# pettni/smooth_feedback

Measured on AMD Instinct MI355X. Metric: QP solves/sec, higher is better.
Workload: dtype f64

## Files before the change

### smooth_feedback_amd/csrc/capi_sparse.hip

```cpp
#include <hip/hip_runtime.h>

#include <algorithm>
#include <chrono>
#include <cstdio>
#include <map>
#include <mutex>
#include <string>
#include <vector>

#include "../../include/sfb.h"
#include "capi_common.h"
#include "qp_sparse_kernel.h"
#include "sparse_plan.h"

struct sfb_sparse_qp_plan {
  sfb::SparsePlanHost host;
  bool pruned = false;
  sfb::SparsePlanHost full;
  std::vector<int32_t> Aorig, Amasked;
  std::mutex mu;
  struct DevCopy {
    int32_t *blob = nullptr, *blob_full = nullptr;
    sfb::SparsePlanDev dev{}, dev_full{};
  };
  std::map<int, DevCopy> per_device;
  struct HostDev {
    std::mutex mu;
    std::pair<char *, size_t> ws{nullptr, 0};
    int64_t batch = -1;
    uint64_t origin = 0;
    hipStream_t stream = nullptr;
    hipEvent_t uploaded = nullptr;
  };
  std::map<int, HostDev> host_dev;
};

namespace sfb {
const SparsePlanHost &plan_host(const sfb_sparse_qp_plan *plan) { return plan->host; }
const SparsePlanHost &plan_io(const sfb_sparse_qp_plan *plan) { return plan->pruned ? plan->full : plan->host; }
}

namespace {

thread_local uint64_t tl_multi_origin = 0;

sfb_status upload_plan(const sfb::SparsePlanHost &h, const std::vector<int32_t> *Aorig, const std::vector<int32_t> *Amasked,
                       int nnzA_io, int32_t **blob_out, sfb::SparsePlanDev &d)
{
  static const std::vector<int32_t> none;
  const std::vector<int32_t> *arrs[] = {&h.Pp, &h.Pi, &h.Pcol, &h.Ap, &h.Aj, &h.Arow, &h.Acp, &h.Aci, &h.Acpos,
                                        &h.Prp, &h.Prj, &h.Prpos, &h.Sp, &h.Sj, &h.Spos, &h.perm, &h.pinv,
                                        &h.Kp, &h.Ki, &h.Kdesc, &h.Lp, &h.Li, &h.Rp, &h.Rk, &h.Rpos, &h.Rlen,
                                        &h.fmap, &h.fidx, &h.bmap, &h.bidx, &h.Kmap, &h.rptr, &h.rtgt, &h.rab, &h.snptr, &h.snR, &h.poff, &h.pmap, &h.fmask, &h.bmask,
                                        &h.f2s, &h.seg, &h.pmapL, &h.rsplit, &h.KmapL, &h.KdescT, &h.KmapT, &h.ztop, &h.ustream, &h.utype, &h.uomap,
                                        Aorig ? Aorig : &none, Amasked ? Amasked : &none};
  constexpr int NA = sizeof(arrs) / sizeof(arrs[0]);
  size_t off[NA + 1];
  off[0] = 0;
  for (int a = 0; a < NA; ++a) off[a + 1] = off[a] + ((arrs[a]->size() + 3) / 4) * 4 + 4;
  const size_t self_words = (sizeof(sfb::SparsePlanDev) + 15) / 16 * 4;
  std::vector<int32_t> blob(off[NA] + self_words, 0);
  for (int a = 0; a < NA; ++a) std::copy(arrs[a]->begin(), arrs[a]->end(), blob.begin() + off[a]);
  int32_t *dblob = nullptr;
  hipError_t e = hipMalloc(reinterpret_cast<void **>(&dblob), blob.size() * sizeof(int32_t));
  if (e != hipSuccess) return sfb::hip_fail(e, "hipMalloc(plan)");
  e = hipMemcpy(dblob, blob.data(), blob.size() * sizeof(int32_t), hipMemcpyHostToDevice);
  if (e != hipSuccess) {
    (void)hipFree(dblob);
    return sfb::hip_fail(e, "hipMemcpy(plan)");
  }
  d.n = h.n; d.m = h.m; d.k = h.k; d.nnzP = h.nnzP; d.nnzA = h.nnzA; d.nnzK = h.nnzK; d.nnzL = h.nnzL;
  const int32_t **ptrs[] = {&d.Pp, &d.Pi, &d.Pcol, &d.Ap, &d.Aj, &d.Arow, &d.Acp, &d.Aci, &d.Acpos,
                            &d.Prp, &d.Prj, &d.Prpos, &d.Sp, &d.Sj, &d.Spos, &d.perm, &d.pinv,
                            &d.Kp, &d.Ki, &d.Kdesc, &d.Lp, &d.Li, &d.Rp, &d.Rk, &d.Rpos, &d.Rlen,
                            &d.fmap, &d.fidx, &d.bmap, &d.bidx, &d.Kmap, &d.rptr, &d.rtgt, &d.rab, &d.snptr, &d.snR, &d.poff, &d.pmap, &d.fmask, &d.bmask,
                            &d.f2s, &d.seg, &d.pmapL, &d.rsplit, &d.KmapL, &d.KdescT, &d.KmapT, &d.ztop, &d.ustream, &d.utype, &d.uomap,
                            &d.Aorig, &d.Amasked};
  d.funits = h.funits; d.bunits = h.bunits; d.ffull0 = h.ffull0; d.ffull1 = h.ffull1; d.bfull0 = h.bfull0; d.bfull1 = h.bfull1; d.idx_scale = h.idx_scale; d.rsteps = h.rsteps; d.maxcol = h.maxcol; d.nsn = h.nsn; d.lds_doubles = h.lds_doubles; d.nseg = h.nseg; d.nnzKT = h.nnzKT; d.nztop = h.nztop; d.units = h.units; d.nunits = h.nunits;
  for (int a = 0; a < NA; ++a) *ptrs[a] = dblob + off[a];
  d.nnzA_io = nnzA_io;
  d.nmasked = Amasked ? (int)Amasked->size() - 512 : 0;
  if (!Aorig) d.Aorig = d.Amasked = nullptr;
  if ((e = sfb::sparse_device_words(&d.dev_active, &d.dev_busy)) != hipSuccess) {
    (void)hipFree(dblob);
    return sfb::hip_fail(e, "launch bookkeeping of the device");
  }
  d.self = reinterpret_cast<const sfb::SparsePlanDev *>(dblob + off[NA]);
  e      = hipMemcpy(dblob + off[NA], &d, sizeof(d), hipMemcpyHostToDevice);
  if (e != hipSuccess) {
    (void)hipFree(dblob);
    return sfb::hip_fail(e, "hipMemcpy(plan struct)");
  }
  *blob_out = dblob;
  return SFB_OK;
}

sfb_status plan_on_device(sfb_sparse_qp_plan *plan, const sfb_sparse_qp_plan::DevCopy **out)
{
  int devid = 0;
  hipError_t e = hipGetDevice(&devid);
  if (e != hipSuccess) return sfb::hip_fail(e, "hipGetDevice");
  std::lock_guard<std::mutex> lk(plan->mu);
  auto it = plan->per_device.find(devid);
  if (it != plan->per_device.end()) {
    *out = &it->second;
    return SFB_OK;
  }
  sfb_sparse_qp_plan::DevCopy dc;
  sfb_status st;
  if (plan->pruned) {
    st = upload_plan(plan->host, &plan->Aorig, &plan->Amasked, plan->full.nnzA, &dc.blob, dc.dev);
    if (st != SFB_OK) return st;
    st = upload_plan(plan->full, nullptr, nullptr, plan->full.nnzA, &dc.blob_full, dc.dev_full);
    if (st != SFB_OK) {
      (void)hipFree(dc.blob);
      return st;
    }
  } else {
    st = upload_plan(plan->host, nullptr, nullptr, plan->host.nnzA, &dc.blob, dc.dev);
    if (st != SFB_OK) return st;
  }
  auto ins = plan->per_device.emplace(devid, dc);
  *out     = &ins.first->second;
  return SFB_OK;
}

struct WsLayout {
  size_t item_bytes, main_bytes, pool_off, aux_off, total;
};
WsLayout ws_layout(const sfb_sparse_qp_plan *plan, int64_t batch)
{
  const sfb::SparsePlanHost &h = plan->host;
  WsLayout L{};
  L.item_bytes = sfb::qp_sparse_ws_doubles(h.n, h.m, h.nnzL, h.funits, h.bunits, plan->pruned ? h.nnzA : 0) * sizeof(double);
  L.main_bytes = (size_t)batch * L.item_bytes;
  L.pool_off   = L.main_bytes;
  size_t pool  = 0;
  if (plan->pruned) {
    const sfb::SparsePlanHost &f = plan->full;
    pool = (size_t)std::min<int64_t>(batch, sfb::qp_sparse_fallback_slots()) *
           sfb::qp_sparse_ws_doubles(f.n, f.m, f.nnzL, f.funits, f.bunits, 0) * sizeof(double);
  }
  L.aux_off = L.pool_off + pool;
  L.total   = L.aux_off + (sfb::qp_sparse_aux_bytes(batch) + 15) / 16 * 16;
  return L;
}

sfb_status check_sparse_args(const sfb_sparse_qp_plan *plan, const sfb_qp_params *prm, int64_t batch, const void *Px,
                             const void *q, const void *Ax, const void *l, const void *u, const void *wx,
                             const void *wy, const void *x, const void *y, const void *code)
{
  if (!plan) return sfb::fail(SFB_ERR_INVALID_ARG, "plan is NULL");
  if (!prm) return sfb::fail(SFB_ERR_INVALID_ARG, "prm is NULL");
  if (batch < 0) return sfb::fail(SFB_ERR_INVALID_ARG, "batch < 0");
  if (batch > 0 && (!q || !l || !u || !x || !y || !code || (plan->host.nnzP > 0 && !Px) || (sfb::plan_io(plan).nnzA > 0 && !Ax)))
    return sfb::fail(SFB_ERR_INVALID_ARG, "NULL problem / solution pointer");
  if ((wx == nullptr) != (wy == nullptr))
    return sfb::fail(SFB_ERR_INVALID_ARG, "warm_x and warm_y must both be given or both be NULL");
  if (prm->max_iter > 0xFFFFFFFFll) return sfb::fail(SFB_ERR_INVALID_ARG, "max_iter exceeds uint32");
  if (batch > 0x7FFFFFFFll) return sfb::fail(SFB_ERR_UNSUPPORTED, "batch exceeds 2^31-1 per call");
  if ((size_t)std::max(plan->host.lds_doubles, plan->pruned ? plan->full.lds_doubles : 0) * sizeof(double) > 150 * 1024)
    return sfb::fail(SFB_ERR_UNSUPPORTED, "n+m too large for the LDS-resident work vector (max 19200)");
  return SFB_OK;
}

}

extern "C" {

sfb_status sfb_sparse_qp_plan_create(int n, int m, const int32_t *P_colptr, const int32_t *P_rowind,
                                     const int32_t *A_rowptr, const int32_t *A_colind, int ordering,
                                     const int32_t *user_perm, sfb_sparse_qp_plan **plan)
{
  return sfb_sparse_qp_plan_create_staged(n, m, P_colptr, P_rowind, A_rowptr, A_colind, ordering, user_perm, nullptr,
                                          plan);
}

sfb_status sfb_sparse_qp_plan_create_staged(int n, int m, const int32_t *P_colptr, const int32_t *P_rowind,
                                            const int32_t *A_rowptr, const int32_t *A_colind, int ordering,
                                            const int32_t *user_perm, const int32_t *stage,
                                            sfb_sparse_qp_plan **plan)
{
  return sfb_sparse_qp_plan_create_pruned(n, m, P_colptr, P_rowind, A_rowptr, A_colind, ordering, user_perm, stage, nullptr,
                                          plan);
}

sfb_status sfb_sparse_qp_plan_create_pruned(int n, int m, const int32_t *P_colptr, const int32_t *P_rowind,
                                            const int32_t *A_rowptr, const int32_t *A_colind, int ordering,
                                            const int32_t *user_perm, const int32_t *stage, const uint8_t *A_keep,
                                            sfb_sparse_qp_plan **plan)
{
  if (!plan) return sfb::fail(SFB_ERR_INVALID_ARG, "plan out-pointer is NULL");
  *plan = nullptr;
  auto *p = new (std::nothrow) sfb_sparse_qp_plan();
  if (!p) return sfb::fail(SFB_ERR_INVALID_ARG, "out of memory");
  const char *msg = "";
  bool any_masked = false;
  if (A_keep && n >= 1 && m >= 1 && A_rowptr && A_rowptr[0] == 0 && A_rowptr[m] >= 0) {
    bool monotone = true;
    for (int r = 0; r < m && monotone; ++r) monotone = A_rowptr[r + 1] >= A_rowptr[r] && A_rowptr[r + 1] <= A_rowptr[m];
    for (int e = 0; monotone && e < A_rowptr[m] && !any_masked; ++e) any_masked = A_keep[e] == 0;
  }
  if (!any_masked) {
    if (!sfb::build_sparse_plan(n, m, P_colptr, P_rowind, A_rowptr, A_colind, ordering, user_perm, stage, p->host, &msg)) {
      delete p;
      return sfb::fail(SFB_ERR_INVALID_ARG, msg);
    }
    *plan = p;
    return SFB_OK;
  }
  const int nnzA = A_rowptr[m];
  if (nnzA > 0 && !A_colind) {
    delete p;
    return sfb::fail(SFB_ERR_INVALID_ARG, "A_colind is NULL");
  }
  std::vector<int32_t> Ap(m + 1, 0), Aj;
  Aj.reserve(nnzA);
  for (int r = 0; r < m; ++r) {
    if (A_rowptr[r + 1] < A_rowptr[r] || A_rowptr[r + 1] > nnzA) {
      delete p;
      return sfb::fail(SFB_ERR_INVALID_ARG, "A row pointers not monotone");
    }
    for (int e = A_rowptr[r]; e < A_rowptr[r + 1]; ++e)
      if (A_colind[e] < 0 || A_colind[e] >= n) {
        delete p;
        return sfb::fail(SFB_ERR_INVALID_ARG, "A column index out of range");
      } else if (A_keep[e]) {
        Aj.push_back(A_colind[e]);
        p->Aorig.push_back(e);
      } else {
        p->Amasked.push_back(e);
      }
// ... 343 lines not shown
```

### smooth_feedback_amd/csrc/knobs.cpp

```cpp
#include "knobs.h"

#include <atomic>
#include <cstdio>
#include <cstring>
#include <deque>
#include <map>
#include <mutex>
#include <string>

namespace sfb {

namespace {
const char *const kKnobs[] = {"SFB_SP_GRID",  "SFB_SP_SLICE",  "SFB_SP_PAUSE",      "SFB_SP_PREDICT",   "SFB_SP_LAT",
                              "SFB_SP_FORCE_LAT", "SFB_SP_LAT_WAVES", "SFB_SP_POLISHERS", "SFB_SP_LAT_HELP", "SFB_SP_PHASED", "SFB_SP_LEAN_WAVES", "SFB_MID_GRID", "SFB_MID_SLICE",
                              "SFB_QP4_MAX_WAVES", "SFB_QP_DENSE_BIG", "SFB_EKF_PERSISTENT", "SFB_PLAN_UNITS", "SFB_PLAN_DEBUG", "SFB_MPC_TIMING"};
std::mutex g_mu;
std::atomic<int> g_set{0};
std::map<std::string, const char *> &table()
{
  static std::map<std::string, const char *> t;
  return t;
}
const char *intern(const char *value)
{
  static std::deque<std::string> pool;
  for (const auto &v : pool)
    if (v == value) return v.c_str();
  pool.emplace_back(value);
  return pool.back().c_str();
}
}

const char *knob(const char *name)
{
  if (g_set.load(std::memory_order_acquire) == 0) return nullptr;
  std::lock_guard<std::mutex> lk(g_mu);
  const auto &t = table();
  const auto it = t.find(name);
  return it == t.end() ? nullptr : it->second;
}

int knob_set(const char *name, const char *value)
{
  if (name == nullptr) return 1;
  bool known = false;
  for (const char *k : kKnobs) known = known || std::strcmp(k, name) == 0;
  if (!known) return 1;
  std::lock_guard<std::mutex> lk(g_mu);
  if (value == nullptr) {
    table().erase(name);
    g_set.store((int)table().size(), std::memory_order_release);
  } else {
    table()[name] = intern(value);
    g_set.store((int)table().size(), std::memory_order_release);
    std::fprintf(stderr, "[sfb] debug knob %s=%s set through sfb_debug_set (tests and measurements only; results do not depend on it)\n",
                 name, value);
  }
  return 0;
}

}
```

### smooth_feedback_amd/csrc/qp_sparse.hip

```cpp
#include <hip/hip_runtime.h>

#include <cstdlib>
#include <map>
#include <mutex>

#include <algorithm>
#include <type_traits>
#include <utility>
#include <cfloat>
#include <cmath>

#include "knobs.h"
#include "../../include/sfb.h"
#include "qp_sparse_kernel.h"
#include "wave_util.h"

#ifndef SFB_SWEEP_ASM
#define SFB_SWEEP_ASM 1
#endif
#ifndef SFB_SWEEP_DEPTH
#define SFB_SWEEP_DEPTH 8
#endif

namespace sfb {

namespace {

__device__ __forceinline__ int uni(const int v) { return __builtin_amdgcn_readfirstlane(v); }

struct Ws {
  double *Lx, *LxF, *LxB, *D, *Dinv, *tv;
  double *sx, *qc, *xs, *xus, *dxus;
  double *sy, *rho, *rinv, *lo, *hi, *ys, *zs, *yus, *zus, *dyus, *act;
  double *hdr;
  double *Axc;
};
constexpr int kHdrStamp = 6, kHdrC = 7, kHdrSigma = 8, kHdrScaling = 9;
constexpr int kHdrCode = 10, kHdrComplete = 11;
[[maybe_unused]] constexpr int kHdrTl2 = 12;
enum { PH_SETUP = 1, PH_ADMM = 2, PH_FINISH = 3 };
constexpr int phases_pack(int ph0, int ph1, unsigned pause_at = 0, int dq_mode = 0)
{
  return ph0 | (ph1 << 4) | (int)((pause_at & 0xFFFFFu) << 8) | (dq_mode << 28);
}
constexpr int PH_EVERYTHING = phases_pack(PH_SETUP, PH_FINISH);
constexpr unsigned long long kFactorStamp = 0x5FB0FAC7A11CE5EDull;

__device__ __forceinline__ Ws carve_ws(double *base, int n, int m, int nnzL, int funits, int bunits)
{
  const int k = n + m;
  Ws w;
  double *p = base;
  w.Lx = p; p += nnzL;
  w.D = p; p += k;
  p += 2;
  w.LxF = p; p += (size_t)(funits + kSweepPadDev) * 128;
  w.LxB = p; p += (size_t)(bunits + kSweepPadDev) * 128;
  w.Dinv = p; p += k;   w.tv = p; p += k;
  w.sx = p; p += n;     w.qc = p; p += n;     w.xs = p; p += n;   w.xus = p; p += n;  w.dxus = p; p += n;
  p += n;
  w.sy = p; p += m;     w.rho = p; p += m;    w.rinv = p; p += m; w.lo = p; p += m;   w.hi = p; p += m;
  w.ys = p; p += m;     w.zs = p; p += m;     w.yus = p; p += m;  w.zus = p; p += m;  w.dyus = p; p += m;
  w.act = p; p += m;
  w.hdr = p; p += 16;
  w.Axc = p;
  return w;
}
__device__ __forceinline__ Ws polish_ws(const Ws &w, double *base, const size_t off, int n, int m, int nnzL, int funits, int bunits)
{
  const int k = n + m;
  Ws v = w;
  double *p = base + off;
  v.Lx = p; p += nnzL;
  v.D = p; p += k;
  p += 2;
  v.LxF = p; p += (size_t)(funits + kSweepPadDev) * 128;
  v.LxB = p; p += (size_t)(bunits + kSweepPadDev) * 128;
  v.Dinv = p;
  return v;
}

struct Item {
  const double *Px, *q, *Ax, *l, *u;
};

typedef int vint4k __attribute__((ext_vector_type(4)));
template<int U>
__device__ __forceinline__ void kkt_fill(const int32_t *__restrict__ desc4, const int32_t *__restrict__ map, const int p_begin,
                                         const int p_end, const Item &it, const Ws &w, double *ACC, const int mode,
                                         const double c, const double sigma, const double delta, const int lane)
{
  const vint4k *desc = reinterpret_cast<const vint4k *>(desc4);
  vint4k dn[U];
  int mn[U];
  auto fetch = [&](const int p0) {
#pragma unroll
    for (int u = 0; u < U; ++u) {
      const bool on = p0 + u * kWave < p_end;
      dn[u] = desc[on ? p0 + u * kWave : p_begin];
      mn[u] = map[on ? p0 + u * kWave : p_begin];
    }
  };
  if (p_begin + lane < p_end) fetch(p_begin + lane);
  for (int p0 = p_begin + lane; p0 < p_end; p0 += kWave * U) {
    vint4k d[U];
    int mp[U];
#pragma unroll
    for (int u = 0; u < U; ++u) {
      d[u]  = dn[u];
      mp[u] = mn[u];
    }
    double s1[U], s2[U], val[U], ac[U];
#pragma unroll
    for (int u = 0; u < U; ++u) {
      const bool on  = p0 + u * kWave < p_end;
      const int kind = on ? d[u].x : K_SIGMA, idx = d[u].y, r = d[u].z, cc = d[u].w;
      d[u].x         = kind;
      const bool isP = kind == K_P, isA = kind == K_A;
      s1[u]  = (isP || isA) ? (isP ? w.sx : w.sy)[r] : 0.0;
      s2[u]  = (isP || isA) ? w.sx[cc] : 0.0;
      val[u] = isP ? it.Px[idx] : (isA ? it.Ax[idx] : (kind == K_RHO ? w.rho[idx] : 0.0));
      ac[u]  = (isA && mode != 0) ? w.act[r] : 1.0;
    }
    if (p0 + kWave * U < p_end) fetch(p0 + kWave * U);
#pragma unroll
    for (int u = 0; u < U; ++u) {
      const int kind = d[u].x, r = d[u].z, cc = d[u].w;
      double v;
      if (kind == K_P) {
        if (mode == 0) v = c * s1[u] * s2[u] * val[u];
        else v = c * s2[u] * s1[u] * val[u];
        if (r == cc) v += (mode == 0) ? sigma : delta;
      } else if (kind == K_A) {
        v = s1[u] * s2[u] * val[u];
        if (ac[u] == 0.0) v = 0.0;
      } else if (kind == K_SIGMA) {
        v = (mode == 0) ? sigma : 0.0 + delta;
      } else {
        v = (mode == 0) ? (-1.0 / val[u]) : 0.0 - delta;
      }
      if (p0 + u * kWave < p_end) ACC[mp[u]] = v;
    }
  }
}

template<int DEPTH, bool PIPE>
__device__ __forceinline__ void trailing_block(const double *pan, const double *mul, const int R, const int wd,
                                               const int (&tp)[DEPTH], const unsigned (&ab)[DEPTH], double (&v)[DEPTH],
                                               double *ACC)
{
  int ra[DEPTH], rb[DEPTH];
#pragma unroll
  for (int dd = 0; dd < DEPTH; ++dd) {
    ra[dd] = wd + (int)(ab[dd] & 0xFFFFu);
    rb[dd] = wd + (int)(ab[dd] >> 16);
  }
  if constexpr (PIPE) {
    double a[DEPTH], b[DEPTH];
#pragma unroll
    for (int dd = 0; dd < DEPTH; ++dd) {
      a[dd] = pan[ra[dd]];
      b[dd] = mul[rb[dd]];
    }
    for (int jj = 0; jj < wd; ++jj) {
      const int jn = (jj + 1 < wd) ? jj + 1 : jj;
      double an[DEPTH], bn[DEPTH];
#pragma unroll
      for (int dd = 0; dd < DEPTH; ++dd) {
        an[dd] = pan[jn * R + ra[dd]];
        bn[dd] = mul[jn * R + rb[dd]];
      }
#pragma unroll
      for (int dd = 0; dd < DEPTH; ++dd) v[dd] = fma(-a[dd], b[dd], v[dd]);
#pragma unroll
      for (int dd = 0; dd < DEPTH; ++dd) {
        a[dd] = an[dd];
        b[dd] = bn[dd];
      }
    }
  } else {
    for (int jj = 0; jj < wd; ++jj) {
      double a[DEPTH], b[DEPTH];
#pragma unroll
      for (int dd = 0; dd < DEPTH; ++dd) {
        a[dd] = pan[jj * R + ra[dd]];
        b[dd] = mul[jj * R + rb[dd]];
      }
#pragma unroll
      for (int dd = 0; dd < DEPTH; ++dd) v[dd] = fma(-a[dd], b[dd], v[dd]);
    }
  }
#pragma unroll
  for (int dd = 0; dd < DEPTH; ++dd) ACC[tp[dd]] = v[dd];
}

constexpr int kPanelCols = 16;

template<int W>
__device__ __forceinline__ bool panel_eliminate_w(double (&reg)[kPanelCols], const int wd, const int R, double *pan,
                                                  double *mul, const int lane)
{
#pragma unroll
  for (int jj = 0; jj < W; ++jj) {
    if (jj < wd) {
      const double d = lane_bcast(reg[jj], jj);
      if (d == 0.0) return false;
      const double v  = reg[jj] / d;
      const double mv = v * d;
      if (lane > jj) reg[jj] = v;
      if (lane < R) {
        pan[jj * R + lane] = reg[jj];
        mul[jj * R + lane] = mv;
      }
#pragma unroll
      for (int rb = jj + 1; rb < W; ++rb) reg[rb] = fma(-v, lane_bcast(mv, rb), reg[rb]);
    }
  }
  return true;
}
__device__ __forceinline__ bool panel_eliminate(double (&reg)[kPanelCols], const int wd, const int R, double *pan, double *mul,
                                                const int lane)
{
  return panel_eliminate_w<kPanelCols>(reg, wd, R, pan, mul, lane);
}

#ifndef SFB_COPY_DEPTH
#define SFB_COPY_DEPTH 16
#endif
#ifndef SFB_COPY_UB
#define SFB_COPY_UB 8
#endif
template<int DEPTH>
__device__ __forceinline__ void ldl_sweep_copies(const SparsePlanDev &pl, const Ws &w, const int lane)
{
  const int k = uni(pl.k), nnzL = uni(pl.nnzL);
  const double *ACC = w.Lx;
  auto gather_copy = [&](const int32_t *__restrict__ map, double *__restrict__ dst, const int total) {
    int srcn[DEPTH];
#pragma unroll
    for (int dd = 0; dd < DEPTH; ++dd) srcn[dd] = map[lane + dd * kWave];
    for (int q0 = lane; q0 < total; q0 += kWave * DEPTH) {
      int src[DEPTH];
      double v[DEPTH];
#pragma unroll
      for (int dd = 0; dd < DEPTH; ++dd) src[dd] = srcn[dd];
#pragma unroll
      for (int dd = 0; dd < DEPTH; ++dd) v[dd] = ACC[src[dd] >= 0 ? src[dd] : nnzL + k + 1];
      if (q0 + kWave * DEPTH < total) {
#pragma unroll
        for (int dd = 0; dd < DEPTH; ++dd) srcn[dd] = map[q0 + kWave * DEPTH + dd * kWave];
      }
#pragma unroll
      for (int dd = 0; dd < DEPTH; ++dd) __builtin_nontemporal_store(v[dd], &dst[q0 + dd * kWave]);
    }
  };
  static_assert(kSweepPadDev * 2 >= DEPTH, "copy loop assumes whole blocks");
  wave_sync();
  gather_copy(pl.fmap, w.LxF, (uni(pl.funits) + kSweepPadDev) * 2 * kWave);
  gather_copy(pl.bmap, w.LxB, (uni(pl.bunits) + kSweepPadDev) * 2 * kWave);
  wave_sync();
}

typedef int vint4u __attribute__((ext_vector_type(4)));
template<int DEPTH>
__device__ inline int ldl_numeric_units(const SparsePlanDev &pl, const Item &it, const Ws &w, double *t, const int mode,
                                        const double c, const double sigma, const double delta, const int lane,
                                        unsigned long long *fill_ticks = nullptr)
{
  unsigned long long fclk = fill_ticks ? wall_clock64() : 0ull;
  auto fill_lap = [&](const bool is_fill) {
    if (fill_ticks) {
      const unsigned long long now = wall_clock64();
      if (is_fill) *fill_ticks += now - fclk;
      fclk = now;
    }
  };
  const int nnzL = uni(pl.nnzL);
#ifdef SFB_PROF_LDL
  unsigned long long pt[6] = {0, 0, 0, 0, 0, 0}, pc = __builtin_amdgcn_s_memtime();
#define SFB_ULAP(i) { const unsigned long long now_ = __builtin_amdgcn_s_memtime(); pt[i] += now_ - pc; pc = now_; }
#else
#define SFB_ULAP(i)
#endif
  double *ACC = w.Lx;
  for (int z = 0, nz = uni(pl.nztop); z < nz; ++z) {
    const int z0 = uni(pl.ztop[2 * z]), zn = uni(pl.ztop[2 * z + 1]);
    for (int p = lane; p < zn; p += kWave) ACC[z0 + p] = 0.0;
  }
  wave_sync();
  kkt_fill<4>(pl.KdescT, pl.KmapT, 0, uni(pl.nnzKT), it, w, ACC, mode, c, sigma, delta, lane);
  wave_sync();
  SFB_ULAP(0)
  fill_lap(true);
  const vint4u *__restrict__ stream = reinterpret_cast<const vint4u *>(pl.ustream);
  auto at = [&](const unsigned off) -> double & { return *reinterpret_cast<double *>(reinterpret_cast<char *>(t) + off); };
  bool zero_pivot = false;
  constexpr int UB = SFB_COPY_UB;
  for (int sg = 0, nseg = uni(pl.nseg); sg < nseg; ++sg) {
    const int32_t *sgp = pl.seg + 12 * sg;
    const int u0 = uni(sgp[0]), u1 = uni(sgp[1]), c0 = uni(sgp[2]), c1 = uni(sgp[3]), closed = uni(sgp[4]), nLs = uni(sgp[5]);
    const int accN = uni(sgp[6]), kp0 = uni(sgp[7]), kp1 = uni(sgp[8]), gL = uni(sgp[9]), nout = uni(sgp[10]);
    const int32_t *__restrict__ omap = pl.uomap + uni(sgp[11]);
    const int sink = accN + nout;
    if (closed) {
      for (int e = lane; e < accN; e += kWave) t[e] = 0.0;
      wave_lds_fence();
      kkt_fill<4>(pl.Kdesc, pl.KmapL, kp0, kp1, it, w, t, mode, c, sigma, delta, lane);
    } else {
      for (int e0 = lane; e0 < accN; e0 += kWave * UB) {
        double v[UB];
#pragma unroll
        for (int e = 0; e < UB; ++e) {
          const int x = e0 + e * kWave;
          v[e] = (x < accN) ? ACC[x < nLs ? gL + x : nnzL + c0 + (x - nLs)] : 0.0;
        }
#pragma unroll
        for (int e = 0; e < UB; ++e)
          if (e0 + e * kWave < accN) t[e0 + e * kWave] = v[e];
      }
    }
    for (int e0 = lane; e0 < nout; e0 += kWave * UB) {
      int src[UB];
      double v[UB];
#pragma unroll
      for (int e = 0; e < UB; ++e) src[e] = omap[e0 + e * kWave];
#pragma unroll
      for (int e = 0; e < UB; ++e) v[e] = ACC[src[e]];
#pragma unroll
      for (int e = 0; e < UB; ++e)
        if (e0 + e * kWave < nout) t[accN + e0 + e * kWave] = v[e];
    }
    if (lane < 3) t[sink + lane] = (lane == 2) ? 1.0 : 0.0;
    wave_lds_fence();
    SFB_ULAP(1)
    fill_lap(true);
    {
      typedef const __attribute__((address_space(1))) vint4u *gstream_t;
      gstream_t sp = (gstream_t)(stream + (size_t)u0 * kWave + lane);
      auto fetch = [&](vint4u (&q)[DEPTH]) {
#pragma unroll
        for (int d = 0; d < DEPTH; ++d) q[d] = sp[d * kWave];
        sp += DEPTH * kWave;
      };
      auto run = [&](const vint4u (&q)[DEPTH], const int ub) {
#pragma unroll
        for (int d = 0; d < DEPTH; ++d) {
          const unsigned x0 = (unsigned)q[d].x, y0 = (unsigned)q[d].y, x1 = (unsigned)q[d].z, y1 = (unsigned)q[d].w;
          const bool dm = __builtin_amdgcn_readfirstlane((int)y0) == -1;
          if (ub + d < u1) {
            if (dm) {
              const double T0 = at(x0 & 0xFFFFu), D0 = at(x0 >> 16), T1 = at(x1 & 0xFFFFu), D1 = at(x1 >> 16);
              at(x0 & 0xFFFFu) = T0 / D0;
              at(x1 & 0xFFFFu) = T1 / D1;
            } else {
              const double T0 = at(x0 & 0xFFFFu), A0 = at(x0 >> 16), B0 = at(y0 & 0xFFFFu), D0 = at(y0 >> 16);
              const double T1 = at(x1 & 0xFFFFu), A1 = at(x1 >> 16), B1 = at(y1 & 0xFFFFu), D1 = at(y1 >> 16);
              at(x0 & 0xFFFFu) = fma(-A0, B0 * D0, T0);
              at(x1 & 0xFFFFu) = fma(-A1, B1 * D1, T1);
            }
          }
        }
      };
      vint4u qa[DEPTH], qb[DEPTH];
      fetch(qa);
      for (int u = u0; u < u1; u += 2 * DEPTH) {
        fetch(qb);
        run(qa, u);
        fetch(qa);
        if (u + DEPTH < u1) run(qb, u + DEPTH);
      }
    }
    wave_lds_fence();
    SFB_ULAP(2)
    for (int e = lane; e < nLs; e += kWave) ACC[gL + e] = t[e];
    for (int j = c0 + lane; j < c1; j += kWave) {
      const double d = t[nLs + (j - c0)];
      zero_pivot = zero_pivot || d == 0.0;
      ACC[nnzL + j]      = d;
      w.Dinv[pl.f2s[j]] = 1.0 / d;
    }
    for (int e0 = lane; e0 < nout; e0 += kWave * UB) {
      int dst[UB];
#pragma unroll
      for (int e = 0; e < UB; ++e) dst[e] = omap[e0 + e * kWave];
#pragma unroll
      for (int e = 0; e < UB; ++e)
        if (e0 + e * kWave < nout) ACC[dst[e]] = t[accN + e0 + e * kWave];
    }
    wave_sync();
    SFB_ULAP(3)
    fill_lap(false);
  }
  if (wave_ballot(zero_pivot)) return 0;
  ldl_sweep_copies<SFB_COPY_DEPTH>(pl, w, lane);
  SFB_ULAP(4)
#ifdef SFB_PROF_LDL
  if (lane == 0 && (blockIdx.x == 0 || blockIdx.x == gridDim.x - 1))
    printf("[ldl units block %u mode %d] zero+open fill %llu  segments: working set in %llu  units %llu  out %llu | copies %llu  (cycles of s_memtime)\n",
           blockIdx.x, mode, pt[0], pt[1], pt[2], pt[3], pt[4]);
#endif
  return 1;
}

template<int DEPTH>
__device__ inline int ldl_numeric_dev(const SparsePlanDev &pl, const Item &it, const Ws &w, double *t, const int mode,
                                      const double c, const double sigma, const double delta, const int lane,
                                      unsigned long long *fill_ticks = nullptr)
{
  if (uni(pl.units)) return ldl_numeric_units<DEPTH>(pl, it, w, t, mode, c, sigma, delta, lane, fill_ticks);
  unsigned long long fclk = fill_ticks ? wall_clock64() : 0ull;
  auto fill_lap = [&](const bool is_fill) {
    if (fill_ticks) {
      const unsigned long long now = wall_clock64();
      if (is_fill) *fill_ticks += now - fclk;
      fclk = now;
    }
  };
  const int k = uni(pl.k), nnzL = uni(pl.nnzL);
#ifdef SFB_PROF_LDL
  unsigned long long pt[14] = {0, 0, 0, 0, 0, 0, 0, 0, 0, 0, 0, 0, 0, 0}, pc = __builtin_amdgcn_s_memtime();
#define SFB_LAP(i) { const unsigned long long now_ = __builtin_amdgcn_s_memtime(); pt[i] += now_ - pc; pc = now_; }
#else
#define SFB_LAP(i)
#endif
  double *ACC   = w.Lx;
  const int pad = nnzL + k;
  for (int z = 0, nz = uni(pl.nztop); z < nz; ++z) {
    const int z0 = uni(pl.ztop[2 * z]), zn = uni(pl.ztop[2 * z + 1]);
    for (int p = lane; p < zn; p += kWave) ACC[z0 + p] = 0.0;
  }
  wave_sync();
  kkt_fill<4>(pl.KdescT, pl.KmapT, 0, uni(pl.nnzKT), it, w, ACC, mode, c, sigma, delta, lane);
  wave_sync();
  SFB_LAP(0)
  fill_lap(true);
  for (int sg = 0, nseg = uni(pl.nseg); sg < nseg; ++sg) {
    const int32_t *sgp = pl.seg + 12 * sg;
    const int sn0 = uni(sgp[0]), sn1 = uni(sgp[1]), on_chip = uni(sgp[4]);
    fill_lap(false);
    if (on_chip) {
      const int accN = uni(sgp[6]), kp0 = uni(sgp[7]), kp1 = uni(sgp[8]), nLs = uni(sgp[5]);
      const int gL = uni(sgp[9]), gD = nnzL + uni(sgp[2]) - nLs;
      const int zero = accN + 1;
      double *scr    = t + ((accN + 2 + 1) & ~1);
      for (int e = lane; e < accN + 2; e += kWave) t[e] = 0.0;
      wave_lds_fence();
      kkt_fill<4>(pl.Kdesc, pl.KmapL, kp0, kp1, it, w, t, mode, c, sigma, delta, lane);
      wave_lds_fence();
      SFB_LAP(1)
      fill_lap(true);
      constexpr int DL = 4;
      int j0 = uni(pl.snptr[sn0]), wd = uni(pl.snptr[sn0 + 1]) - j0, R = uni(pl.snR[sn0]);
      int srcL[kPanelCols];
      {
        const int32_t *pmL = pl.pmapL + uni(pl.poff[sn0]);
#pragma unroll
        for (int jj = 0; jj < kPanelCols; ++jj) srcL[jj] = (jj < wd && lane < R) ? pmL[jj * R + lane] : zero;
      }
      for (int sn = sn0; sn < sn1; ++sn) {
        const int s0 = uni(pl.rptr[sn]), sp = uni(pl.rsplit[sn]), s1 = uni(pl.rptr[sn + 1]);
        double *pan = scr, *mul = scr + wd * R;
        int tpx[DL];
        unsigned abx[DL];
        double accx[DL];
#pragma unroll
        for (int dd = 0; dd < DL; ++dd) {
          tpx[dd] = pl.rtgt[(sp + dd) * kWave + lane];
          abx[dd] = (unsigned)pl.rab[(sp + dd) * kWave + lane];
          if (sp + dd >= s1) {
            tpx[dd] = pad;
            abx[dd] = 0u;
          }
        }
#pragma unroll
        for (int dd = 0; dd < DL; ++dd) accx[dd] = ACC[tpx[dd]];
        double reg[kPanelCols];
#pragma unroll
        for (int jj = 0; jj < kPanelCols; ++jj) reg[jj] = t[srcL[jj]];
        const int snn = (sn + 1 < sn1) ? sn + 1 : sn;
        const int j0n = uni(pl.snptr[snn]), wdn = uni(pl.snptr[snn + 1]) - j0n, Rn = uni(pl.snR[snn]);
        int srcN[kPanelCols];
        {
          const int32_t *pmN = pl.pmapL + uni(pl.poff[snn]);
#pragma unroll
          for (int jj = 0; jj < kPanelCols; ++jj) srcN[jj] = (jj < wdn && lane < Rn) ? pmN[jj * Rn + lane] : zero;
        }
        SFB_LAP(8)
        if (!panel_eliminate(reg, wd, R, pan, mul, lane)) return 0;
        SFB_LAP(9)
#pragma unroll
        for (int jj = 0; jj < kPanelCols; ++jj) {
          if (srcL[jj] < accN) ACC[srcL[jj] + (srcL[jj] < nLs ? gL : gD)] = reg[jj];
          if (jj < wd && lane == jj) t[srcL[jj]] = reg[jj];
        }
        wave_lds_fence();
        SFB_LAP(10)
        for (int s = s0; s < sp; s += DL) {
          int tp[DL];
          unsigned ab[DL];
          double acc[DL];
#pragma unroll
          for (int dd = 0; dd < DL; ++dd) {
            tp[dd] = pl.rtgt[(s + dd) * kWave + lane];
            ab[dd] = (unsigned)pl.rab[(s + dd) * kWave + lane];
            if (s + dd >= sp) {
              tp[dd] = accN;
              ab[dd] = 0u;
            }
          }
#pragma unroll
          for (int dd = 0; dd < DL; ++dd) acc[dd] = t[tp[dd]];
          trailing_block<DL, true>(pan, mul, R, wd, tp, ab, acc, t);
        }
        SFB_LAP(11)
        trailing_block<DL, true>(pan, mul, R, wd, tpx, abx, accx, ACC);
        for (int s = sp + DL; s < s1; s += DL) {
          int tp[DL];
          unsigned ab[DL];
          double acc[DL];
#pragma unroll
          for (int dd = 0; dd < DL; ++dd) {
            tp[dd] = pl.rtgt[(s + dd) * kWave + lane];
            ab[dd] = (unsigned)pl.rab[(s + dd) * kWave + lane];
            if (s + dd >= s1) {
              tp[dd] = pad;
              ab[dd] = 0u;
            }
          }
#pragma unroll
          for (int dd = 0; dd < DL; ++dd) acc[dd] = ACC[tp[dd]];
          trailing_block<DL, true>(pan, mul, R, wd, tp, ab, acc, ACC);
        }
        wave_lds_fence();
        SFB_LAP(12)
        j0 = j0n; wd = wdn; R = Rn;
#pragma unroll
        for (int jj = 0; jj < kPanelCols; ++jj) srcL[jj] = srcN[jj];
      }
      {
        const int c0 = uni(sgp[2]), c1 = uni(sgp[3]);
        for (int j = c0 + lane; j < c1; j += kWave) w.Dinv[pl.f2s[j]] = 1.0 / t[nLs + (j - c0)];
      }
      SFB_LAP(2)
      wave_sync();
      continue;
    }
    for (int sn = sn0; sn < sn1; ++sn) {
    const int j0 = uni(pl.snptr[sn]), wd = uni(pl.snptr[sn + 1]) - j0;
    const int R  = uni(pl.snR[sn]);
    double *pan  = t;
    double *mul  = t + wd * R;
    const int s0 = uni(pl.rsplit[sn]), s1 = uni(pl.rptr[sn + 1]);
    int tp0[DEPTH];
    unsigned ab0[DEPTH];
    double acc0[DEPTH];
#pragma unroll
    for (int dd = 0; dd < DEPTH; ++dd) {
      tp0[dd] = pl.rtgt[(s0 + dd) * kWave + lane];
      ab0[dd] = (unsigned)pl.rab[(s0 + dd) * kWave + lane];
      if (s0 + dd >= s1) {
        tp0[dd] = pad;
        ab0[dd] = 0u;
// ... 242 lines not shown
                     "ds_read_b64 %[a1], %[np1]\n\t"
                     "ds_read_b64 %[b1], %[nt1]\n\t"
                     "global_load_dwordx2 %[ixo], %[ip], off offset:%[io]"
                     : [a0] "+v"(a0), [b0] "+v"(b0), [a1] "+v"(a1), [b1] "+v"(b1), [np0] "=&v"(np0), [nt0] "=&v"(nt0), [np1] "=&v"(np1),
                       [nt1] "=&v"(nt1), [ixo] "=v"(ix[D])
                     : [vx] "v"(vx), [vy] "v"(vy), [ct0] "v"(ct0), [ct1] "v"(ct1), [tb] "v"(tb), [ixx] "v"(ix[N].x), [ixy] "v"(ix[N].y),
                       [ip] "v"(ip[D / 8]), [io] "n"((D % 8) * kWave * 8), [w] "n"(W));
      }
      ct0 = nt0;
      ct1 = nt1;
      (void)np0; (void)np1;
    };
    auto unit = [&]<int D>(std::integral_constant<int, D> dd) {
      unit_g(dd, std::integral_constant<int, 12>{}, std::integral_constant<int, 0>{}, lx[D].x, lx[D].y);
    };
    int u_first = 0;
    if constexpr (RES > 0) {
      auto for_prefix = [&]<int... U>(std::integer_sequence<int, U...>, auto &&fn) { (fn(std::integral_constant<int, U>{}), ...); };
      for_prefix(std::make_integer_sequence<int, RES + DEPTH>{}, [&]<int U>(std::integral_constant<int, U>) {
        constexpr int D = U % DEPTH;
        constexpr auto loads = [](int v) { return v < RES ? 1 : 2; };
        constexpr int W = loads(U + 2) + loads(U + 3) + loads(U + 4) + loads(U + 5) + loads(U + 6) + loads(U + 7);
        constexpr int TK = (U + DEPTH < RES) ? 1 : 0;
        double vx, vy;
        if constexpr (U < RES) {
          int l0, h0, l1, h1;
          asm volatile("v_accvgpr_read_b32 %0, a[%4]\n\tv_accvgpr_read_b32 %1, a[%5]\n\tv_accvgpr_read_b32 %2, a[%6]\n\tv_accvgpr_read_b32 %3, a[%7]"
                       : "=v"(l0), "=v"(h0), "=v"(l1), "=v"(h1)
                       : "n"(kAgprFree + 4 * U), "n"(kAgprFree + 4 * U + 1), "n"(kAgprFree + 4 * U + 2), "n"(kAgprFree + 4 * U + 3));
          vx = __hiloint2double(h0, l0);
          vy = __hiloint2double(h1, l1);
        } else {
          vx = lx[D].x;
          vy = lx[D].y;
        }
        unit_g(std::integral_constant<int, D>{}, std::integral_constant<int, W>{}, std::integral_constant<int, TK>{}, vx, vy);
        if constexpr (D == DEPTH - 1) {
          advance(DEPTH);
          mt += DEPTH;
        }
      });
      static_assert((RES + DEPTH) % DEPTH == 0, "whole blocks");
      u_first = RES + DEPTH;
    }
    for (int u0 = u_first; u0 + (NEXT ? DEPTH : 0) < units; u0 += DEPTH) {
      for_units(std::make_integer_sequence<int, DEPTH>{}, unit);
      advance(DEPTH);
      mt += DEPTH;
    }
    if constexpr (NEXT) {
#pragma unroll
      for (int e = 0; e < NVP; ++e) vp[e] = reinterpret_cast<const vdouble2 *>(vals_next) + lane + e * 4 * kWave;
#pragma unroll
      for (int e = 0; e < NIP; ++e) ip[e] = reinterpret_cast<const vint2 *>(idx_next) + lane + e * 8 * kWave;
      {
        const unsigned long long a = reinterpret_cast<unsigned long long>(mask_next);
        const unsigned lo = (unsigned)__builtin_amdgcn_readfirstlane((int)(unsigned)a);
        const unsigned hi = (unsigned)__builtin_amdgcn_readfirstlane((int)(unsigned)(a >> 32));
        mt = reinterpret_cast<const int32_t *>(((unsigned long long)hi << 32) | lo);
      }
      for_units(std::make_integer_sequence<int, DEPTH>{}, unit);
    }
    asm volatile("s_waitcnt lgkmcnt(0)" : "+v"(a0), "+v"(b0), "+v"(a1), "+v"(b1) : : "memory");
    if constexpr (NEXT) {
      wave_lds_fence();
    } else {
#pragma unroll
      for (int d = 0; d < DEPTH; ++d) stream_wait<0>(lx[d], ix[d]);
      wave_sync();
    }
    return;
#undef SFB_SDWA_HI
#undef SFB_SDWA_LO
  }
  stream_wait<2 * (DEPTH - 1)>(lx[0], ix[0]);
  Addr cur = extract(ix[0]);
  auto block = [&]<int MODE>(std::integral_constant<int, MODE> msk, const int u0) {
    constexpr bool MASKED = MODE == 2;
    sint8 mk;
    if constexpr (MASKED) mask_fetch(mk, mask32, __builtin_amdgcn_readfirstlane((u0 + DEPTH) * 4));
    for_units(std::make_integer_sequence<int, DEPTH>{}, [&]<int D>(std::integral_constant<int, D> dd) {
      constexpr int N = (D + 1) % DEPTH;
      const double a0 = at(cur.p0), b0 = at(cur.t0), a1 = at(cur.p1), b1 = at(cur.t1);
      stream_wait<2 * (DEPTH - 2)>(lx[N], ix[N]);
      const Addr nxt = extract(ix[N]);
      at(cur.t0) = fma(-lx[D].x, a0, b0);
      at(cur.t1) = fma(-lx[D].y, a1, b1);
      if constexpr (D == 0 && MASKED) mask_wait(mk);
      issue(dd, msk, mk);
      cur = nxt;
    });
    advance(DEPTH);
  };
  const int r0 = max(0, min(units, full0 - DEPTH)), r1 = max(r0, min(units, full1 - DEPTH));
  int u0 = 0;
  if constexpr (LEAN) {
    for (; u0 < r0; u0 += DEPTH) block(std::integral_constant<int, 2>{}, u0);
    for (; u0 < r1; u0 += DEPTH) block(std::integral_constant<int, 1>{}, u0);
    for (; u0 < units; u0 += DEPTH) block(std::integral_constant<int, 2>{}, u0);
  } else {
    for (; u0 + (NEXT ? DEPTH : 0) < units; u0 += DEPTH) {
      block(std::integral_constant<int, 0>{}, u0);
    }
    if constexpr (NEXT) {
#pragma unroll
      for (int e = 0; e < NVP; ++e) vp[e] = reinterpret_cast<const vdouble2 *>(vals_next) + lane + e * 4 * kWave;
#pragma unroll
      for (int e = 0; e < NIP; ++e) ip[e] = reinterpret_cast<const vint2 *>(idx_next) + lane + e * 8 * kWave;
      block(std::integral_constant<int, 0>{}, u0);
    }
  }
  if constexpr (NEXT) {
    wave_lds_fence();
  } else {
#pragma unroll
    for (int d = 0; d < DEPTH; ++d) stream_wait<0>(lx[d], ix[d]);
    wave_sync();
  }
}

template<int SD>
__device__ inline void ldl_solve_dev(const SparsePlanDev &pl, const Ws &w, double *t, const int lane, const bool lean,
                                     const double *dinv_lds = nullptr)
{
  const double *const Dinv = dinv_lds ? dinv_lds : w.Dinv;
  const int k = uni(pl.k);
  const bool bo = uni(pl.idx_scale) == 8;
  auto sweep = [&](const int32_t *idx, const int units, const double *vals, const int32_t *mask, const int f0, const int f1) {
    if (lean) {
      vdouble2 lx[SFB_SWEEP_DEPTH];
      vint2 ix[SFB_SWEEP_DEPTH];
      if (bo) sweep_dev<SFB_SWEEP_DEPTH, true, true>(idx, units, vals, t, lane, mask, f0, f1, lx, ix);
      else sweep_dev<SFB_SWEEP_DEPTH, false, true>(idx, units, vals, t, lane, mask, f0, f1, lx, ix);
    } else {
      vdouble2 lx[SD];
      vint2 ix[SD];
      if (bo) sweep_dev<SD, true, false>(idx, units, vals, t, lane, mask, f0, f1, lx, ix);
      else sweep_dev<SD, false, false>(idx, units, vals, t, lane, mask, f0, f1, lx, ix);
    }
  };
  sweep(pl.fidx, uni(pl.funits), w.LxF, pl.fmask, uni(pl.ffull0), uni(pl.ffull1));
  for (int j0 = lane; j0 < k; j0 += kWave * 8) {
    double dv[8];
#pragma unroll
    for (int e = 0; e < 8; ++e) dv[e] = (j0 + e * kWave < k) ? Dinv[j0 + e * kWave] : 0.0;
#pragma unroll
    for (int e = 0; e < 8; ++e)
      if (j0 + e * kWave < k) t[j0 + e * kWave] = dv[e] * t[j0 + e * kWave];
  }
  wave_sync();
  sweep(pl.bidx, uni(pl.bunits), w.LxB, pl.bmask, uni(pl.bfull0), uni(pl.bfull1));
}

constexpr int kLatRegRows = 12;
__host__ __device__ constexpr size_t lat_lds_doubles(const int n, const int m)
{
  return (size_t)(((n + m + 2) + 1) & ~1) + n + 2 * (size_t)m + (n + m) + 8 + (2 * kLatRegRows * 64) / 4 + (kLatRegRows * 64) / 8 + 4;
}
constexpr int kLatResident = (256 - kAgprFree) / 4;
__device__ __forceinline__ bool lat_resident_ok(const SparsePlanDev &pl) { return uni(pl.funits) >= kLatResident + 16; }
__device__ __forceinline__ void lat_resident_load(const double *LxF, const int lane)
{
  asm volatile("" ::: "a255");
  const vdouble2 *p = reinterpret_cast<const vdouble2 *>(LxF) + lane;
  auto for_units = [&]<int... U>(std::integer_sequence<int, U...>, auto &&fn) { (fn(std::integral_constant<int, U>{}), ...); };
  for_units(std::make_integer_sequence<int, kLatResident / 4>{}, [&]<int G>(std::integral_constant<int, G>) {
    const vdouble2 *pg = p + G * 4 * kWave;
    asm volatile("global_load_dwordx4 a[%1:%2], %0, off\n\t"
                 "global_load_dwordx4 a[%3:%4], %0, off offset:1024\n\t"
                 "global_load_dwordx4 a[%5:%6], %0, off offset:2048\n\t"
                 "global_load_dwordx4 a[%7:%8], %0, off offset:3072"
                 :
                 : "v"(pg), "n"(kAgprFree + 16 * G), "n"(kAgprFree + 16 * G + 3), "n"(kAgprFree + 16 * G + 4), "n"(kAgprFree + 16 * G + 7),
                   "n"(kAgprFree + 16 * G + 8), "n"(kAgprFree + 16 * G + 11), "n"(kAgprFree + 16 * G + 12), "n"(kAgprFree + 16 * G + 15)
                 : "memory");
  });
  asm volatile("s_waitcnt vmcnt(0)" ::: "memory");
}
__device__ __forceinline__ void ldl_solve_lat(const SparsePlanDev &pl, const Ws &w, double *t, const int lane, const double *Dinv,
                                              vdouble2 (&lx)[8], vint2 (&ix)[8], const bool pre, const bool next, const bool resident = false)
{
  const int k = uni(pl.k);
  if (resident) sweep_dev<8, true, false, false, true, kLatResident>(pl.fidx, uni(pl.funits), w.LxF, t, lane, pl.fmask, 0, 0, lx, ix, pl.bidx, w.LxB, pl.bmask);
  else if (pre) sweep_dev<8, true, false, true, true>(pl.fidx, uni(pl.funits), w.LxF, t, lane, pl.fmask, 0, 0, lx, ix, pl.bidx, w.LxB, pl.bmask);
  else sweep_dev<8, true, false, false, true>(pl.fidx, uni(pl.funits), w.LxF, t, lane, pl.fmask, 0, 0, lx, ix, pl.bidx, w.LxB, pl.bmask);
  for (int j0 = lane; j0 < k; j0 += kWave * 8) {
    double dv[8];
#pragma unroll
    for (int e = 0; e < 8; ++e) dv[e] = (j0 + e * kWave < k) ? Dinv[j0 + e * kWave] : 0.0;
#pragma unroll
    for (int e = 0; e < 8; ++e)
      if (j0 + e * kWave < k) t[j0 + e * kWave] = dv[e] * t[j0 + e * kWave];
  }
  wave_lds_fence();
  if (next) sweep_dev<8, true, false, true, true>(pl.bidx, uni(pl.bunits), w.LxB, t, lane, pl.bmask, 0, 0, lx, ix, pl.fidx, w.LxF, pl.fmask);
  else sweep_dev<8, true, false, true, false>(pl.bidx, uni(pl.bunits), w.LxB, t, lane, pl.bmask, 0, 0, lx, ix);
}

template<int UB>
__device__ __forceinline__ double lane_max_abs_b(const double *v, const int len, const int lane)
{
  double r = 0.0;
  for (int e0 = lane; e0 < len; e0 += kWave * UB) {
    double x[UB];
#pragma unroll
    for (int e = 0; e < UB; ++e) x[e] = (e0 + e * kWave < len) ? v[e0 + e * kWave] : 0.0;
#pragma unroll
    for (int e = 0; e < UB; ++e) r = fmax(r, fabs(x[e]));
  }
  return wave_max(r);
}
__device__ __forceinline__ double lane_max_abs(const double *v, int len, int lane)
{
  double r = 0.0;
  for (int e = lane; e < len; e += kWave) r = fmax(r, fabs(v[e]));
  return wave_max(r);
}

constexpr int kRowChunk = 8;
template<class PosF, class IdxF>
__device__ __forceinline__ double sp_row_dot(const int p0, const int p1, const double *vals, PosF pos, IdxF idx,
                                             const double *v)
{
  double s = 0.0;
  for (int q = p0; q < p1; q += kRowChunk) {
    int ps[kRowChunk], ix[kRowChunk];
    double a[kRowChunk], x[kRowChunk];
#pragma unroll
    for (int e = 0; e < kRowChunk; ++e) {
      const bool on = q + e < p1;
      ps[e] = on ? pos(q + e) : 0;
      ix[e] = on ? idx(q + e) : 0;
    }
#pragma unroll
    for (int e = 0; e < kRowChunk; ++e) {
      a[e] = vals[ps[e]];
      x[e] = v[ix[e]];
    }
#pragma unroll
    for (int e = 0; e < kRowChunk; ++e)
      if (q + e < p1) s = fma(a[e], x[e], s);
  }
  return s;
}
template<int RB, int CE, class PtrF, class PosF, class IdxF>
__device__ __forceinline__ void sp_rows_dot(double (&s)[RB], const int i0, const int nrows, PtrF ptr, const double *vals, PosF pos,
                                            IdxF idx, const double *v)
{
  int p[RB], pe[RB];
#pragma unroll
  for (int r = 0; r < RB; ++r) {
    const int i = i0 + r * kWave;
    const bool on = i < nrows;
    p[r]  = on ? ptr(i) : 0;
    pe[r] = on ? ptr(i + 1) : 0;
    s[r]  = 0.0;
  }
  for (;;) {
    bool more = false;
#pragma unroll
    for (int r = 0; r < RB; ++r) more = more || p[r] < pe[r];
    if (!more) break;
    int ps[RB][CE], ix[RB][CE];
    double a[RB][CE], x[RB][CE];
#pragma unroll
    for (int r = 0; r < RB; ++r)
#pragma unroll
      for (int e = 0; e < CE; ++e) {
        const bool on = p[r] + e < pe[r];
        ps[r][e] = on ? pos(p[r] + e) : 0;
        ix[r][e] = on ? idx(p[r] + e) : 0;
      }
#pragma unroll
    for (int r = 0; r < RB; ++r)
#pragma unroll
      for (int e = 0; e < CE; ++e) {
        a[r][e] = vals[ps[r][e]];
        x[r][e] = v[ix[r][e]];
      }
#pragma unroll
    for (int r = 0; r < RB; ++r) {
#pragma unroll
      for (int e = 0; e < CE; ++e)
        if (p[r] + e < pe[r]) s[r] = fma(a[r][e], x[r][e], s[r]);
      p[r] += CE;
    }
  }
}
template<int RB, int CE>
__device__ __forceinline__ void sp_rows_A(double (&s)[RB], const SparsePlanDev &pl, const Item &it, int i0, const double *v)
{
  sp_rows_dot<RB, CE>(s, i0, uni(pl.m), [&](int i) { return pl.Ap[i]; }, it.Ax, [](int p) { return p; },
                      [&](int p) { return pl.Aj[p]; }, v);
}
template<int RB, int CE>
__device__ __forceinline__ void sp_rows_P(double (&s)[RB], const SparsePlanDev &pl, const Item &it, int i0, const double *v)
{
  sp_rows_dot<RB, CE>(s, i0, uni(pl.n), [&](int i) { return pl.Prp[i]; }, it.Px, [&](int p) { return pl.Prpos[p]; },
                      [&](int p) { return pl.Prj[p]; }, v);
}
template<int RB, int CE>
__device__ __forceinline__ void sp_rows_At(double (&s)[RB], const SparsePlanDev &pl, const Item &it, int j0, const double *v)
{
  sp_rows_dot<RB, CE>(s, j0, uni(pl.n), [&](int j) { return pl.Acp[j]; }, it.Ax, [&](int p) { return pl.Acpos[p]; },
                      [&](int p) { return pl.Aci[p]; }, v);
}
__device__ __forceinline__ double sp_row_A(const SparsePlanDev &pl, const Item &it, int i, const double *v)
{
  return sp_row_dot(pl.Ap[i], pl.Ap[i + 1], it.Ax, [](int p) { return p; }, [&](int p) { return pl.Aj[p]; }, v);
}
__device__ __forceinline__ double sp_row_At(const SparsePlanDev &pl, const Item &it, int j, const double *v)
// ... 145 lines not shown
        for (int rr = 0; rr < RBX; ++rr) an = fmax(an, fabs(Atdy[rr]));
      }
      const double Aty_norm = wave_max(an);
      wave_sync();
      const double mxv      = (side == 1 || !(Aty_norm < acc)) ? Aty_norm : acc;
      if (mxv < thr) return SFB_QP_PRIMAL_INFEASIBLE;
    }
  }
  {
    double dmx = 0.0;
    constexpr int UBV = RBX > 4 ? 6 : 1;
    for (int e0 = lane; e0 < n; e0 += kWave * UBV) {
      double v[UBV];
#pragma unroll
      for (int e = 0; e < UBV; ++e) v[e] = (e0 + e * kWave < n) ? w.dxus[e0 + e * kWave] : 0.0;
#pragma unroll
      for (int e = 0; e < UBV; ++e)
        if (e0 + e * kWave < n) {
          t[e0 + e * kWave] = v[e];
          dmx               = fmax(dmx, fabs(v[e]));
        }
    }
    const double dx_norm = wave_max(dmx);
    const double thr     = kp.eps_dinf * dx_norm;
    wave_sync();
    double pn            = 0.0;
    for (int j0 = lane; j0 < n; j0 += kWave * 8) {
      double Pdx[8];
      sp_rows_P<8, 1>(Pdx, pl, it, j0, t);
#pragma unroll
      for (int rr = 0; rr < 8; ++rr) pn = fmax(pn, fabs(Pdx[rr]));
    }
    const double Pdx_n = wave_max(pn);
    if (!(Pdx_n <= thr)) return -1;
    wave_sync();
    double qdx = 0.0;
    for (int c0 = 0; c0 < n; c0 += chunk) {
      const int c1 = min(n, c0 + chunk);
      for (int j = c0 + lane; j < c1; j += kWave) {
        t[2 * (j - c0)]     = it.q[j];
        t[2 * (j - c0) + 1] = w.dxus[j];
      }
      wave_sync();
      {
        const int cnt = c1 - c0;
        int e = 0;
        for (; e + 8 <= cnt; e += 8) {
          vdouble2 v[8];
#pragma unroll
          for (int qq = 0; qq < 8; ++qq) v[qq] = *reinterpret_cast<const vdouble2 *>(t + 2 * (e + qq));
#pragma unroll
          for (int qq = 0; qq < 8; ++qq) qdx = fma(v[qq].x, v[qq].y, qdx);
        }
        for (; e < cnt; ++e) qdx = fma(t[2 * e], t[2 * e + 1], qdx);
      }
      wave_sync();
    }
    if (!(qdx <= thr)) return -1;
    bool rowok = true;
    for (int i = lane; i < m; i += kWave) {
      const double Adx = sp_row_A(pl, it, i, w.dxus), ui = it.u[i], li = it.l[i];
      if (ui == inf) rowok = rowok && (Adx >= -thr);
      else if (li == -inf) rowok = rowok && (Adx <= thr);
      else rowok = rowok && (fabs(Adx) < thr);
    }
    if (!wave_ballot(!rowok)) return SFB_QP_DUAL_INFEASIBLE;
  }
  return -1;
}

__device__ __noinline__ void sp_trace_row(const SparsePlanDev &pl, const Item &it, const Ws &w, double *t, const int lane,
                                          const uint32_t iter, const unsigned long long t0_ticks, double *row)
{
  const int n = uni(pl.n), m = uni(pl.m);
  const int chunk = (uni(pl.k) + 1) / 2;
  double pri = 0.0, dua = 0.0, o = 0.0;
  for (int i = lane; i < m; i += kWave) pri = fmax(pri, fabs(sp_row_A(pl, it, i, w.xus) - w.zus[i]));
  for (int c0 = 0; c0 < n; c0 += chunk) {
    const int c1 = min(n, c0 + chunk);
    for (int j = c0 + lane; j < c1; j += kWave) {
      const double Px = sp_row_P(pl, it, j, w.xus), qj = it.q[j];
      dua = fmax(dua, fabs(Px + qj + sp_row_At(pl, it, j, w.yus)));
      t[2 * (j - c0)]     = 0.5 * Px + qj;
      t[2 * (j - c0) + 1] = w.xus[j];
    }
    wave_sync();
    for (int e = 0; e < c1 - c0; ++e) o += t[2 * e] * t[2 * e + 1];
    wave_sync();
  }
  pri = wave_max(pri);
  dua = wave_max(dua);
  if (lane == 0) {
    row[0] = (double)iter;
    row[1] = o;
    row[2] = pri;
    row[3] = dua;
    row[4] = (double)(wall_clock64() - t0_ticks) * 0.01;
  }
}

template<int RB, int CE, class PtrF, class IdxF, class LoadF, class FmaF>
__device__ __forceinline__ void sp_rows_chain(double (&acc)[RB], const int i0, const int nrows, PtrF ptr, IdxF idx, LoadF load, FmaF fm)
{
  using IdxT = decltype(idx(0));
  using ValT = decltype(load(idx(0)));
  int p[RB], pe[RB];
#pragma unroll
  for (int r = 0; r < RB; ++r) {
    const int i = i0 + r * kWave;
    p[r] = pe[r] = 0;
    if (i < nrows) {
      const auto pp = ptr(i);
      p[r]  = pp.a;
      pe[r] = pp.b;
    }
  }
  IdxT ix[RB][CE];
  auto fetch = [&] {
#pragma unroll
    for (int r = 0; r < RB; ++r)
#pragma unroll
      for (int e = 0; e < CE; ++e) ix[r][e] = idx((p[r] + e < pe[r]) ? p[r] + e : 0);
  };
  fetch();
  for (;;) {
    bool more = false;
#pragma unroll
    for (int r = 0; r < RB; ++r) more = more || p[r] < pe[r];
    if (!more) break;
    ValT v[RB][CE];
    IdxT ic[RB][CE];
    bool on[RB][CE];
#pragma unroll
    for (int r = 0; r < RB; ++r)
#pragma unroll
      for (int e = 0; e < CE; ++e) {
        ic[r][e] = ix[r][e];
        v[r][e]  = load(ic[r][e]);
        on[r][e] = p[r] + e < pe[r];
      }
#pragma unroll
    for (int r = 0; r < RB; ++r) p[r] += CE;
    fetch();
#pragma unroll
    for (int r = 0; r < RB; ++r)
#pragma unroll
      for (int e = 0; e < CE; ++e)
        if (on[r][e]) acc[r] = fm(r, ic[r][e], v[r][e], acc[r]);
  }
}

template<int SD, bool WIDE = false>
__device__ inline void sp_polish(const SparsePlanDev &pl, const Item &it, const Ws &w, const Ws &wf, const DenseKernelParams &kp,
                                 double *t, const double c, const int lane, const bool lean)
{
  const int n = uni(pl.n), m = uni(pl.m), k = uni(pl.k);
  const double inf = INFINITY, eps = DBL_EPSILON;
  for (int i = lane; i < m; i += kWave) {
    const double yi = w.ys[i];
    double a        = 0.0;
    if (yi < -100 * eps && it.l[i] != -inf) a = 1.0;
    if (yi > 100 * eps && it.u[i] != inf) a = 2.0;
    w.act[i] = a;
  }
  for (int e = lane; e < k; e += kWave) w.tv[e] = 0.0;
  wave_sync();
  if (!ldl_numeric_dev<8>(pl, it, wf, t, 1, c, kp.sigma, kp.delta, lane)) return;
  for (uint32_t iter = 0; iter != kp.polish_iter; ++iter) {
#ifndef SFB_POLISH_RB
#define SFB_POLISH_RB 2
#define SFB_POLISH_CE 2
#endif
#ifndef SFB_POLISH_WIDE_RB
#define SFB_POLISH_WIDE_RB 2
#define SFB_POLISH_WIDE_CE 4
#endif
    constexpr int RB = WIDE ? SFB_POLISH_WIDE_RB : SFB_POLISH_RB, CE = WIDE ? SFB_POLISH_WIDE_CE : SFB_POLISH_CE;
    struct Ix { int a, b; };
    struct V3 { double a, b, c; };
    struct V4 { double a, b, c, d; };
    const bool zero_tv = iter == 0;
    for (int i0 = lane; i0 < n; i0 += kWave * RB) {
      double acc[RB], sxi[RB], qi[RB];
      int pv[RB];
#pragma unroll
      for (int r = 0; r < RB; ++r) {
        const int i = i0 + r * kWave;
        const bool on = i < n;
        acc[r] = 0.0;
        sxi[r] = on ? w.sx[i] : 0.0;
        qi[r]  = on ? it.q[i] : 0.0;
        pv[r]  = on ? pl.pinv[i] : k;
      }
      sp_rows_chain<RB, CE>(acc, i0, n, [&](int i) { return zero_tv ? Ix{0, 0} : Ix{pl.Sp[i], pl.Sp[i + 1]}; },
                            [&](int q) { return Ix{pl.Spos[q], pl.Sj[q]}; },
                            [&](const Ix &x) { return V3{it.Px[x.a], w.sx[x.b], w.tv[x.b]}; },
                            [&](int r, const Ix &x, const V3 &v, double a) {
                              const int i = i0 + r * kWave;
                              const double s_ec = (x.b > i) ? v.b : sxi[r], s_er = (x.b > i) ? sxi[r] : v.b;
                              return fma(c * s_ec * s_er * v.a, v.c, a);
                            });
      sp_rows_chain<RB, CE>(acc, i0, n, [&](int i) { return zero_tv ? Ix{0, 0} : Ix{pl.Acp[i], pl.Acp[i + 1]}; },
                            [&](int q) { return Ix{pl.Acpos[q], pl.Aci[q]}; },
                            [&](const Ix &x) { return V4{w.act[x.b], w.sy[x.b], it.Ax[x.a], w.tv[n + x.b]}; },
                            [&](int r, const Ix &, const V4 &v, double a) { return (v.a != 0.0) ? fma(v.b * sxi[r] * v.c, v.d, a) : a; });
#pragma unroll
      for (int r = 0; r < RB; ++r) {
        const double h = -c * (sxi[r] * qi[r]);
        if (i0 + r * kWave < n) t[pv[r]] = h - acc[r];
      }
    }
    for (int r0 = lane; r0 < m; r0 += kWave * RB) {
      double acc[RB], a_[RB], syr[RB], lb[RB], ub[RB];
      int pv[RB];
#pragma unroll
      for (int r = 0; r < RB; ++r) {
        const int rr = r0 + r * kWave;
        const bool on = rr < m;
        acc[r] = 0.0;
        a_[r]  = on ? w.act[rr] : 0.0;
        syr[r] = on ? w.sy[rr] : 0.0;
        lb[r]  = on ? it.l[rr] : 0.0;
        ub[r]  = on ? it.u[rr] : 0.0;
        pv[r]  = on ? pl.pinv[n + rr] : k;
      }
      sp_rows_chain<RB, CE>(acc, r0, m,
                            [&](int rr) { return (!zero_tv && w.act[rr] != 0.0) ? Ix{pl.Ap[rr], pl.Ap[rr + 1]} : Ix{0, 0}; },
                            [&](int q) { return Ix{q, pl.Aj[q]}; },
                            [&](const Ix &x) { return V3{it.Ax[x.a], w.sx[x.b], w.tv[x.b]}; },
                            [&](int r, const Ix &, const V3 &v, double a) { return fma(syr[r] * v.b * v.a, v.c, a); });
#pragma unroll
      for (int r = 0; r < RB; ++r) {
        double h = 0.0;
        if (a_[r] != 0.0) h = (a_[r] == 1.0) ? syr[r] * lb[r] : syr[r] * ub[r];
        if (r0 + r * kWave < m) t[pv[r]] = h - acc[r];
      }
    }
    wave_sync();
    ldl_solve_dev<SD>(pl, wf, t, lane, lean);
    for (int e = lane; e < k; e += kWave) w.tv[e] += t[pl.pinv[e]];
    wave_sync();
  }
  for (int j = lane; j < n; j += kWave) w.xs[j] = w.tv[j];
  for (int i = lane; i < m; i += kWave)
    if (w.act[i] != 0.0) w.ys[i] = w.tv[n + i];
  wave_sync();
}

constexpr int kQFresh = 0, kQHead = 16, kQTail = 32, kQRing = 48;

enum { SP_DONE = 0, SP_SUSPENDED = 2, SP_PAUSED = 3 };

__device__ __forceinline__ bool sp_guard_ok(const SparsePlanDev &pl, const double *__restrict__ Ax, const int lane)
{
  constexpr int UB = 8;
  const int nmasked = uni(pl.nmasked);
  bool bad = false;
  int srcn[UB];
#pragma unroll
  for (int e = 0; e < UB; ++e) srcn[e] = pl.Amasked[lane + e * kWave];
  for (int p0 = lane; p0 < nmasked; p0 += kWave * UB) {
    int src[UB];
    double v[UB];
#pragma unroll
    for (int e = 0; e < UB; ++e) src[e] = srcn[e];
#pragma unroll
    for (int e = 0; e < UB; ++e) v[e] = Ax[src[e]];
    if (p0 + kWave * UB < nmasked) {
#pragma unroll
      for (int e = 0; e < UB; ++e) srcn[e] = pl.Amasked[p0 + kWave * UB + e * kWave];
    }
#pragma unroll
    for (int e = 0; e < UB; ++e) bad = bad || !(v[e] == 0.0);
  }
  return wave_ballot(bad) == 0ull;
}

template<bool LAT, bool TRACE = false, bool WIDE = false>
__device__ __forceinline__ int sp_solve_item(const SparsePlanDev &pl, const DenseKernelParams &kp, const double *__restrict__ gPx,
                                             const double *__restrict__ gq, const double *__restrict__ gAx,
                                             const double *__restrict__ gl, const double *__restrict__ gu,
                                             const double *__restrict__ gwx, const double *__restrict__ gwy,
                                             double *__restrict__ gx, double *__restrict__ gy, double *__restrict__ gobj,
                                             uint32_t *__restrict__ giter, int32_t *__restrict__ gcode,
                                             double *__restrict__ gws, const size_t ws_doubles, const int lean_waves,
                                             bool lean, const size_t b, const size_t slot, double *t, const int lane,
                                             bool resume, const int32_t *queue, const int batch,
                                             const uint32_t slice, const bool allow_reuse, const int phases, float *score,
                                             double *trace = nullptr, const int trace_cap = 0, double *phase_us = nullptr)
{
  [[maybe_unused]] unsigned long long ph_clk = 0, ph_fill = 0;
  [[maybe_unused]] unsigned long long ph_t[6] = {0, 0, 0, 0, 0, 0};
  [[maybe_unused]] auto phase_lap = [&](const int i) {
    if constexpr (TRACE) {
      const unsigned long long now = wall_clock64();
      ph_t[i] += now - ph_clk;
      ph_clk = now;
    }
  };
  if constexpr (TRACE) ph_clk = wall_clock64();
  const int ph0 = phases & 15, ph1 = (phases >> 4) & 15;
  const uint32_t pause_at = ((uint32_t)phases >> 8) & 0xFFFFFu;
  const int n = uni(pl.n), m = uni(pl.m), k = uni(pl.k);
  const int nnzP = uni(pl.nnzP), nnzA = uni(pl.nnzA);
  Item it{gPx + b * (size_t)nnzP, gq + b * (size_t)n, gAx + b * (size_t)uni(pl.nnzA_io), gl + b * (size_t)m,
          gu + b * (size_t)m};
  const Ws w = carve_ws(gws + slot * ws_doubles, n, m, uni(pl.nnzL), uni(pl.funits), uni(pl.bunits));
#ifdef SFB_SP_TIMELINE
  unsigned long long tl0 = wall_clock64(), tl1 = 0, tl2 = 0;
#endif
  double c = 1.0;
  int ret_code = -1;
  uint32_t iter = 0;
  const uint32_t sci   = kp.stop_check_iter;
  const uint32_t maxit = kp.max_iter;
  uint32_t next_chk    = (sci >= 2) ? 1u : 0xFFFFFFFFu;
  [[maybe_unused]] int trace_rows = 0;
  if (lane == 0) t[k] = 0.0;
  const double inf = INFINITY;
  unsigned long long t0_ticks = wall_clock64();
  if (ph0 >= PH_ADMM) {
    if (w.hdr[kHdrComplete] == 1.0) return SP_DONE;
#ifdef SFB_SP_TIMELINE
    const bool tl_continued = !resume;
#endif
    if (!resume) ret_code = (int)w.hdr[kHdrCode];
    resume = true;
#ifdef SFB_SP_TIMELINE
    if (tl_continued && lane == 0) w.hdr[5] = (double)wall_clock64();
    wave_sync();
#endif
  }
  if (resume) {
    c        = w.hdr[0];
    iter     = (uint32_t)w.hdr[1];
    next_chk = (uint32_t)w.hdr[2];
    t0_ticks = (unsigned long long)w.hdr[3];
#ifdef SFB_SP_TIMELINE
    tl0 = (unsigned long long)w.hdr[4];
    tl1 = (unsigned long long)w.hdr[5];
#endif
    if (pl.Aorig != nullptr) it.Ax = w.Axc;
  } else {
  const bool keep = allow_reuse && kp.reuse != 0 && (unsigned long long)__double_as_longlong(w.hdr[kHdrStamp]) == kFactorStamp &&
                    w.hdr[kHdrSigma] == kp.sigma && w.hdr[kHdrScaling] == (double)kp.scaling;
  if (pl.Aorig != nullptr && keep) it.Ax = w.Axc;
  else if (pl.Aorig != nullptr) {
    constexpr int UB = 8;
    int srcn[UB];
#pragma unroll
    for (int e = 0; e < UB; ++e) srcn[e] = pl.Aorig[lane + e * kWave];
    for (int p0 = lane; p0 < nnzA; p0 += kWave * UB) {
      int src[UB];
      double v[UB];
#pragma unroll
      for (int e = 0; e < UB; ++e) src[e] = srcn[e];
#pragma unroll
      for (int e = 0; e < UB; ++e) v[e] = it.Ax[src[e]];
      if (p0 + kWave * UB < nnzA) {
#pragma unroll
        for (int e = 0; e < UB; ++e) srcn[e] = pl.Aorig[p0 + kWave * UB + e * kWave];
      }
#pragma unroll
      for (int e = 0; e < UB; ++e)
        if (p0 + e * kWave < nnzA) w.Axc[p0 + e * kWave] = v[e];
    }
    it.Ax = w.Axc;
    wave_sync();
  }

  bool keep_scaling = keep && !kp.scaling;
  if (kp.scaling) {
    for (int j = lane; j < n; j += kWave) {
      double v = 0.0;
      for (int p = pl.Pp[j]; p < pl.Pp[j + 1]; ++p) v = fmax(v, fabs(it.Px[p]));
      if (v == 0.0) v = 1.0;
      t[j] = v;
    }
    wave_sync();
    double sum = t[0];
    {
      int j = 1;
      for (; j + 16 <= n; j += 16) {
        double v[16];
#pragma unroll
        for (int qq = 0; qq < 16; ++qq) v[qq] = t[j + qq];
#pragma unroll
        for (int qq = 0; qq < 16; ++qq) sum += v[qq];
      }
      for (; j < n; ++j) sum += t[j];
    }
    const double qn = lane_max_abs(it.q, n, lane);
    c               = 1.0 / fmax(fmax(1e-6, sum / (double)n), qn);
    wave_sync();
    keep_scaling = keep && c == w.hdr[kHdrC];
  }
  if (!keep_scaling) {
    for (int j = lane; j < n; j += kWave) w.sx[j] = 1.0;
    for (int i = lane; i < m; i += kWave) w.sy[i] = 1.0;
    wave_sync();
  }
  if (kp.scaling && !keep_scaling) {
    int pass = 0;
    double crit;
    do {
      for (int e = lane; e < k; e += kWave) t[e] = 0.0;
      wave_sync();
      constexpr int UB = 8;
      {
        int rr[UB], cc[UB];
        double pv[UB];
        auto fetchP = [&](const int p0) {
#pragma unroll
          for (int e = 0; e < UB; ++e) {
            const int p = p0 + e * kWave;
            const bool on = p < nnzP;
            rr[e] = on ? pl.Pi[p] : 0;
            cc[e] = on ? pl.Pcol[p] : 0;
            pv[e] = on ? it.Px[p] : 0.0;
          }
        };
        fetchP(lane);
        for (int p0 = lane; p0 < nnzP; p0 += kWave * UB) {
          int c0[UB];
          double v0[UB], sr[UB], sc[UB];
#pragma unroll
          for (int e = 0; e < UB; ++e) {
            sr[e] = w.sx[rr[e]];
            sc[e] = w.sx[cc[e]];
            c0[e] = cc[e];
            v0[e] = pv[e];
          }
          fetchP(p0 + kWave * UB);
#pragma unroll
          for (int e = 0; e < UB; ++e)
            if (p0 + e * kWave < nnzP)
              __hip_atomic_fetch_max(&t[c0[e]], fabs(c * sr[e] * sc[e] * v0[e]), __ATOMIC_RELAXED, __HIP_MEMORY_SCOPE_WORKGROUP);
        }
      }
      {
        int rr[UB], cc[UB];
        double av[UB];
        auto fetchA = [&](const int p0) {
#pragma unroll
          for (int e = 0; e < UB; ++e) {
            const int p = p0 + e * kWave;
            const bool on = p < nnzA;
            rr[e] = on ? pl.Arow[p] : 0;
            cc[e] = on ? pl.Aj[p] : 0;
            av[e] = on ? it.Ax[p] : 0.0;
          }
        };
        fetchA(lane);
        for (int p0 = lane; p0 < nnzA; p0 += kWave * UB) {
          int r0[UB], c0[UB];
          double v0[UB], sr[UB], sc[UB];
#pragma unroll
          for (int e = 0; e < UB; ++e) {
            sr[e] = w.sy[rr[e]];
            sc[e] = w.sx[cc[e]];
            r0[e] = rr[e];
            c0[e] = cc[e];
            v0[e] = av[e];
          }
          fetchA(p0 + kWave * UB);
#pragma unroll
          for (int e = 0; e < UB; ++e) {
            if (p0 + e * kWave < nnzA) {
              const double v = fabs(sr[e] * sc[e] * v0[e]);
              __hip_atomic_fetch_max(&t[c0[e]], v, __ATOMIC_RELAXED, __HIP_MEMORY_SCOPE_WORKGROUP);
              __hip_atomic_fetch_max(&t[n + r0[e]], v, __ATOMIC_RELAXED, __HIP_MEMORY_SCOPE_WORKGROUP);
            }
          }
        }
      }
      wave_sync();
      double cm = 0.0;
      for (int e = lane; e < k; e += kWave) {
        double inc = t[e];
        if (inc == 0.0) inc = 1.0;
        t[e] = inc;
        cm   = fmax(cm, fabs(inc - 1.0));
      }
      wave_sync();
      for (int j = lane; j < n; j += kWave) w.sx[j] = sqrt(1.0 / fmax(t[j], 1e-8)) * w.sx[j];
      for (int i = lane; i < m; i += kWave) w.sy[i] = sqrt(1.0 / fmax(t[n + i], 1e-8)) * w.sy[i];
      crit = wave_max(cm);
      wave_sync();
    } while (pass++ < 10 && crit > 0.1);
  }

  bool keep_factor = keep_scaling;
  {
    bool bad = false, rho_changed = false;
    for (int i = lane; i < m; i += kWave) {
      const double li = it.l[i], ui = it.u[i], syi = w.sy[i];
      bad = bad || (li == inf) || (ui == -inf) || (ui - li < 0.0);
      double rho;
      if (li == -inf && ui == inf) rho = 1e-6;
      else if (syi * fabs(li - ui) < 1e-5) rho = 1e3 * kp.rho_bar;
      else rho = kp.rho_bar;
      if (keep_scaling) rho_changed = rho_changed || !(w.rho[i] == rho);
      w.rho[i]  = rho;
      w.rinv[i] = 1.0 / rho;
      w.lo[i]   = syi * li;
      w.hi[i]   = syi * ui;
    }
    for (int j = lane; j < n; j += kWave) w.qc[j] = c * w.sx[j] * it.q[j];
    if (wave_ballot(bad)) ret_code = SFB_QP_PRIMAL_INFEASIBLE;
    if (keep_scaling && wave_ballot(rho_changed)) keep_factor = false;
  }
  wave_sync();

  phase_lap(0);
  if (!keep_factor) {
    if (lane == 0) w.hdr[kHdrStamp] = 0.0;
    if (!ldl_numeric_dev<8>(pl, it, w, t, 0, c, kp.sigma, kp.delta, lane, TRACE ? &ph_fill : nullptr)) {
      ret_code = SFB_QP_UNKNOWN;
    } else if (lane == 0 && allow_reuse) {
      w.hdr[kHdrStamp]   = __longlong_as_double((long long)kFactorStamp);
      w.hdr[kHdrC]       = c;
      w.hdr[kHdrSigma]   = kp.sigma;
      w.hdr[kHdrScaling] = (double)kp.scaling;
    }
  }

  if constexpr (TRACE) {
    phase_lap(2);
    ph_t[1] = ph_fill;
    ph_t[2] -= ph_fill;
  }
#ifdef SFB_SP_TIMELINE
  tl1 = wall_clock64();
#endif
  if (gwx != nullptr) {
    const double *wx = gwx + b * (size_t)n, *wy = gwy + b * (size_t)m;
    for (int j = lane; j < n; j += kWave) w.xs[j] = (1.0 / w.sx[j]) * wx[j];
    for (int i = lane; i < m; i += kWave) {
      const double syi = w.sy[i];
      w.ys[i]          = c * ((1.0 / syi) * wy[i]);
      double acc       = 0.0;
      for (int q = pl.Ap[i], q1 = pl.Ap[i + 1]; q < q1; q += kRowChunk) {
        int j[kRowChunk];
        double av[kRowChunk], xv[kRowChunk];
#pragma unroll
        for (int a = 0; a < kRowChunk; ++a) {
          j[a]  = (q + a < q1) ? pl.Aj[q + a] : 0;
          av[a] = (q + a < q1) ? it.Ax[q + a] : 0.0;
        }
#pragma unroll
        for (int a = 0; a < kRowChunk; ++a) xv[a] = wx[j[a]];
#pragma unroll
        for (int a = 0; a < kRowChunk; ++a)
          if (q + a < q1) acc = fma(syi * av[a], xv[a], acc);
      }
      w.zs[i] = acc;
    }
  } else {
    for (int j = lane; j < n; j += kWave) w.xs[j] = 0.0;
    for (int i = lane; i < m; i += kWave) {
      w.ys[i] = 0.0;
      w.zs[i] = 0.0;
    }
  }
  wave_sync();
  }

  if (ph1 == PH_SETUP) {
    if (lane == 0) {
      w.hdr[0] = c;
      w.hdr[1] = 0.0;
      w.hdr[2] = (double)next_chk;
      w.hdr[3] = (double)t0_ticks;
#ifdef SFB_SP_TIMELINE
      w.hdr[4] = (double)tl0;
      w.hdr[5] = (double)tl1;
#endif
      w.hdr[kHdrCode]     = (double)ret_code;
      w.hdr[kHdrComplete] = 0.0;
    }
    return SP_DONE;
  }

  const uint32_t iter0 = iter;
  bool need_rhs        = true;
  double *vxs = w.xs, *vqc = w.qc, *vys = w.ys, *vzs = w.zs, *vrinv = w.rinv, *vrho = w.rho, *vlo = w.lo, *vhi = w.hi;
  const int32_t *vpinv = pl.pinv;
  [[maybe_unused]] double *vdinv = nullptr;
  [[maybe_unused]] const uint16_t *vp16 = nullptr;
  [[maybe_unused]] const uint8_t *vcls  = nullptr;
  const double rho_c0 = 1e-6, rho_c1 = 1e3 * kp.rho_bar, rho_c2 = kp.rho_bar;
  const double rinv_c0 = 1.0 / rho_c0, rinv_c1 = 1.0 / rho_c1, rinv_c2 = 1.0 / rho_c2;
  auto pinv_at = [&](const int e) -> int {
    if constexpr (LAT) return (int)vp16[e];
    else return vpinv[e];
  };
  auto rho_at = [&](const int i) -> double {
    if constexpr (LAT) { const int cl = vcls[i]; return cl == 0 ? rho_c0 : (cl == 1 ? rho_c1 : rho_c2); }
    else return vrho[i];
  };
  auto rinv_at = [&](const int i) -> double {
    if constexpr (LAT) { const int cl = vcls[i]; return cl == 0 ? rinv_c0 : (cl == 1 ? rinv_c1 : rinv_c2); }
    else return vrinv[i];
  };
  const bool iterates  = ph0 <= PH_ADMM && iter != maxit && ret_code < 0;
  constexpr int kLatRows = kLatRegRows;
  if constexpr (LAT) {
    if (n > kLatRows * kWave || m > kLatRows * kWave) __builtin_trap();
  }
  [[maybe_unused]] double xr[kLatRows], yr[kLatRows], zr[kLatRows];
  [[maybe_unused]] double *lqc = nullptr, *llo = nullptr, *lhi = nullptr;
  [[maybe_unused]] const double *lrtab = nullptr;
  auto regs_to_lds = [&](const double (&v)[kLatRows], double *dst, const int len) {
    double *const dl = dst + lane;
#pragma unroll
    for (int r = 0; r < kLatRows; ++r)
      if (lane < len - r * kWave) dl[r * kWave] = v[r];
  };
  auto lds_to_regs = [&](double (&v)[kLatRows], const double *src, const int len) {
    const double *const sl = src + lane;
#pragma unroll
    for (int r = 0; r < kLatRows; ++r) v[r] = (lane < len - r * kWave) ? sl[r * kWave] : 0.0;
  };
  [[maybe_unused]] auto copy_in = [&](double *dst, const double *src, const int len) {
    constexpr int UB = 6;
    for (int e0 = lane; e0 < len; e0 += kWave * UB) {
      double v[UB];
#pragma unroll
      for (int e = 0; e < UB; ++e) v[e] = (e0 + e * kWave < len) ? src[e0 + e * kWave] : 0.0;
#pragma unroll
      for (int e = 0; e < UB; ++e)
        if (e0 + e * kWave < len) dst[e0 + e * kWave] = v[e];
    }
  };
  auto iterate_in = [&] {
    if constexpr (LAT) {
      copy_in(t, w.xs, n);
      copy_in(t + n, w.ys, m);
      copy_in(lhi, w.zs, m);
      wave_sync();
      lds_to_regs(xr, t, n);
      lds_to_regs(yr, t + n, m);
      lds_to_regs(zr, lhi, m);
      wave_sync();
      copy_in(lhi, w.hi, m);
      wave_sync();
    }
  };
  if constexpr (LAT) {
    double *cq = t + ((k + 2) & ~1), *clo = cq + n, *chi = clo + m;
    lqc = cq; llo = clo; lhi = chi;
    vdinv = chi + m;
    constexpr int kPad = kLatRows * kWave;
    double *ltab = vdinv + k;
    lrtab = ltab;
    uint16_t *lp = reinterpret_cast<uint16_t *>(ltab + 8);
    uint8_t *lc  = reinterpret_cast<uint8_t *>(lp + 2 * kPad);
    vp16 = lp;
    vcls = lc;
#pragma unroll
    for (int r = 0; r < kLatRows; ++r) xr[r] = yr[r] = zr[r] = 0.0;
    if (iterates) {
      copy_in(cq, w.qc, n);
      copy_in(clo, w.lo, m);
#pragma unroll 1
      for (int e0 = lane; e0 < kPad; e0 += 4 * kWave) {
        int px[4], py[4];
        double rho[4];
#pragma unroll
        for (int q = 0; q < 4; ++q) {
// ... 244 lines not shown
          const double nu = tv[e], yo = yr[R0 + e], zo = zr[R0 + e];
          double zn = v_alpha * (ri * nu) + v_alphac * (ri * yo) + zo;
          zn = (zn < lo[e]) ? lo[e] : zn;
          zn = (hi[e] < zn) ? hi[e] : zn;
          const double yn = v_alphac * yo + v_alpha * nu + rh * zo - rh * zn;
          yr[R0 + e]  = yn;
          zr[R0 + e]  = zn;
          t_at(pv[e]) = zn - ri * yn;
        }
      };
      static_assert(kLatRows == 12, "batches of the register form");
      xbatch(std::integral_constant<int, 0>{}, std::integral_constant<int, 6>{});
      xbatch(std::integral_constant<int, 6>{}, std::integral_constant<int, 6>{});
      ybatch(std::integral_constant<int, 0>{}, std::integral_constant<int, 4>{});
      ybatch(std::integral_constant<int, 4>{}, std::integral_constant<int, 4>{});
      ybatch(std::integral_constant<int, 8>{}, std::integral_constant<int, 4>{});
    } else
    {
    all_rows(std::integral_constant<int, UNR_A>{}, n, xrows);
    all_rows(std::integral_constant<int, UNR_B>{}, m, yrows);
    }
    if constexpr (LAT) {
      if (chk) {
        vectors_home();
        vxs = t; vys = t + n; vzs = lhi;
      }
    }
    if (chk) {
      constexpr int UBU = LAT ? 6 : 1;
      for (int j0 = lane; j0 < n; j0 += kWave * UBU) {
        double sxv[UBU], xov[UBU];
#pragma unroll
        for (int e = 0; e < UBU; ++e) {
          const bool on = j0 + e * kWave < n;
          sxv[e] = on ? w.sx[j0 + e * kWave] : 0.0;
          xov[e] = on ? w.dxus[j0 + e * kWave] : 0.0;
        }
#pragma unroll
        for (int e = 0; e < UBU; ++e) {
          const int j = j0 + e * kWave;
          if (j < n) {
            const double xn = vxs[j], sxj = sxv[e], xo = xov[e];
            w.xus[j]  = sxj * xn;
            t[j]      = sxj * xn;
            w.dxus[j] = sxj * (xn - xo);
          }
        }
      }
      for (int i0 = lane; i0 < m; i0 += kWave * UBU) {
        double syv[UBU], yov[UBU];
#pragma unroll
        for (int e = 0; e < UBU; ++e) {
          const bool on = i0 + e * kWave < m;
          syv[e] = on ? w.sy[i0 + e * kWave] : 1.0;
          yov[e] = on ? w.dyus[i0 + e * kWave] : 0.0;
        }
#pragma unroll
        for (int e = 0; e < UBU; ++e) {
          const int i = i0 + e * kWave;
          if (i < m) {
            const double yn = vys[i], zn = vzs[i], syi = syv[e], yo = yov[e];
            w.yus[i]  = syi * yn / c;
            t[n + i]  = syi * yn / c;
            w.zus[i]  = (1.0 / syi) * zn;
            w.dyus[i] = syi * (yn - yo) / c;
          }
        }
      }
    }
    wave_sync();
    if (chk) {
      ret_code = sp_check_stopping<LAT ? 6 : 4>(pl, it, w, kp, t, lane, pause_at != 0 ? score : nullptr);
      if constexpr (TRACE) {
        if (trace != nullptr && trace_rows < trace_cap) sp_trace_row(pl, it, w, t, lane, iter, t0_ticks, trace + ((size_t)b * (size_t)trace_cap + (size_t)trace_rows) * 5);
        ++trace_rows;
      }
      if (ret_code < 0 && max_time_exceeded(kp.max_time_ns, t0_ticks)) ret_code = SFB_QP_MAX_TIME;
      wave_sync();
      if constexpr (LAT) iterate_in();
      lean = __builtin_amdgcn_readfirstlane(__hip_atomic_load(pl.dev_active, __ATOMIC_RELAXED, __HIP_MEMORY_SCOPE_AGENT)) >
             lean_waves;
      if (iter > 600) __builtin_amdgcn_s_setprio(3);
      else if (iter > 300) __builtin_amdgcn_s_setprio(2);
      else if (iter > 100) __builtin_amdgcn_s_setprio(1);
      if (pause_at != 0 && ret_code < 0 && iter + 1 >= pause_at && iter + 1 != maxit) {
        if (lane == 0) {
          w.hdr[0] = c;
          w.hdr[1] = (double)(iter + 1);
          w.hdr[2] = (double)next_chk;
          w.hdr[3] = (double)t0_ticks;
#ifdef SFB_SP_TIMELINE
          w.hdr[4] = (double)tl0;
          w.hdr[5] = (double)tl1;
#endif
          w.hdr[kHdrCode]     = -1.0;
          w.hdr[kHdrComplete] = 0.0;
        }
        __builtin_amdgcn_s_setprio(0);
        vectors_home();
        return SP_PAUSED;
      }
      if (queue != nullptr && ret_code < 0 && iter + 1 != maxit && iter + 1 - iter0 >= slice) {
        int wait = 0;
        if (lane == 0) {
          const int fresh = __hip_atomic_load(&queue[kQFresh], __ATOMIC_RELAXED, __HIP_MEMORY_SCOPE_AGENT);
          const int head  = __hip_atomic_load(&queue[kQHead], __ATOMIC_RELAXED, __HIP_MEMORY_SCOPE_AGENT);
          const int tail  = __hip_atomic_load(&queue[kQTail], __ATOMIC_RELAXED, __HIP_MEMORY_SCOPE_AGENT);
          wait            = (fresh < batch) || (tail - head > 0);
        }
        if (__builtin_amdgcn_readfirstlane(wait)) {
          if (lane == 0) {
            w.hdr[0] = c;
            w.hdr[1] = (double)(iter + 1);
            w.hdr[2] = (double)next_chk;
            w.hdr[3] = (double)t0_ticks;
#ifdef SFB_SP_TIMELINE
            w.hdr[4] = (double)tl0;
            w.hdr[5] = (double)tl1;
#endif
          }
          __builtin_amdgcn_s_setprio(0);
          vectors_home();
          return SP_SUSPENDED;
        }
      }
    }
  }
  __builtin_amdgcn_s_setprio(0);
  vectors_home();

#ifdef SFB_SP_TIMELINE
  tl2 = wall_clock64();
#endif
  if (ph1 == PH_ADMM) {
    if (lane == 0) {
      w.hdr[0] = c;
      w.hdr[1] = (double)iter;
      w.hdr[kHdrCode] = (double)ret_code;
#ifdef SFB_SP_TIMELINE
      w.hdr[kHdrTl2] = (double)tl2;
#endif
    }
    return SP_DONE;
  }
#ifdef SFB_SP_TIMELINE
  if (ph0 == PH_FINISH) tl2 = (unsigned long long)w.hdr[kHdrTl2];
#endif
  phase_lap(3);
  if (ret_code == SFB_QP_OPTIMAL && kp.polish) {
    if (kp.reuse != 0 && allow_reuse) {
      const Ws wp = polish_ws(w, gws + slot * ws_doubles,
                              qp_sparse_polish_offset(n, m, uni(pl.nnzL), uni(pl.funits), uni(pl.bunits), pl.Aorig ? nnzA : 0), n, m,
                              uni(pl.nnzL), uni(pl.funits), uni(pl.bunits));
      sp_polish<SFB_SWEEP_DEPTH, WIDE>(pl, it, w, wp, kp, t, c, lane, lean);
    } else {
      if (lane == 0) w.hdr[kHdrStamp] = 0.0;
      sp_polish<SFB_SWEEP_DEPTH, WIDE>(pl, it, w, w, kp, t, c, lane, lean);
    }
  }

  phase_lap(4);
  double *ox = gx + b * (size_t)n, *oy = gy + b * (size_t)m;
  for (int j = lane; j < n; j += kWave) {
    const double v = w.sx[j] * w.xs[j];
    ox[j]    = v;
    w.xus[j] = v;
  }
  for (int i = lane; i < m; i += kWave) oy[i] = w.sy[i] * w.ys[i] / c;
  wave_sync();
  if (gobj != nullptr) {
    const int chunk = (k + 1) / 2;
    double o        = 0.0;
    for (int c0 = 0; c0 < n; c0 += chunk) {
      const int c1 = min(n, c0 + chunk);
      struct Ix { int a, b; };
      struct V2 { double a, b; };
      constexpr int RB = 4, CE = 2;
      for (int i0 = c0 + lane; i0 < c1; i0 += kWave * RB) {
        double acc[RB], xi[RB], qi[RB];
#pragma unroll
        for (int r = 0; r < RB; ++r) {
          const int i = i0 + r * kWave;
          acc[r] = 0.0;
          xi[r]  = (i < c1) ? w.xus[i] : 0.0;
          qi[r]  = (i < c1) ? it.q[i] : 0.0;
        }
        sp_rows_chain<RB, CE>(acc, i0, c1, [&](int i) { return Ix{pl.Prp[i], pl.Prp[i + 1]}; },
                              [&](int q) { return Ix{pl.Prpos[q], pl.Prj[q]}; },
                              [&](const Ix &x) { return V2{it.Px[x.a], w.xus[x.b]}; },
                              [&](int, const Ix &, const V2 &v, double a) { return fma(0.5 * v.a, v.b, a); });
#pragma unroll
        for (int r = 0; r < RB; ++r) {
          const int i = i0 + r * kWave;
          if (i < c1) {
            t[2 * (i - c0)]     = xi[r];
            t[2 * (i - c0) + 1] = acc[r] + qi[r];
          }
        }
      }
      wave_sync();
      const int cnt = c1 - c0;
      int e = 0;
      for (; e + 8 <= cnt; e += 8) {
        vdouble2 v[8];
#pragma unroll
        for (int qq = 0; qq < 8; ++qq) v[qq] = *reinterpret_cast<const vdouble2 *>(t + 2 * (e + qq));
#pragma unroll
        for (int qq = 0; qq < 8; ++qq) o = fma(v[qq].x, v[qq].y, o);
      }
      for (; e < cnt; ++e) o = fma(t[2 * e], t[2 * e + 1], o);
      wave_sync();
    }
    if (lane == 0) gobj[b] = o;
  }
  if (lane == 0) {
    gcode[b] = (ret_code >= 0) ? ret_code : SFB_QP_MAX_ITERATIONS;
    if (giter != nullptr) giter[b] = iter;
#ifdef SFB_SP_TIMELINE
    oy[0] = (double)tl0; oy[1] = (double)tl1; oy[2] = (double)tl2; oy[3] = (double)wall_clock64();
#endif
  }
  if constexpr (TRACE) {
    wave_sync();
    phase_lap(5);
    if (phase_us != nullptr && lane == 0)
      for (int i = 0; i < 6; ++i) phase_us[b * 6 + i] = (double)ph_t[i] * 0.01;
  }
  return SP_DONE;
}

}

constexpr int kFbSlots = 64;
constexpr int kDqTail = 0, kDqHead = 32, kDqOver = 64, kDqOwn = 80, kDqRing = 96;
constexpr int kDqStarted = 88;

template<bool LAT, bool TRACE = false, bool POLISHER = false>
__global__ void __launch_bounds__(64, LAT ? 1 : ((TRACE || POLISHER) ? 2 : 3)) qp_sparse_kernel(const SparsePlanDev *__restrict__ plp, const DenseKernelParams kp,
                                                       const double *__restrict__ gPx, const double *__restrict__ gq,
                                                       const double *__restrict__ gAx, const double *__restrict__ gl,
                                                       const double *__restrict__ gu, const double *__restrict__ gwx,
                                                       const double *__restrict__ gwy, double *__restrict__ gx,
                                                       double *__restrict__ gy, double *__restrict__ gobj,
                                                       uint32_t *__restrict__ giter, int32_t *__restrict__ gcode,
                                                       double *__restrict__ gws, const size_t ws_doubles,
                                                       const int lean_waves, const int32_t *__restrict__ order,
                                                       int32_t *__restrict__ queue, const int batch, const uint32_t slice,
                                                       const SparsePlanDev *__restrict__ plf, double *__restrict__ gwsf,
                                                       const size_t wsf_doubles, int32_t *__restrict__ fbflags, const int phases, const int nfb,
                                                       float *__restrict__ keys, const int32_t *__restrict__ nfresh_dev,
                                                       const int mode_sel, double *__restrict__ trace, const int trace_cap,
                                                       double *__restrict__ phase_us)
{
  constexpr int dq_mode = POLISHER ? 2 : 0;
  const int ph0    = phases & 15;
  if constexpr (LAT) {
    if (blockIdx.x == 0 && threadIdx.x == 0 && ((phases >> 28) & 1) == 1)
      __hip_atomic_store(&(fbflags + kFbSlots + 2 * batch + 16)[kDqStarted], 1, __ATOMIC_RELAXED, __HIP_MEMORY_SCOPE_AGENT);
  }
  const int nfresh = nfresh_dev ? __builtin_amdgcn_readfirstlane(nfresh_dev[0]) : batch;
  const int nwaves = nfresh_dev ? __builtin_amdgcn_readfirstlane(nfresh_dev[1]) : (queue == nullptr ? (int)gridDim.x : batch);
  if (nfresh_dev != nullptr && (int)blockIdx.x >= nwaves) return;
  if (nfresh_dev != nullptr && mode_sel >= 0 && __builtin_amdgcn_readfirstlane(nfresh_dev[2]) != mode_sel) return;
  extern __shared__ __attribute__((aligned(16))) double t[];
  const int lane = threadIdx.x;
  for (bool first = true;; first = false) {
    int item = -1, resume = 0;
    if constexpr (dq_mode == 2) {
      if (first && (int)blockIdx.x >= __builtin_amdgcn_readfirstlane((fbflags + kFbSlots + 2 * batch)[10])) return;
      if (lane == 0) {
        int32_t *const doneq = fbflags + kFbSlots + 2 * batch + 16;
        for (;;) {
          if (__hip_atomic_load(&doneq[kDqOver], __ATOMIC_RELAXED, __HIP_MEMORY_SCOPE_AGENT) != 0) break;
          const int head = __hip_atomic_load(&doneq[kDqHead], __ATOMIC_RELAXED, __HIP_MEMORY_SCOPE_AGENT);
          const int tail = __hip_atomic_load(&doneq[kDqTail], __ATOMIC_RELAXED, __HIP_MEMORY_SCOPE_AGENT);
          if (head < tail) {
            if (atomicCAS(&doneq[kDqHead], head, head + 1) != head) continue;
            int v;
            while ((v = __hip_atomic_load(&doneq[kDqRing + head], __ATOMIC_RELAXED, __HIP_MEMORY_SCOPE_AGENT)) == 0) __builtin_amdgcn_s_sleep(4);
            item = v - 1;
            break;
          }
          __builtin_amdgcn_s_sleep(100);
        }
      }
      resume = 1;
    } else if (queue == nullptr) {
      if (first) item = order ? order[blockIdx.x] : (int)blockIdx.x;
    } else if (lane == 0) {
      if (__hip_atomic_load(&queue[kQFresh], __ATOMIC_RELAXED, __HIP_MEMORY_SCOPE_AGENT) < nfresh) {
        const int tk = atomicAdd(&queue[kQFresh], 1);
        if (tk < nfresh) item = order ? order[tk] : tk;
      }
      while (item < 0) {
        const int head = __hip_atomic_load(&queue[kQHead], __ATOMIC_RELAXED, __HIP_MEMORY_SCOPE_AGENT);
        const int tail = __hip_atomic_load(&queue[kQTail], __ATOMIC_RELAXED, __HIP_MEMORY_SCOPE_AGENT);
        if (tail - head <= 0) break;
        if (atomicCAS(&queue[kQHead], head, head + 1) != head) continue;
        int32_t *e = &queue[kQRing + (unsigned)head % (unsigned)batch];
        int v;
        while ((v = __hip_atomic_load(e, __ATOMIC_RELAXED, __HIP_MEMORY_SCOPE_AGENT)) == 0) __builtin_amdgcn_s_sleep(4);
        __hip_atomic_store(e, 0, __ATOMIC_RELAXED, __HIP_MEMORY_SCOPE_AGENT);
        item   = v - 1;
        resume = 1;
      }
      if constexpr (LAT) {
        if (item < 0 && ((phases >> 28) & 3) == 3) {
          int32_t *const doneq = fbflags + kFbSlots + 2 * batch + 16;
          const unsigned long long own_bit = 1ull << (nfresh_dev[8] & 63);
          for (;;) {
            if ((__hip_atomic_load(plp->dev_busy, __ATOMIC_RELAXED, __HIP_MEMORY_SCOPE_SYSTEM) & ~own_bit) != 0ull) break;
            if (__hip_atomic_load(plp->dev_active, __ATOMIC_RELAXED, __HIP_MEMORY_SCOPE_AGENT) -
                    __hip_atomic_load(&doneq[kDqOwn], __ATOMIC_RELAXED, __HIP_MEMORY_SCOPE_AGENT) > 0)
              break;
            const int head = __hip_atomic_load(&doneq[kDqHead], __ATOMIC_RELAXED, __HIP_MEMORY_SCOPE_AGENT);
            const int tail = __hip_atomic_load(&doneq[kDqTail], __ATOMIC_RELAXED, __HIP_MEMORY_SCOPE_AGENT);
            if (head >= tail) break;
            if (atomicCAS(&doneq[kDqHead], head, head + 1) != head) continue;
            int v;
            while ((v = __hip_atomic_load(&doneq[kDqRing + head], __ATOMIC_RELAXED, __HIP_MEMORY_SCOPE_AGENT)) == 0) __builtin_amdgcn_s_sleep(4);
            item   = v - 1;
            resume = 2;
            break;
          }
        }
      }
    }
    item   = __builtin_amdgcn_readfirstlane(item);
    resume = __builtin_amdgcn_readfirstlane(resume);
    const int lean_waves_item = lean_waves;
    if (item < 0) break;
    if (resume) __builtin_amdgcn_fence(__ATOMIC_ACQUIRE, "agent");
    const bool helper = LAT && resume == 2;
    if (dq_mode == 2 || helper) resume = 0;
    wave_sync();
    const SparsePlanDev *use = plp;
    double *wsb              = gws;
    size_t wsd = ws_doubles, slot = (queue == nullptr) ? (size_t)blockIdx.x : (size_t)item;
    int fbslot = -1;
    if (plf != nullptr && !resume && ph0 <= PH_SETUP && !sp_guard_ok(*plp, gAx + (size_t)item * (size_t)uni(plp->nnzA_io), lane)) {
      if (lane == 0) {
        for (int probe = blockIdx.x % nfb;; probe = (probe + 1) % nfb) {
          if (atomicCAS(&fbflags[probe], 0, 1) == 0) { fbslot = probe; break; }
          __builtin_amdgcn_s_sleep(8);
        }
      }
      fbslot = __builtin_amdgcn_readfirstlane(fbslot);
      use = plf; wsb = gwsf; wsd = wsf_doubles; slot = (size_t)fbslot;
    }
    int seen = 0;
    const bool counts_own = dq_mode == 2 || (LAT && ((phases >> 28) & 1) == 1);
    if (counts_own && lane == 0) atomicAdd(&(fbflags + kFbSlots + 2 * batch + 16)[kDqOwn], 1);
    int32_t *const active = plp->dev_active;
    if (lane == 0) seen = atomicAdd(active, 1);
    const bool lean = (nwaves > lean_waves_item) || __builtin_amdgcn_readfirstlane(seen) >= lean_waves_item;
    const int st = sp_solve_item<LAT, TRACE, LAT || POLISHER>(*use, kp, gPx, gq, gAx, gl, gu, gwx, gwy, gx, gy, gobj, giter, gcode, wsb, wsd, lean_waves_item,
                                 lean, (size_t)item, slot, t, lane, resume != 0, fbslot >= 0 ? nullptr : queue, nfresh, slice,
                                  fbslot < 0 && slot == (size_t)item,
                                 fbslot >= 0 ? PH_EVERYTHING : (helper ? (PH_FINISH | (PH_FINISH << 4)) : phases), keys ? keys + item : nullptr, trace,
                                 trace_cap, phase_us);
    if (keys != nullptr && st != SP_PAUSED && lane == 0) keys[item] = -1.0f;
    if (fbslot >= 0 && phases != PH_EVERYTHING && lane == 0)
      carve_ws(gws + (size_t)item * ws_doubles, uni(plp->n), uni(plp->m), uni(plp->nnzL), uni(plp->funits), uni(plp->bunits)).hdr[kHdrComplete] = 1.0;
    if ((dq_mode == 2 || helper) && lane == 0)
      carve_ws(gws + (size_t)item * ws_doubles, uni(plp->n), uni(plp->m), uni(plp->nnzL), uni(plp->funits), uni(plp->bunits)).hdr[kHdrComplete] = 1.0;
    wave_sync();
    if constexpr (LAT) {
      if (st == SP_DONE && !helper && (phases & 0xFF) == (PH_ADMM | (PH_ADMM << 4)) && ((phases >> 28) & 1) == 1 && lane == 0) {
        int32_t *const doneq = fbflags + kFbSlots + 2 * batch + 16;
        __builtin_amdgcn_fence(__ATOMIC_RELEASE, "agent");
        asm volatile("s_waitcnt vmcnt(0)" ::: "memory");
        const int tl = atomicAdd(&doneq[kDqTail], 1);
        __hip_atomic_store(&doneq[kDqRing + tl], item + 1, __ATOMIC_RELAXED, __HIP_MEMORY_SCOPE_AGENT);
      }
    }
    if (lane == 0) {
      atomicSub(active, 1);
      if (counts_own) atomicSub(&(fbflags + kFbSlots + 2 * batch + 16)[kDqOwn], 1);
      if (fbslot >= 0) __hip_atomic_store(&fbflags[fbslot], 0, __ATOMIC_RELEASE, __HIP_MEMORY_SCOPE_AGENT);
      if (st == SP_SUSPENDED) {
        __builtin_amdgcn_fence(__ATOMIC_RELEASE, "agent");
        asm volatile("s_waitcnt vmcnt(0)" ::: "memory");
        const int tl = atomicAdd(&queue[kQTail], 1);
        int32_t *e   = &queue[kQRing + (unsigned)tl % (unsigned)batch];
        while (__hip_atomic_load(e, __ATOMIC_RELAXED, __HIP_MEMORY_SCOPE_AGENT) != 0) __builtin_amdgcn_s_sleep(4);
        __hip_atomic_store(e, item + 1, __ATOMIC_RELAXED, __HIP_MEMORY_SCOPE_AGENT);
      }
    }
    wave_sync();
    if (queue == nullptr && dq_mode != 2) break;
  }
}

__global__ void sp_gate_kernel(const int32_t *__restrict__ started)
{
  for (int spin = 0; spin < 200000; ++spin) {
    if (__hip_atomic_load(started, __ATOMIC_RELAXED, __HIP_MEMORY_SCOPE_AGENT) != 0) break;
    __builtin_amdgcn_s_sleep(32);
  }
}

constexpr int kRankBins = 4096, kRankThreads = 1024;
__global__ __launch_bounds__(kRankThreads) void sp_rank_kernel(const float *__restrict__ keys, const int batch,
                                                               int32_t *__restrict__ order2, int32_t *__restrict__ count,
                                                               const int g_lo, const int g_hi, const int lat_lo, const int lat_hi,
                                                               const int lat_max, const int stream_bit, const int pol_lo, const int pol_hi)
{
  __shared__ int hist[kRankBins];
  __shared__ int psum[kRankThreads];
  const int tid = threadIdx.x;
  auto bin_of = [](float k) { return (kRankBins - 1) - (int)(__float_as_uint(k) >> 19); };
  for (int b = tid; b < kRankBins; b += kRankThreads) hist[b] = 0;
  __syncthreads();
  for (int i = tid; i < batch; i += kRankThreads) {
    const float k = keys[i];
    if (!(k < 0.0f)) atomicAdd(&hist[bin_of(fabsf(k))], 1);
  }
  __syncthreads();
  constexpr int per = kRankBins / kRankThreads;
  int mine[per], tot = 0;
  for (int e = 0; e < per; ++e) { mine[e] = hist[tid * per + e]; tot += mine[e]; }
  psum[tid] = tot;
  __syncthreads();
  for (int d = 1; d < kRankThreads; d <<= 1) {
    const int v = (tid >= d) ? psum[tid - d] : 0;
    __syncthreads();
    psum[tid] += v;
    __syncthreads();
  }
  int start = psum[tid] - tot;
  for (int e = 0; e < per; ++e) { hist[tid * per + e] = start; start += mine[e]; }
  const int total = psum[kRankThreads - 1];
  __syncthreads();
  {
    auto lg = [](int b) { return exp2f(fminf(40.0f, fmaxf(0.0f, (float)((kRankBins - 1) - b) * (1.0f / 16.0f) - 127.0f))); };
    float part = 0.0f;
    int first  = kRankBins;
    for (int e = 0; e < per; ++e) {
      part += (float)mine[e] * lg(tid * per + e);
      if (mine[e] > 0 && first == kRankBins) first = tid * per + e;
    }
    __shared__ float fsum[kRankThreads];
    fsum[tid] = part;
    psum[tid] = first;
    __syncthreads();
    for (int d = kRankThreads / 2; d > 0; d >>= 1) {
      if (tid < d) {
        fsum[tid] += fsum[tid + d];
        psum[tid] = min(psum[tid], psum[tid + d]);
      }
      __syncthreads();
    }
    if (tid == 0) {
      const float want = (psum[0] < kRankBins) ? fsum[0] / lg(psum[0]) : 0.0f;
      const int w64 = ((int)fminf(want, 1e9f) + 32) / 64 * 64;
      const int lat = lat_hi > 0 && w64 <= lat_max;
      count[0] = total;
      count[1] = lat ? max(lat_lo, min(lat_hi, w64)) : max(g_lo, min(g_hi, w64));
      count[2] = lat;
      count[4] = total;
      count[5] = g_hi;
      count[6] = lat;
      count[8] = stream_bit;
      count[10] = (total >= 8 * max(1, lat_hi) && fsum[0] / (float)total < 100.0f) ? pol_hi : pol_lo;
    }
  }
  __syncthreads();
  for (int i = tid; i < batch; i += kRankThreads) {
    const float k = keys[i];
    if (!(k < 0.0f)) order2[atomicAdd(&hist[bin_of(fabsf(k))], 1)] = i;
  }
}

struct SparseDeviceBook {
  struct Slot {
    int bit = 0;
    hipStream_t polish = nullptr;
    hipEvent_t ev1 = nullptr, ev2 = nullptr, last = nullptr;
    int inflight = 0;
    int enqueueing = 0;
  };
  std::mutex mu;
  int dev = -1, cus = 0;
  int lat_opt_in = -1;
  std::map<size_t, int> per_cu_std, per_cu_lat;
  int32_t *active = nullptr;
  unsigned long long *busy_host = nullptr;
  const unsigned long long *busy_dev = nullptr;
  std::map<hipStream_t, Slot> slots;
  int next_bit = 0;
};

static SparseDeviceBook *sparse_book()
{
  static std::mutex mu;
  static std::map<int, SparseDeviceBook *> books;
  int dev = 0;
  if (hipGetDevice(&dev) != hipSuccess) { (void)hipGetLastError(); return nullptr; }
  std::lock_guard<std::mutex> lk(mu);
  const auto it = books.find(dev);
  if (it != books.end()) return it->second;
  auto *b = new SparseDeviceBook();
  b->dev  = dev;
  int32_t *words = nullptr;
  if (hipDeviceGetAttribute(&b->cus, hipDeviceAttributeMultiprocessorCount, dev) != hipSuccess ||
      hipMalloc(reinterpret_cast<void **>(&words), 64 * sizeof(int32_t)) != hipSuccess ||
      hipMemset(words, 0, 64 * sizeof(int32_t)) != hipSuccess) {
    (void)hipGetLastError();
    if (words) (void)hipFree(words);
    delete b;
    return nullptr;
  }
  b->active   = words;
  b->busy_dev = reinterpret_cast<const unsigned long long *>(words + 32);
  void *hostw = nullptr, *devw = nullptr;
  if (hipHostMalloc(&hostw, 64, hipHostMallocMapped) == hipSuccess && hipHostGetDevicePointer(&devw, hostw, 0) == hipSuccess) {
    b->busy_host  = static_cast<unsigned long long *>(hostw);
    *b->busy_host = 0ull;
    b->busy_dev   = static_cast<const unsigned long long *>(devw);
  } else {
    (void)hipGetLastError();
    if (hostw) (void)hipHostFree(hostw);
  }
  books[dev] = b;
  return b;
}

hipError_t sparse_device_words(int32_t **active, const unsigned long long **busy)
{
  SparseDeviceBook *b = sparse_book();
  if (b == nullptr) return hipErrorOutOfMemory;
  *active = b->active;
  *busy   = b->busy_dev;
  return hipSuccess;
}

static SparseDeviceBook::Slot &sparse_slot(SparseDeviceBook &b, hipStream_t stream)
{
  const auto it = b.slots.find(stream);
  if (it != b.slots.end()) return it->second;
  if (b.slots.size() >= 64) {
    auto sh = b.slots.begin();
    std::advance(sh, (size_t)(reinterpret_cast<uintptr_t>(stream) >> 6) % b.slots.size());
    return sh->second;
  }
  SparseDeviceBook::Slot sl;
  sl.bit = b.next_bit++ & 63;
  int least = 0, greatest = 0;
  if (hipDeviceGetStreamPriorityRange(&least, &greatest) != hipSuccess ||
      hipStreamCreateWithPriority(&sl.polish, hipStreamNonBlocking, least) != hipSuccess) {
    (void)hipGetLastError();
    sl.polish = nullptr;
  }
  if (hipEventCreateWithFlags(&sl.ev1, hipEventDisableTiming) != hipSuccess || hipEventCreateWithFlags(&sl.ev2, hipEventDisableTiming) != hipSuccess ||
      hipEventCreateWithFlags(&sl.last, hipEventDisableTiming) != hipSuccess) {
    (void)hipGetLastError();
    if (sl.polish) (void)hipStreamDestroy(sl.polish);
    sl.polish = nullptr;
    sl.ev1 = sl.ev2 = sl.last = nullptr;
  }
  return b.slots.emplace(stream, sl).first->second;
}

static SparseDeviceBook::Slot sparse_enqueue_begin(SparseDeviceBook &b, hipStream_t stream, bool *others_busy)
{
  std::lock_guard<std::mutex> lk(b.mu);
  SparseDeviceBook::Slot &mine = sparse_slot(b, stream);
  bool others = false;
  for (auto &kv : b.slots) {
    SparseDeviceBook::Slot &sl = kv.second;
    if (&sl == &mine || sl.inflight == 0) continue;
    if (sl.enqueueing > 0) {
      others = true;
      continue;
    }
    const hipError_t q = hipEventQuery(sl.last);
    if (q == hipErrorNotReady) {
      (void)hipGetLastError();
      others = true;
      continue;
    }
    (void)hipGetLastError();
    sl.inflight = 0;
    if (b.busy_host) __atomic_fetch_and(b.busy_host, ~(1ull << sl.bit), __ATOMIC_RELEASE);
  }
  if (mine.last != nullptr) {
    mine.inflight = 1;
    ++mine.enqueueing;
    if (b.busy_host) __atomic_fetch_or(b.busy_host, 1ull << mine.bit, __ATOMIC_RELEASE);
  }
  *others_busy = others;
  return mine;
}
static void sparse_enqueue_end(SparseDeviceBook &b, const SparseDeviceBook::Slot &sl, hipStream_t stream)
{
  if (sl.last == nullptr) return;
  if (hipEventRecord(sl.last, stream) != hipSuccess) (void)hipGetLastError();
  std::lock_guard<std::mutex> lk(b.mu);
  for (auto &kv : b.slots)
    if (kv.second.last == sl.last && kv.second.enqueueing > 0) --kv.second.enqueueing;
}

static bool sparse_lat_opt_in(SparseDeviceBook &b)
{
  std::lock_guard<std::mutex> lk(b.mu);
  if (b.lat_opt_in < 0) {
    b.lat_opt_in = hipFuncSetAttribute(reinterpret_cast<const void *>(qp_sparse_kernel<true>), hipFuncAttributeMaxDynamicSharedMemorySize, 80 * 1024) == hipSuccess;
    if (!b.lat_opt_in) (void)hipGetLastError();
  }
  return b.lat_opt_in == 1;
}

static int sparse_resident_blocks(SparseDeviceBook &b, size_t lds, bool lat = false)
{
  std::lock_guard<std::mutex> lk(b.mu);
  auto &cache = lat ? b.per_cu_lat : b.per_cu_std;
  const auto it = cache.find(lds);
  if (it != cache.end()) return it->second * b.cus;
  int per_cu = 0;
  const hipError_t e = lat ? hipOccupancyMaxActiveBlocksPerMultiprocessor(&per_cu, qp_sparse_kernel<true>, kWave, lds)
                           : hipOccupancyMaxActiveBlocksPerMultiprocessor(&per_cu, qp_sparse_kernel<false>, kWave, lds);
  if (e != hipSuccess) { (void)hipGetLastError(); return 0; }
  cache[lds] = per_cu;
  return per_cu * b.cus;
}

static size_t sparse_aux_queue_ints(int64_t batch) { return (size_t)batch + kQRing + kFbSlots; }
size_t qp_sparse_aux_bytes(int64_t batch) { return (sparse_aux_queue_ints(batch) + 2 * (size_t)batch + 16 + kDqRing + (size_t)batch) * sizeof(int32_t); }
int qp_sparse_fallback_slots() { return kFbSlots; }

hipError_t qp_sparse_launch(const SparsePlanDev &pl, const DenseKernelParams &kp, int64_t batch, const double *Px,
                            const double *q, const double *Ax, const double *l, const double *u, const double *wx,
                            const double *wy, double *x, double *y, double *obj, uint32_t *iter, int32_t *code,
                            double *workspace, hipStream_t stream, const int32_t *order, int32_t *aux,
                            const SparsePlanDev *fallback, double *fallback_ws, double *trace, int trace_cap, double *phase_us)
{
  if (pl.Aorig != nullptr && (fallback == nullptr || fallback_ws == nullptr || aux == nullptr)) return hipErrorInvalidValue;
  SparseDeviceBook *const book = sparse_book();
  if (book == nullptr) return hipErrorInvalidDevice;
  const bool pruned = pl.Aorig != nullptr;
  const size_t lds = (size_t)std::max(pl.lds_doubles, pruned ? fallback->lds_doubles : 0) * sizeof(double);
  const size_t wsd = qp_sparse_ws_doubles(pl);
  const char *lw        = sfb::knob("SFB_SP_LEAN_WAVES");
  const int lean_waves  = lw ? atoi(lw) : 512;
  const char *sl   = sfb::knob("SFB_SP_SLICE");
  const int slice  = sl ? atoi(sl) : 50;
  unsigned grid    = (unsigned)batch;
  int32_t *qarg    = nullptr;
  bool sliced      = false;
  if (aux != nullptr && slice > 0) {
    int resident = sparse_resident_blocks(*book, lds);
    if (const char *g = sfb::knob("SFB_SP_GRID"); g && atoi(g) > 0) resident = std::min(resident, atoi(g));
    const bool lat_ok  = pl.n <= kLatRegRows * kWave && pl.m <= kLatRegRows * kWave && lat_lds_doubles(pl.n, pl.m) * sizeof(double) <= 80 * 1024;
    const int64_t hold = lat_ok ? std::min<int64_t>(resident, 3 * (int64_t)book->cus) : resident;
    if (resident > 0 && batch > hold) {
      grid   = (unsigned)std::min<int64_t>(resident, batch);
      qarg   = aux;
      sliced = true;
    }
  }
  const char *ph    = sfb::knob("SFB_SP_PHASED");
  const bool phased = sliced && ph && atoi(ph) == 1;
  struct DoneQ { int32_t *q = nullptr; int mode = 0; hipStream_t on = nullptr; };
  auto launch = [&](unsigned g, int32_t *qa, int lw, int phases, const int32_t *ord = nullptr, uint32_t slc = 0, float *keys = nullptr,
                    const int32_t *nfresh = nullptr, int mode_sel = -1, bool lat = false, size_t lds_lat = 0, DoneQ dq = DoneQ{}) -> hipError_t {
    if ((qa != nullptr || pruned) && dq.mode != 2) {
      hipError_t e = hipMemsetAsync(aux, 0, sparse_aux_queue_ints(batch) * sizeof(int32_t), stream);
      if (e != hipSuccess) return e;
    }
    auto *kern = (trace || phase_us) ? qp_sparse_kernel<false, true>
                                     : (dq.mode == 2 ? qp_sparse_kernel<false, false, true> : (lat ? qp_sparse_kernel<true> : qp_sparse_kernel<false>));
    hipLaunchKernelGGL(kern, dim3(g), dim3(kWave), lat ? lds_lat : lds, dq.mode == 2 ? dq.on : stream, pl.self, kp, Px, q, Ax, l, u, wx, wy, x, y,
                       obj, iter, code, workspace, wsd, lw, ord, qa, (int)batch, slc ? slc : (uint32_t)std::max(1, slice),
                       pruned ? fallback->self : nullptr, fallback_ws, pruned ? qp_sparse_ws_doubles(*fallback) : 0,
                       aux ? aux + batch + kQRing : nullptr, phases, (int)std::min<int64_t>(batch, kFbSlots), keys, nfresh, mode_sel,
                       trace, trace_cap, phase_us);
    return hipGetLastError();
  };
  if (trace != nullptr || phase_us != nullptr) return launch((unsigned)batch, nullptr, lean_waves, PH_EVERYTHING, order);
  const char *pr       = sfb::knob("SFB_SP_PREDICT");
  const char *pa       = sfb::knob("SFB_SP_PAUSE");
  const unsigned pause = pa ? (unsigned)std::max(0, atoi(pa)) : 2u;
  const bool predicted = sliced && !phased && !(pr && atoi(pr) == 0) && pause > 0 && kp.stop_check_iter >= 2 && kp.max_iter > 2 * pause;
  if (predicted) {
    int32_t *xtra   = aux + sparse_aux_queue_ints(batch);
    float *keys     = reinterpret_cast<float *>(xtra);
    int32_t *order2 = xtra + batch, *count = xtra + 2 * batch;
    bool others_busy = false;
    const SparseDeviceBook::Slot slot = sparse_enqueue_begin(*book, stream, &others_busy);
    struct EnqueueEnd {
      SparseDeviceBook &bk;
      const SparseDeviceBook::Slot &sl;
      hipStream_t st;
      ~EnqueueEnd() { sparse_enqueue_end(bk, sl, st); }
    } enqueue_end{*book, slot, stream};
    hipError_t e = launch(grid, qarg, lean_waves, phases_pack(PH_SETUP, PH_FINISH, pause), order, 0, keys);
    if (e != hipSuccess) return e;
    const double stream_bytes = (double)(pl.funits + pl.bunits) * 128.0 * sizeof(double), mall = 256.0 * 1024.0 * 1024.0;
    unsigned g_lo = std::min(grid, ((unsigned)std::max(256.0, 0.70 * mall / stream_bytes) + 32u) / 64u * 64u), g_hi = grid;
    const size_t lds_lat = std::max(lds, lat_lds_doubles(pl.n, pl.m) * sizeof(double));
    int lat_hi = 0, lat_lo = 0;
    const bool lat_fits = lds_lat <= 80 * 1024 && pl.n <= kLatRegRows * kWave && pl.m <= kLatRegRows * kWave;
    if (const char *lt = sfb::knob("SFB_SP_LAT"); !(lt && atoi(lt) == 0) && lat_fits) {
      if (sparse_lat_opt_in(*book)) lat_hi = std::min<int>(sparse_resident_blocks(*book, lds_lat, true), (int)grid);
      if (const char *lw = sfb::knob("SFB_SP_LAT_WAVES"); lw && atoi(lw) > 0) lat_hi = std::min(lat_hi, atoi(lw));
      lat_lo = std::min(lat_hi, 448);
    }
    const int lat_max = 0x7FFFFFFF;
    int pol_lo = book->cus, pol_hi = 2 * book->cus;
    if (const char *pk = sfb::knob("SFB_SP_POLISHERS"); pk && atoi(pk) > 0) pol_lo = pol_hi = atoi(pk);
    pol_lo = (int)std::min<int64_t>(pol_lo, batch);
    pol_hi = (int)std::min<int64_t>(pol_hi, batch);
    hipLaunchKernelGGL(sp_rank_kernel, dim3(1), dim3(kRankThreads), 0, stream, keys, (int)batch, order2, count, (int)g_lo, (int)g_hi,
                       lat_lo, lat_hi, lat_max, slot.bit, pol_lo, pol_hi);
    if ((e = hipGetLastError()) != hipSuccess) return e;
    const uint32_t slice3 = 0x40000000u;
    if (lat_hi > 0) {
      DoneQ prod{}, cons{};
      const char *po  = sfb::knob("SFB_SP_POLISHERS");
      const int npolish = pol_hi;
      if (hipStream_t hs = (po && atoi(po) == 0) ? nullptr : slot.polish; hs != nullptr) {
        int32_t *dq = count + 16;
        if (hipMemsetAsync(dq, 0, (size_t)(kDqRing + batch) * sizeof(int32_t), stream) == hipSuccess && hipEventRecord(slot.ev1, stream) == hipSuccess) {
          const char *hp = sfb::knob("SFB_SP_LAT_HELP");
          prod = DoneQ{dq, ((hp && atoi(hp) == 0) || others_busy) ? 1 : 3, nullptr};
          cons = DoneQ{dq, 2, hs};
        }
      }
      (void)hipGetLastError();
      e = launch((unsigned)lat_hi, qarg, 0x7FFFFFFF, phases_pack(PH_ADMM, PH_ADMM, 0, prod.mode), order2, slice3, nullptr, count, 1, true, lds_lat, prod);
      if (e == hipSuccess && cons.mode == 2) {
        e = hipMemsetAsync(cons.q + kDqOver, 0xFF, sizeof(int32_t), stream);
        bool polishers_out = false;
        if (e == hipSuccess) e = hipStreamWaitEvent(cons.on, slot.ev1, 0);
        if (e == hipSuccess) {
          hipLaunchKernelGGL(sp_gate_kernel, dim3(1), dim3(1), 0, cons.on, cons.q + kDqStarted);
          e = hipGetLastError();
        }
        if (e == hipSuccess) {
          e = launch((unsigned)npolish, qarg, 0, phases_pack(PH_FINISH, PH_FINISH, 0, 2), nullptr, slice3, nullptr, nullptr, -1, false, 0, cons);
          polishers_out = e == hipSuccess;
        }
        if (e == hipSuccess) e = hipEventRecord(slot.ev2, cons.on);
        if (e == hipSuccess) e = hipStreamWaitEvent(stream, slot.ev2, 0);
        if (e != hipSuccess && polishers_out) {
          (void)hipStreamSynchronize(stream);
          (void)hipStreamSynchronize(cons.on);
        }
      }
      if (e != hipSuccess) return e;
      e = launch(grid, qarg, lean_waves, phases_pack(PH_FINISH, PH_FINISH), order2, slice3, nullptr, count + 4, 1);
      if (e != hipSuccess) return e;
    }
    return launch(g_hi, qarg, (int)std::max(512.0, mall / stream_bytes), phases_pack(PH_ADMM, PH_FINISH), order2, slice3,
                  nullptr, count, lat_hi > 0 ? 0 : -1);
  }
  if (const char *fl = sfb::knob("SFB_SP_FORCE_LAT"); !phased && fl && atoi(fl) == 1 && pl.n <= kLatRegRows * kWave && pl.m <= kLatRegRows * kWave) {
    const size_t lds_lat = std::max(lds, lat_lds_doubles(pl.n, pl.m) * sizeof(double));
    (void)hipFuncSetAttribute(reinterpret_cast<const void *>(qp_sparse_kernel<true>), hipFuncAttributeMaxDynamicSharedMemorySize, 160 * 1024);
    return launch(grid, qarg, lean_waves, PH_EVERYTHING, order, 0, nullptr, nullptr, -1, true, lds_lat);
  }
  if (!phased && !sliced) {
    const char *lt       = sfb::knob("SFB_SP_LAT");
    const size_t lds_lat = std::max(lds, lat_lds_doubles(pl.n, pl.m) * sizeof(double));
    if (!(lt && atoi(lt) == 0) && batch <= 3 * (int64_t)book->cus && lds_lat <= 80 * 1024 && pl.n <= kLatRegRows * kWave &&
        pl.m <= kLatRegRows * kWave && sparse_lat_opt_in(*book))
      return launch(grid, qarg, 0x7FFFFFFF , PH_EVERYTHING, order, 0, nullptr, nullptr, -1, true, lds_lat);
  }
  if (!phased) return launch(grid, qarg, lean_waves, PH_EVERYTHING, order);
  const double stream_bytes = (double)(pl.funits + pl.bunits) * 128.0 * sizeof(double);
  unsigned grid2 = (unsigned)std::max(256.0, 0.70 * 256.0 * 1024.0 * 1024.0 / stream_bytes);
  grid2 = std::min(grid2, grid);
  const int lean_waves2 = grid2 < grid ? 0x7FFFFFFF : lean_waves;
  hipError_t e = launch(grid, qarg, lean_waves, phases_pack(PH_SETUP, PH_SETUP), order);
  if (e != hipSuccess) return e;
  e = launch(grid2, qarg, lean_waves2, phases_pack(PH_ADMM, PH_ADMM), order);
  if (e != hipSuccess) return e;
  return launch(grid, qarg, lean_waves, phases_pack(PH_FINISH, PH_FINISH), order);
}

}
```

### smooth_feedback_amd/csrc/qp_sparse_kernel.h

```cpp
#pragma once
#include <hip/hip_runtime.h>

#include <cstdint>

#include "qp_dense_kernel.h"

namespace sfb {

#ifndef SFB_KKT_KINDS
#define SFB_KKT_KINDS
enum { K_P = 0, K_A = 1, K_SIGMA = 2, K_RHO = 3 };
#endif

struct SparsePlanDev {
  int n, m, k, nnzP, nnzA, nnzK, nnzL;
  const int32_t *Pp, *Pi, *Pcol, *Ap, *Aj, *Arow;
  const int32_t *Acp, *Aci, *Acpos, *Prp, *Prj, *Prpos, *Sp, *Sj, *Spos;
  const int32_t *perm, *pinv, *Kp, *Ki, *Kdesc, *Lp, *Li, *Rp, *Rk, *Rpos, *Rlen;
  const int32_t *fmap, *fidx, *bmap, *bidx;
  const int32_t *fmask, *bmask;
  int funits, bunits, idx_scale, ffull0, ffull1, bfull0, bfull1;
  const int32_t *Kmap, *rptr, *rtgt, *rab;
  int rsteps, maxcol;
  const int32_t *snptr, *snR, *poff, *pmap;
  int nsn, lds_doubles;
  const int32_t *f2s, *seg, *pmapL, *rsplit, *KmapL, *KdescT, *KmapT, *ztop;
  int nseg, nnzKT, nztop;
  const int32_t *ustream, *utype, *uomap;
  int units, nunits;
  int nnzA_io, nmasked;
  const int32_t *Aorig, *Amasked;
  int32_t *dev_active;
  const unsigned long long *dev_busy;
  const SparsePlanDev *self;
};

hipError_t sparse_device_words(int32_t **active, const unsigned long long **busy);

constexpr int kSweepPadDev = 16;
#ifdef __HIPCC__
#define SFB_HD __host__ __device__
#else
#define SFB_HD
#endif
SFB_HD inline size_t qp_sparse_factor_doubles(int n, int m, int nnzL, int funits, int bunits)
{
  return (size_t)nnzL + 2 * ((size_t)n + m) + 2 + (size_t)(funits + bunits + 2 * kSweepPadDev) * 128;
}
SFB_HD inline size_t qp_sparse_polish_offset(int n, int m, int nnzL, int funits, int bunits, int nnzA_compact)
{
  const size_t k   = (size_t)n + m;
  const size_t off = qp_sparse_factor_doubles(n, m, nnzL, funits, bunits) + k + 6 * (size_t)n + 11 * (size_t)m + 16 +
                     (((size_t)nnzA_compact + 1) & ~(size_t)1);
  return (off + 1) & ~(size_t)1;
}
inline size_t qp_sparse_ws_doubles(int n, int m, int nnzL, int funits, int bunits, int nnzA_compact = 0)
{
  const size_t tot = qp_sparse_polish_offset(n, m, nnzL, funits, bunits, nnzA_compact) +
                     qp_sparse_factor_doubles(n, m, nnzL, funits, bunits) + m + 4;
  return (tot + 1) & ~(size_t)1;
}

inline size_t qp_sparse_ws_doubles(const SparsePlanDev &pl)
{
  return qp_sparse_ws_doubles(pl.n, pl.m, pl.nnzL, pl.funits, pl.bunits, pl.Aorig ? pl.nnzA : 0);
}

hipError_t qp_sparse_launch(const SparsePlanDev &pl, const DenseKernelParams &kp, int64_t batch, const double *Px,
                            const double *q, const double *Ax, const double *l, const double *u, const double *wx,
                            const double *wy, double *x, double *y, double *obj, uint32_t *iter, int32_t *code,
                            double *workspace, hipStream_t stream, const int32_t *order = nullptr, int32_t *aux = nullptr,
                            const SparsePlanDev *fallback = nullptr, double *fallback_ws = nullptr,
                            double *trace = nullptr, int trace_cap = 0, double *phase_us = nullptr);
size_t qp_sparse_aux_bytes(int64_t batch);
int qp_sparse_fallback_slots();

}
```

### smooth_feedback_amd/csrc/sparse_plan.cpp

```cpp
#include "knobs.h"
#include "sparse_plan.h"

#include <algorithm>
#include <cstdio>
#include <cstdlib>
#include <iterator>
#include <array>
#include <numeric>
#include <tuple>

namespace sfb {

namespace {

void transpose_pattern(int nouter, int ninner, const std::vector<int32_t> &outer_ptr,
                       const std::vector<int32_t> &inner, std::vector<int32_t> &tp, std::vector<int32_t> &ti,
                       std::vector<int32_t> &tpos)
{
  const int nnz = outer_ptr[nouter];
  tp.assign(ninner + 1, 0);
  ti.resize(nnz);
  tpos.resize(nnz);
  for (int p = 0; p < nnz; ++p) tp[inner[p] + 1]++;
  for (int i = 0; i < ninner; ++i) tp[i + 1] += tp[i];
  std::vector<int32_t> fill(ninner, 0);
  for (int o = 0; o < nouter; ++o)
    for (int p = outer_ptr[o]; p < outer_ptr[o + 1]; ++p) {
      const int i       = inner[p];
      ti[tp[i] + fill[i]]   = o;
      tpos[tp[i] + fill[i]] = p;
      fill[i]++;
    }
}

struct UnitPlacer {
  struct S { int32_t tgt, piv; };
  int lanes = 0;
  std::vector<S> sl;
  std::vector<int> where;

  int capacity(int wg) const
  {
    const int l0 = (wg & 3) * 16;
    return std::max(0, std::min(lanes, l0 + 16) - l0);
  }
  std::vector<int> pid;
  std::vector<int> pbank;
  int np = 0;
  template<int NBANK>
  struct Banks {
    int n[NBANK], hist[130], mx;
    void clear() { std::fill(n, n + NBANK, 0); std::fill(hist, hist + 130, 0); hist[0] = NBANK; mx = 0; }
    void inc(int b) { hist[n[b]]--; hist[++n[b]]++; if (n[b] > mx) mx = n[b]; }
    void dec(int b) { hist[n[b]]--; hist[--n[b]]++; while (mx > 0 && hist[mx] == 0) --mx; }
  };
  Banks<32> tc[4], pb[4];
  Banks<16> wc[8];
  std::vector<int> pc[4];
  void reset()
  {
    for (auto &b : tc) b.clear();
    for (auto &b : pb) b.clear();
    for (auto &b : wc) b.clear();
    for (auto &v : pc) v.assign((size_t)np, 0);
  }
  void add(int e, int g, int d)
  {
    const int r = g >> 1;
    int &n = pc[r][pid[e]];
    if (d > 0) {
      tc[r].inc(sl[e].tgt & 31);
      wc[g].inc(sl[e].tgt & 15);
      if (n++ == 0) pb[r].inc(pbank[pid[e]]);
    } else {
      tc[r].dec(sl[e].tgt & 31);
      wc[g].dec(sl[e].tgt & 15);
      if (--n == 0) pb[r].dec(pbank[pid[e]]);
    }
  }
  int rcost(int r) const { return tc[r].mx + pb[r].mx; }
  int wcost(int g) const { return wc[g].mx; }
  int cost_of(int g, int h) const
  {
    int c = wcost(g) + wcost(h) + rcost(g >> 1);
    if ((h >> 1) != (g >> 1)) c += rcost(h >> 1);
    return c;
  }
  int total() const
  {
    int c = 0;
    for (int g = 0; g < 8; ++g) c += wcost(g);
    for (int r = 0; r < 4; ++r) c += rcost(r);
    return c;
  }
  bool bad(int e, int g) const
  {
    const int r = g >> 1;
    const int t = tc[r].n[sl[e].tgt & 31], w = wc[g].n[sl[e].tgt & 15], p = pb[r].n[pbank[pid[e]]];
    return (t > 1 && t == tc[r].mx) || (w > 1 && w == wc[g].mx) || (p > 1 && p == pb[r].mx);
  }
  std::pair<int, int> place(const int search)
  {
    const int c = (int)sl.size();
    pid.assign((size_t)c, 0);
    pbank.clear();
    {
      std::vector<std::pair<int32_t, int>> pv;
      for (int e = 0; e < c; ++e) pv.emplace_back(sl[e].piv, e);
      std::sort(pv.begin(), pv.end());
      np = 0;
      for (int i = 0; i < c; ++i) {
        if (i == 0 || pv[i].first != pv[i - 1].first) { pbank.push_back(pv[i].first & 31); ++np; }
        pid[pv[i].second] = np - 1;
      }
    }
    std::vector<int> grp((size_t)c);
    reset();
    for (int e = 0; e < c; ++e) {
      const int lane = e % lanes, half = e / lanes;
      grp[e] = half * 4 + (lane >> 4);
      add(e, grp[e], +1);
    }
    const int before = total();
    std::vector<int> natural(grp);
    std::vector<int> cnt((size_t)np, 0), order((size_t)c), fill(8, 0);
    for (int e = 0; e < c; ++e) cnt[pid[e]]++;
    std::iota(order.begin(), order.end(), 0);
    std::stable_sort(order.begin(), order.end(), [&](int x, int y) {
      if (cnt[pid[x]] != cnt[pid[y]]) return cnt[pid[x]] > cnt[pid[y]];
      if (pid[x] != pid[y]) return pid[x] < pid[y];
      return sl[x].tgt < sl[y].tgt;
    });
    reset();
    for (int e : order) {
      int bg = -1;
      long bs = 0;
      for (int g = 0; g < 8; ++g) {
        if (fill[g] >= capacity(g)) continue;
        const int r = g >> 1;
        const bool has = pc[r][pid[e]] > 0;
        const int col = tc[r].n[sl[e].tgt & 31] + wc[g].n[sl[e].tgt & 15] + (has ? 0 : pb[r].n[pbank[pid[e]]]);
        const long score = 1000L * col + (has ? 0 : 100) + fill[g];
        if (bg < 0 || score < bs) { bg = g; bs = score; }
      }
      grp[e] = bg;
      fill[bg]++;
      add(e, bg, +1);
    }
    int nrg = 0, nwg = 0;
    for (int g = 0; g < 8; ++g) nwg += capacity(g) > 0;
    for (int r = 0; r < 4; ++r) nrg += capacity(2 * r) > 0;
    for (int pass = 0; pass < search && total() > 2 * nrg + nwg; ++pass) {
      bool improved = false;
// ... 202 lines not shown
    for (int r = 0; r < k; ++r) {
      flag[r] = r;
      for (int p = rp[r]; p < rp[r + 1]; ++p)
        for (int i = rj[p]; flag[i] != r; i = parent[i]) {
          if (parent[i] == -1) parent[i] = r;
          lnz[i]++;
          flag[i] = r;
        }
    }
  }
  o.nnzK = (int)pe.size();
  o.Kp.assign(k + 1, 0); o.Ki.resize(o.nnzK); o.Kkind.resize(o.nnzK); o.Kidx.resize(o.nnzK);
  for (int t = 0; t < o.nnzK; ++t) {
    o.Kp[pe[t].j + 1]++;
    o.Ki[t] = pe[t].i; o.Kkind[t] = pe[t].kind; o.Kidx[t] = pe[t].idx;
  }
  for (int j = 0; j < k; ++j) o.Kp[j + 1] += o.Kp[j];
  o.Lp.assign(k + 1, 0);
  for (int j = 0; j < k; ++j) o.Lp[j + 1] = o.Lp[j] + lnz[j];
  o.nnzL = o.Lp[k];
  o.Li.resize(o.nnzL);
  {
    std::vector<int32_t> fill(k, 0);
    std::fill(flag.begin(), flag.end(), -1);
    for (int r = 0; r < k; ++r) {
      flag[r] = r;
      for (int p = rp[r]; p < rp[r + 1]; ++p)
        for (int i = rj[p]; flag[i] != r; i = parent[i]) {
          o.Li[o.Lp[i] + fill[i]++] = r;
          flag[i] = r;
        }
    }
  }
  transpose_pattern(k, k, o.Lp, o.Li, o.Rp, o.Rk, o.Rpos);
  o.Rlen.resize(o.nnzL);
  for (int t = 0; t < o.nnzL; ++t) o.Rlen[t] = o.Lp[o.Rk[t] + 1] - o.Rpos[t];

  std::vector<int32_t> rankF(k), parF(k, -1);
  {
    std::vector<int32_t> head(k, -1), next(k, -1), stack;
    for (int j = k - 1; j >= 0; --j)
      if (parent[j] >= 0) { next[j] = head[parent[j]]; head[parent[j]] = j; }
    o.f2s.clear();
    o.f2s.reserve(k);
    for (int r = 0; r < k; ++r) {
      if (parent[r] >= 0) continue;
      stack.push_back(r);
      while (!stack.empty()) {
        const int v = stack.back(), c = head[v];
        if (c >= 0) { head[v] = next[c]; stack.push_back(c); }
        else { rankF[v] = (int32_t)o.f2s.size(); o.f2s.push_back(v); stack.pop_back(); }
      }
    }
    for (int j = 0; j < k; ++j)
      if (parent[j] >= 0) parF[rankF[j]] = rankF[parent[j]];
  }
  std::vector<int32_t> FLp(k + 1, 0), FLi(o.nnzL), posF(o.nnzL);
  {
    std::vector<std::pair<int32_t, int32_t>> tmp;
    for (int jF = 0; jF < k; ++jF) {
      const int jS = o.f2s[jF];
      tmp.clear();
      for (int p = o.Lp[jS]; p < o.Lp[jS + 1]; ++p) tmp.emplace_back(rankF[o.Li[p]], p);
      std::sort(tmp.begin(), tmp.end());
      FLp[jF + 1] = FLp[jF] + (int)tmp.size();
      for (size_t e = 0; e < tmp.size(); ++e) {
        if (tmp[e].first <= jF) { *msg = "internal: postorder does not keep ancestors behind"; return false; }
        FLi[FLp[jF] + e]   = tmp[e].first;
        posF[tmp[e].second] = FLp[jF] + (int)e;
      }
    }
  }
  std::vector<int32_t> FKp(k + 1, 0), FKi(o.nnzK), FKkind(o.nnzK), FKidx(o.nnzK);
  {
    std::vector<std::array<int32_t, 4>> fe;
    fe.reserve(o.nnzK);
    for (int jS = 0; jS < k; ++jS)
      for (int p = o.Kp[jS]; p < o.Kp[jS + 1]; ++p) fe.push_back({rankF[jS], rankF[o.Ki[p]], o.Kkind[p], o.Kidx[p]});
    std::sort(fe.begin(), fe.end());
    for (int t = 0; t < o.nnzK; ++t) {
      if (fe[t][1] < fe[t][0]) { *msg = "internal: KKT entry above the diagonal in the factorisation numbering"; return false; }
      FKp[fe[t][0] + 1]++;
      FKi[t] = fe[t][1]; FKkind[t] = fe[t][2]; FKidx[t] = fe[t][3];
    }
    for (int j = 0; j < k; ++j) FKp[j + 1] += FKp[j];
  }

  {
    auto pos_in_col = [&](int col, int row) {
      const int32_t *b = FLi.data() + FLp[col], *e = FLi.data() + FLp[col + 1];
      const int32_t *it = std::lower_bound(b, e, row);
      return (it != e && *it == row) ? (int)(it - FLi.data()) : -1;
    };
    o.Kmap.resize(o.nnzK);
    for (int j = 0; j < k; ++j)
      for (int p = FKp[j]; p < FKp[j + 1]; ++p) {
        const int i = FKi[p];
        o.Kmap[p]   = (i == j) ? o.nnzL + j : pos_in_col(j, i);
        if (o.Kmap[p] < 0) { *msg = "internal: KKT entry outside the pattern of L"; return false; }
      }
    o.maxcol = 0;
    for (int kk = 0; kk < k; ++kk) o.maxcol = std::max(o.maxcol, FLp[kk + 1] - FLp[kk]);
    if (o.maxcol >= (1 << 16)) { *msg = "column of L too long for the update encoding"; return false; }
    constexpr int kLdsTarget = 2048, kLdsSmall = 1536;
    const int lds_floor = std::max(k + 2, 2 * o.maxcol + 4);
    const int lds_small = lds_hint > 0 ? std::max(lds_floor, lds_hint)
                                       : (std::max(lds_floor, std::min(o.nnzL + k + 3, kLdsSmall)) + 63) / 64 * 64;
    const int lds_large = std::max(lds_small, lds_hint > 0 ? lds_hint : kLdsTarget);
    o.lds_doubles = lds_small;

    std::vector<int32_t> fdesc(k);
    for (int j = 0; j < k; ++j) fdesc[j] = j;
    for (int j = 0; j < k; ++j)
      if (parF[j] >= 0) fdesc[parF[j]] = std::min(fdesc[parF[j]], fdesc[j]);
    std::vector<int32_t> maxR1(k);
    for (int j = 0; j < k; ++j) maxR1[j] = 1 + FLp[j + 1] - FLp[j];
    for (int j = 0; j < k; ++j)
      if (parF[j] >= 0) maxR1[parF[j]] = std::max(maxR1[parF[j]], maxR1[j]);
    struct Seg { int c0, c1, lds, nL, accN, sn0, sn1, nout, omap0; };
    std::vector<Seg> segs;
    auto choose_segments = [&](const bool units) {
      segs.clear();
      constexpr int kMinCols = 8;
      std::vector<char> in_lds(k, 0);
      for (int j = k - 1; j >= 0;) {
        const int c0 = fdesc[j], nc = j - c0 + 1, nL = FLp[j + 1] - FLp[c0];
        const int reserve = std::max(2 * maxR1[j], 384);
        const int ccj = FLp[j + 1] - FLp[j];
        const bool fits = units ? nL + nc + ccj * (ccj + 1) / 2 + 3 <= o.lds_doubles
                                : (maxR1[j] <= 64 && nL + nc + 2 + reserve <= o.lds_doubles);
        if (nc >= kMinCols && fits) {
          for (int c = c0; c <= j; ++c) in_lds[c] = 1;
          j = c0 - 1;
        } else {
          --j;
        }
      }
      for (int c = 0; c < k;) {
        int e = c + 1;
        if (in_lds[c]) {
          while (e < k && in_lds[e] && fdesc[e] >= c) ++e;
          int root = e - 1;
          while (fdesc[root] != c) --root;
          e = root + 1;
          segs.push_back({c, e, 1, FLp[e] - FLp[c], FLp[e] - FLp[c] + (e - c), 0, 0, 0, 0});
        } else {
          while (e < k && !in_lds[e]) ++e;
          segs.push_back({c, e, 0, 0, 0, 0, 0, 0, 0});
        }
        c = e;
      }
    };

    o.units = 0;
    o.ustream.clear(); o.utype.clear(); o.uomap.clear();
    {
      const char *uk = sfb::knob("SFB_PLAN_UNITS");
      bool ok = false;
      for (int attempt = 0; attempt < 2 && !ok; ++attempt) {
      if (attempt == 1 && lds_large == lds_small) break;
      o.lds_doubles = attempt == 0 ? lds_small : lds_large;
      ok = !(uk && uk[0] == '0') && (size_t)o.lds_doubles * 8 < (1u << 16);
      if (ok) {
        choose_segments(true);
        std::vector<Seg> cut;
        std::vector<int32_t> seen(o.nnzL + k, -1), percol(k + 1, 0);
        for (const Seg &sg : segs) {
          if (sg.lds) { cut.push_back(sg); continue; }
          int c0 = sg.c0;
          while (c0 < sg.c1 && ok) {
            int own = 0, nout = 0, best = -1;
            std::vector<int32_t> touched;
            for (int j = c0; j < sg.c1; ++j) {
              own += FLp[j + 1] - FLp[j] + 1;
              nout -= percol[j];
              for (int bp = FLp[j]; bp < FLp[j + 1]; ++bp)
                for (int ap = bp; ap < FLp[j + 1]; ++ap) {
                  const int b = FLi[bp], a = FLi[ap];
                  const int g = (a == b) ? o.nnzL + b : pos_in_col(b, a);
                  if (g < 0) { *msg = "internal: update outside the pattern of L"; return false; }
                  if (seen[g] != c0) { seen[g] = c0; touched.push_back(g); percol[b]++; ++nout; }
                }
              if (own + nout + 3 <= o.lds_doubles) best = j + 1;
              else if (best >= 0) break;
              else if (j == c0) break;
            }
            for (int g : touched) seen[g] = -1;
            std::fill(percol.begin(), percol.end(), 0);
            if (best < 0) { ok = false; break; }
            cut.push_back({c0, best, 0, 0, 0, 0, 0, 0, 0});
            c0 = best;
          }
        }
        if (ok) segs.swap(cut);
      }
      }
      if (ok) {
        struct Op { int32_t t, a, b, d; };
        std::vector<int32_t> outidx(o.nnzL + k, -1);
        for (Seg &sg : segs) {
          const int c0 = sg.c0, c1 = sg.c1;
          sg.nL   = FLp[c1] - FLp[c0];
          sg.accN = sg.nL + (c1 - c0);
          sg.omap0 = (int)o.uomap.size();
          sg.sn0   = (int)o.utype.size();
          int nout = 0;
          auto off_of = [&](int g) {
            if (g < o.nnzL) { if (g >= FLp[c0] && g < FLp[c1]) return g - FLp[c0]; }
            else if (g - o.nnzL >= c0 && g - o.nnzL < c1) return sg.nL + (g - o.nnzL - c0);
            if (outidx[g] < 0) { outidx[g] = nout++; o.uomap.push_back(g); }
            return sg.accN + outidx[g];
          };
          std::vector<Op> ops;
          std::vector<std::array<int32_t, 3>> deps;
          std::vector<int32_t> dm_of(sg.nL, -1);
          std::vector<int32_t> writer;
          for (int j = c0; j < c1; ++j) {
            const int dOff = sg.nL + (j - c0);
            if ((int)writer.size() < sg.accN) writer.resize(sg.accN, -1);
            for (int p = FLp[j]; p < FLp[j + 1]; ++p) {
              const int tOff = p - FLp[c0];
              deps.push_back({writer[tOff], writer[dOff], -1});
              dm_of[tOff] = (int)ops.size();
              writer[tOff] = (int)ops.size();
              ops.push_back({tOff, -1, -1, dOff});
            }
            for (int bp = FLp[j]; bp < FLp[j + 1]; ++bp)
              for (int ap = bp; ap < FLp[j + 1]; ++ap) {
                const int b = FLi[bp], a = FLi[ap];
                const int g = (a == b) ? o.nnzL + b : pos_in_col(b, a);
                if (g < 0) { *msg = "internal: update outside the pattern of L"; return false; }
                const int T = off_of(g);
                if ((int)writer.size() <= T) writer.resize(T + 1, -1);
                deps.push_back({dm_of[ap - FLp[c0]], dm_of[bp - FLp[c0]], writer[T]});
                writer[T] = (int)ops.size();
                ops.push_back({T, ap - FLp[c0], bp - FLp[c0], dOff});
              }
          }
          for (int e = sg.omap0; e < (int)o.uomap.size(); ++e) outidx[o.uomap[e]] = -1;
          sg.nout = nout;
          if (sg.accN + nout + 3 > o.lds_doubles) { *msg = "internal: segment does not fit the LDS"; return false; }
          const int SINK = sg.accN + nout, ZEROL = SINK + 1, ONE = SINK + 2;
          const int nops = (int)ops.size();
          std::vector<int32_t> nsucc(nops + 1, 0), succ, height(nops, 1), npred(nops, 0);
          for (int i = 0; i < nops; ++i)
            for (int d : deps[i])
              if (d >= 0) { nsucc[d + 1]++; npred[i]++; }
          for (int i = 0; i < nops; ++i) nsucc[i + 1] += nsucc[i];
          succ.resize(nsucc[nops]);
          {
            std::vector<int32_t> fill(nops, 0);
            for (int i = 0; i < nops; ++i)
              for (int d : deps[i])
                if (d >= 0) succ[nsucc[d] + fill[d]++] = i;
          }
          for (int i = nops - 1; i >= 0; --i)
            for (int d : deps[i])
              if (d >= 0) height[d] = std::max(height[d], height[i] + 1);
          std::vector<std::pair<int32_t, int32_t>> ready[2];
          for (int i = 0; i < nops; ++i)
            if (npred[i] == 0) ready[ops[i].a < 0].emplace_back(height[i], -i);
          for (auto &h : ready) std::make_heap(h.begin(), h.end());
          int done = 0;
          std::vector<int32_t> cur, arriving;
          while (done < nops) {
            int kind;
            if (ready[0].empty()) kind = 1;
            else if (ready[1].empty()) kind = 0;
            else kind = ready[1].front().first >= ready[0].front().first;
            cur.clear();
            arriving.clear();
            while ((int)cur.size() < 128 && !ready[kind].empty()) {
              std::pop_heap(ready[kind].begin(), ready[kind].end());
              cur.push_back(-ready[kind].back().second);
              ready[kind].pop_back();
            }
            done += (int)cur.size();
            const size_t base = o.ustream.size();
            o.ustream.resize(base + 256);
            o.utype.push_back(kind);
            for (int e = 0; e < 128; ++e) {
              const int lane = e % 64, half = e / 64;
              int32_t w0, w1;
              if (e < (int)cur.size()) {
                const Op &op = ops[cur[e]];
                if (kind) { w0 = (op.t * 8) | ((op.d * 8) << 16); w1 = -1; }
                else { w0 = (op.t * 8) | ((op.a * 8) << 16); w1 = (op.b * 8) | ((op.d * 8) << 16); }
              } else if (kind) { w0 = (SINK * 8) | ((ONE * 8) << 16); w1 = -1; }
              else { w0 = (SINK * 8) | ((ZEROL * 8) << 16); w1 = (ZEROL * 8) | ((ZEROL * 8) << 16); }
              o.ustream[base + (size_t)lane * 4 + 2 * half]     = w0;
              o.ustream[base + (size_t)lane * 4 + 2 * half + 1] = w1;
            }
            for (int i : cur)
              for (int q = nsucc[i]; q < nsucc[i + 1]; ++q)
                if (--npred[succ[q]] == 0) arriving.push_back(succ[q]);
            for (int i : arriving) {
              auto &h = ready[ops[i].a < 0];
              h.emplace_back(height[i], -i);
              std::push_heap(h.begin(), h.end());
            }
          }
          sg.sn1 = (int)o.utype.size();
        }
        o.units  = 1;
        o.nunits = (int)o.utype.size();
        o.ustream.resize(o.ustream.size() + (size_t)256 * 2 * SparsePlanHost::kSweepPad, 0);
        o.utype.resize(o.utype.size() + SparsePlanHost::kSweepPad + 32, 0);
        o.uomap.resize(o.uomap.size() + 64 * 8, o.nnzL + k);
      } else {
        o.ustream.clear(); o.utype.clear(); o.uomap.clear();
        o.lds_doubles = lds_large;
        choose_segments(false);
      }
    }

    constexpr int kRelax = 4, kMaxWidth = 16;
    const int ZERO = o.nnzL + k + 1, SCRATCH = o.nnzL + k;
    o.snptr.clear(); o.snR.clear(); o.poff.clear(); o.pmap.clear(); o.pmapL.clear(); o.rptr.clear(); o.rsplit.clear();
    o.rtgt.clear(); o.rab.clear();
    o.rptr.push_back(0);
    for (Seg &sg : segs) {
      if (o.units) break;
      sg.sn0 = (int)o.snptr.size();
      const int scratch = sg.lds ? o.lds_doubles - ((sg.accN + 2 + 1) & ~1) : o.lds_doubles;
      auto lds_off = [&](int g) {
        if (g == SCRATCH) return sg.accN;
        if (g == ZERO) return sg.accN + 1;
        if (g < o.nnzL) return (g >= FLp[sg.c0] && g < FLp[sg.c1]) ? g - FLp[sg.c0] : -1;
        const int j = g - o.nnzL;
        return (j >= sg.c0 && j < sg.c1) ? sg.nL + (j - sg.c0) : -1;
      };
      int j0 = sg.c0;
      while (j0 < sg.c1) {
        std::vector<int32_t> U(FLi.begin() + FLp[j0], FLi.begin() + FLp[j0 + 1]);
        int w = 1;
        while (j0 + w < sg.c1 && w < kMaxWidth) {
          const int jn = j0 + w;
          std::vector<int32_t> Un;
          std::set_union(U.begin(), U.end(), FLi.begin() + FLp[jn], FLi.begin() + FLp[jn + 1], std::back_inserter(Un));
          Un.erase(std::remove_if(Un.begin(), Un.end(), [&](int32_t r) { return r <= jn; }), Un.end());
          const int Rn = (w + 1) + (int)Un.size();
          if (2 * (w + 1) * Rn > scratch) break;
          if (sg.lds && Rn > 64) break;
          int ubase = 0;
          for (int32_t r : U) ubase += (r != jn);
          const int base = std::max(ubase, FLp[jn + 1] - FLp[jn]);
          if ((int)Un.size() - base > kRelax) break;
          U.swap(Un);
          ++w;
        }
        const int nu = (int)U.size(), R = w + nu;
        if (2 * w * R > scratch) { *msg = "internal: panel does not fit the LDS scratch"; return false; }
        o.snptr.push_back(j0);
        o.snR.push_back(R);
        o.poff.push_back((int)o.pmap.size());
        for (int jj = 0; jj < w; ++jj)
          for (int r = 0; r < R; ++r) {
            int src = SCRATCH;
            if (r == jj) src = o.nnzL + j0 + jj;
            else if (r > jj) {
              const int g = (r < w) ? j0 + r : U[r - w];
              const int pos = pos_in_col(j0 + jj, g);
              src = (pos >= 0) ? pos : ZERO;
            }
            o.pmap.push_back(src);
            o.pmapL.push_back(sg.lds ? lds_off(src) : 0);
            if (sg.lds && o.pmapL.back() < 0) { *msg = "internal: panel entry outside its LDS segment"; return false; }
          }
        std::vector<std::array<int32_t, 2>> slots[2];
        for (int bq = 0; bq < nu; ++bq)
          for (int aq = bq; aq < nu; ++aq) {
            const int rb = U[bq], ra = U[aq];
            int tgt;
            if (aq == bq) tgt = o.nnzL + rb;
            else {
              tgt = pos_in_col(rb, ra);
              if (tgt < 0) continue;
            }
            bool touched = false;
            for (int jj = 0; jj < w && !touched; ++jj)
              touched = pos_in_col(j0 + jj, ra) >= 0 && pos_in_col(j0 + jj, rb) >= 0;
            if (!touched) continue;
            const int off = sg.lds ? lds_off(tgt) : -1;
            if (off >= 0) slots[0].push_back({off, aq | (bq << 16)});
            else slots[1].push_back({tgt, aq | (bq << 16)});
          }
        int total = 0;
        for (int part = 0; part < 2; ++part) {
          const int steps = (int)((slots[part].size() + 63) / 64);
          const size_t q0 = o.rtgt.size();
          o.rtgt.resize(q0 + (size_t)steps * 64, part == 0 ? sg.accN : SCRATCH);
          o.rab.resize(q0 + (size_t)steps * 64, 0);
          for (size_t e = 0; e < slots[part].size(); ++e) { o.rtgt[q0 + e] = slots[part][e][0]; o.rab[q0 + e] = slots[part][e][1]; }
          total += steps;
          if (part == 0) o.rsplit.push_back(o.rptr.back() + steps);
        }
        o.rptr.push_back(o.rptr.back() + total);
        j0 += w;
      }
      sg.sn1 = (int)o.snptr.size();
    }
    o.nsn = (int)o.snptr.size();
    o.nseg = (int)segs.size();
    o.seg.clear();
    for (const Seg &sg : segs)
      for (int v : {sg.sn0, sg.sn1, sg.c0, sg.c1, sg.lds, sg.nL, sg.accN, (int)FKp[sg.c0], (int)FKp[sg.c1], (int)FLp[sg.c0], sg.nout, sg.omap0})
        o.seg.push_back(v);
    static_assert(SparsePlanHost::kSegStride == 12, "segment table layout");
    std::vector<char> col_lds(k, 0);
    for (const Seg &sg : segs)
      if (sg.lds) std::fill(col_lds.begin() + sg.c0, col_lds.begin() + sg.c1, 1);
    o.Kdesc.assign((size_t)(o.nnzK + 64 * 8) * 4, 0);
    o.KmapL.assign((size_t)o.nnzK + 64 * 8, 0);
    o.KdescT.clear(); o.KmapT.clear();
    {
      size_t si = 0;
      for (int j = 0; j < k; ++j) {
        while (segs[si].c1 <= j) ++si;
        const Seg &sg = segs[si];
        for (int p = FKp[j]; p < FKp[j + 1]; ++p) {
          const int kind = FKkind[p], idx = FKidx[p];
          int r = 0, c = 0;
          if (kind == K_P) { r = o.Pi[idx]; c = o.Pcol[idx]; }
          else if (kind == K_A) { r = o.Arow[idx]; c = o.Aj[idx]; }
          const int32_t d4[4] = {kind, idx, r, c};
          std::copy(d4, d4 + 4, o.Kdesc.begin() + 4 * (size_t)p);
          if (sg.lds) {
            const int g = o.Kmap[p];
            o.KmapL[p]  = (g < o.nnzL) ? g - FLp[sg.c0] : sg.nL + (g - o.nnzL - sg.c0);
          } else {
            o.KdescT.insert(o.KdescT.end(), d4, d4 + 4);
            o.KmapT.push_back(o.Kmap[p]);
          }
        }
      }
    }
    o.nnzKT = (int)o.KmapT.size();
    for (int pad = 0; pad < 64 * 8; ++pad) {
      const int32_t d4[4] = {K_SIGMA, 0, 0, 0};
      o.KdescT.insert(o.KdescT.end(), d4, d4 + 4);
      o.KmapT.push_back(SCRATCH);
    }
    for (size_t p = o.nnzK; p < (size_t)o.nnzK + 64 * 8; ++p) o.Kdesc[4 * p] = K_SIGMA;
    o.Kmap.resize((size_t)o.nnzK + 64 * 8, SCRATCH);
    o.ztop.clear();
    for (const Seg &sg : segs)
      if (!sg.lds) {
        o.ztop.push_back(FLp[sg.c0]); o.ztop.push_back(FLp[sg.c1] - FLp[sg.c0]);
        o.ztop.push_back(o.nnzL + sg.c0); o.ztop.push_back(sg.c1 - sg.c0);
      }
    o.ztop.push_back(SCRATCH); o.ztop.push_back(2);
    o.nztop = (int)o.ztop.size() / 2;
    if (const char *dbg = sfb::knob("SFB_PLAN_DEBUG"); dbg && dbg[0] == '1') {
      int maxR = 0, over64 = 0, nlds = 0, cols_lds = 0;
      long long panel = 0, acc_lds = 0, ext = 0, internal = 0;
      for (const Seg &sg : segs) {
        nlds += sg.lds; cols_lds += sg.lds ? sg.c1 - sg.c0 : 0; acc_lds += sg.lds ? sg.accN : 0;
        fprintf(stderr, "[sfb plan] segment columns %d..%d %s accumulators %d supernodes %d\n", sg.c0, sg.c1 - 1, sg.lds ? "LDS" : "top",
                sg.lds ? sg.accN : FLp[sg.c1] - FLp[sg.c0] + sg.c1 - sg.c0, sg.sn1 - sg.sn0);
      }
      for (int sn = 0; sn < o.nsn; ++sn) {
        const int w = (sn + 1 < o.nsn ? o.snptr[sn + 1] : k) - o.snptr[sn], R = o.snR[sn];
        maxR = std::max(maxR, R);
        over64 += R > 64;
        panel += (long long)w * R;
        internal += o.rsplit[sn] - o.rptr[sn];
        ext += o.rptr[sn + 1] - o.rsplit[sn];
      }
      if (o.units) {
        int nf = 0, nd = 0, maxw = 0;
        for (int u = 0; u < o.nunits; ++u) (o.utype[u] ? nd : nf)++;
        for (const Seg &sg : segs) maxw = std::max(maxw, sg.accN + sg.nout + 3);
        fprintf(stderr, "[sfb plan] unit engine: %d units (%d update + %d division), %d segments, largest working set %d of %d doubles\n",
                o.nunits, nf, nd, (int)segs.size(), maxw, o.lds_doubles);
      }
      fprintf(stderr, "[sfb plan] %d supernodes, max R %d, %d with R > 64, panel entries %lld, trailing steps %d on chip + %d in HBM; "
              "%d segments, %d on chip with %d columns and %lld accumulators of %d; lds_doubles %d\n", o.nsn, maxR, over64, panel,
              (int)internal, (int)ext, (int)segs.size(), nlds, cols_lds, acc_lds, o.nnzL + k, o.lds_doubles);
    }
    o.snptr.push_back(k);
    o.poff.push_back((int)o.pmap.size());
    o.rsplit.push_back(o.rptr.back());
    o.rsteps = o.rptr.back();
    for (int pad = 0; pad < 64 * SparsePlanHost::kSweepPad; ++pad) {
      o.pmap.push_back(SCRATCH);
      o.pmapL.push_back(0);
      o.rtgt.push_back(SCRATCH);
      o.rab.push_back(0);
    }
  }
  auto acc_of = [&](int posS) { return posF[posS]; };

  if (k + 1 >= (1 << 16)) { *msg = "n+m too large for the packed sweep encoding (max 65534)"; return false; }
  o.idx_scale = ((k + 1) * 8 < (1 << 16)) ? 8 : 1;
  auto build = [&](bool forward, std::vector<int32_t> &xmap, std::vector<int32_t> &xidx, int &units,
                   std::vector<int32_t> &xmask, int &full0, int &full1) {
    const int cap = 128;
    struct Slot { int32_t pos, tgt, piv; };
    std::vector<Slot> sl;
    sl.reserve(o.nnzL);
    std::vector<int32_t> col_first(k + 1, 0);
    for (int t = 0; t < k; ++t) {
      const int j = forward ? t : k - 1 - t;
      col_first[t] = (int32_t)sl.size();
      const int p0 = forward ? o.Lp[j] : o.Rp[j], p1 = forward ? o.Lp[j + 1] : o.Rp[j + 1];
      for (int p = p0; p < p1; ++p) sl.push_back({forward ? p : o.Rpos[p], forward ? o.Li[p] : o.Rk[p], j});
    }
    col_first[k] = (int32_t)sl.size();
    const int ns = (int)sl.size();
    auto tof = [&](int j) { return forward ? j : k - 1 - j; };
    std::vector<int32_t> prev_same(ns, -1), next_same(ns, -1), last_upd(k, -1);
    for (int q = 0; q < ns; ++q) {
      const int tg = sl[q].tgt;
      if (last_upd[tg] >= 0) { prev_same[q] = last_upd[tg]; next_same[last_upd[tg]] = q; }
      last_upd[tg] = q;
    }
    std::vector<int32_t> height(ns, 1), colh(k, 0);
    for (int q = ns - 1; q >= 0; --q) {
      int h = 0;
      if (next_same[q] >= 0) h = height[next_same[q]];
      else h = std::max(h, (int)colh[sl[q].tgt]);
      height[q] = h + 1;
      colh[sl[q].piv] = std::max(colh[sl[q].piv], height[q]);
    }
    std::vector<int32_t> npred(ns, 0);
    for (int q = 0; q < ns; ++q) npred[q] = (prev_same[q] >= 0 ? 1 : 0) + (last_upd[sl[q].piv] >= 0 ? 1 : 0);
    std::vector<std::vector<std::array<int32_t, 3>>> slots;
    std::vector<std::pair<int32_t, int32_t>> heap;
    std::vector<int32_t> arriving;
    for (int q = 0; q < ns; ++q)
      if (npred[q] == 0) heap.emplace_back(height[q], -q);
    std::make_heap(heap.begin(), heap.end());
    int done = 0;
    while (done < ns) {
      slots.emplace_back();
      arriving.clear();
      for (int c = 0; c < cap && !heap.empty(); ++c) {
        std::pop_heap(heap.begin(), heap.end());
        const int q = -heap.back().second;
        heap.pop_back();
        slots.back().push_back({sl[q].pos, sl[q].tgt, sl[q].piv});
        ++done;
        if (next_same[q] >= 0) {
          if (--npred[next_same[q]] == 0) arriving.push_back(next_same[q]);
        } else {
          const int tt = tof(sl[q].tgt);
          for (int r = col_first[tt]; r < col_first[tt + 1]; ++r)
            if (--npred[r] == 0) arriving.push_back(r);
        }
      }
      for (int q : arriving) {
        heap.emplace_back(height[q], -q);
        std::push_heap(heap.begin(), heap.end());
      }
    }
    const int steps = (int)slots.size();
    if (const char *dbg = sfb::knob("SFB_PLAN_DEBUG"); dbg && dbg[0] == '1') {
      fprintf(stderr, "[sfb plan] %s sweep: %d units, slots per unit:", forward ? "forward" : "backward", steps);
      for (int s = 0; s < steps; ++s) fprintf(stderr, " %d", (int)slots[s].size());
      fprintf(stderr, "\n");
    }
    units           = steps;
    units = ((units + 7) / 8) * 8;
    const size_t total = (size_t)(units + SparsePlanHost::kSweepPad) * 128;
    xmap.assign(total, -1);
    const int sc = o.idx_scale;
    xidx.assign(total, (k * sc) | ((k * sc) << 16));
    xmask.assign((size_t)units + 2 * SparsePlanHost::kSweepPad, 63);
    constexpr bool bank_aware = true;
    long cyc_before = 0, cyc_after = 0;
    UnitPlacer up;
    const int search_passes = ns <= 20000 ? 1 : 0;
    for (int s = 0; s < steps; ++s) {
      const int lanes = std::max(1, ((int)slots[s].size() + 1) / 2);
      xmask[s]        = 64 - lanes;
      up.lanes = lanes;
      up.sl.clear();
      for (const auto &e : slots[s]) up.sl.push_back({e[1], e[2]});
      const auto cyc = up.place(search_passes);
      cyc_before += cyc.first;
      cyc_after += bank_aware ? cyc.second : cyc.first;
      for (size_t e = 0; e < slots[s].size(); ++e) {
        const int pos  = bank_aware ? up.where[e] : (int)((e % (size_t)lanes) * 2 + e / (size_t)lanes);
        const size_t q = (size_t)s * 128 + (size_t)pos;
        xmap[q] = acc_of(slots[s][e][0]);
        xidx[q] = (slots[s][e][1] * sc) | ((slots[s][e][2] * sc) << 16);
      }
    }
    if (const char *dbg = sfb::knob("SFB_PLAN_DEBUG"); dbg && dbg[0] == '1')
      fprintf(stderr, "[sfb plan] %s sweep: modelled LDS cycles of the slot accesses per sweep: natural placement %ld, bank-aware %ld (floor %d)\n",
              forward ? "forward" : "backward", cyc_before, cyc_after, 16 * steps);
    full0 = full1 = 0;
    for (int s = 0; s < steps;) {
      if ((int)slots[s].size() != cap) { ++s; continue; }
      int e = s;
      while (e < steps && (int)slots[e].size() == cap) ++e;
      const int a = ((s + 7) / 8) * 8, b = (e / 8) * 8;
      if (b - a > full1 - full0) { full0 = a; full1 = b; }
      s = e;
    }
  };
  build(true, o.fmap, o.fidx, o.funits, o.fmask, o.ffull0, o.ffull1);
  build(false, o.bmap, o.bidx, o.bunits, o.bmask, o.bfull0, o.bfull1);

  return true;
}

}
```

### smooth_feedback_amd/csrc/sparse_plan.h

```cpp
#pragma once
#include <cstdint>
#include <vector>

namespace sfb {

#ifndef SFB_KKT_KINDS
#define SFB_KKT_KINDS
enum { K_P = 0, K_A = 1, K_SIGMA = 2, K_RHO = 3 };
#endif

struct SparsePlanHost {
  int n = 0, m = 0, k = 0, nnzP = 0, nnzA = 0, nnzK = 0, nnzL = 0;
  std::vector<int32_t> Pp, Pi, Pcol;
  std::vector<int32_t> Ap, Aj, Arow;
  std::vector<int32_t> Acp, Aci, Acpos;
  std::vector<int32_t> Prp, Prj, Prpos;
  std::vector<int32_t> Sp, Sj, Spos;
  std::vector<int32_t> perm, pinv;
  std::vector<int32_t> Kp, Ki, Kkind, Kidx;
  std::vector<int32_t> Lp, Li;
  std::vector<int32_t> Rp, Rk, Rpos;
  std::vector<int32_t> Rlen;
  static constexpr int kSweepPad = 16;
  std::vector<int32_t> fmap, fidx, bmap, bidx, fmask, bmask;
  int funits = 0, bunits = 0, idx_scale = 1, ffull0 = 0, ffull1 = 0, bfull0 = 0, bfull1 = 0;
  std::vector<int32_t> Kmap, rptr, rtgt, rab, snptr, snR, poff, pmap;
  std::vector<int32_t> Kdesc;
  int rsteps = 0, maxcol = 0, nsn = 0, lds_doubles = 0;
  std::vector<int32_t> f2s;
  static constexpr int kSegStride = 12;
  std::vector<int32_t> seg, pmapL, rsplit, KmapL, KdescT, KmapT, ztop;
  int nseg = 0, nnzKT = 0, nztop = 0;
  std::vector<int32_t> ustream, utype, uomap;
  int units = 0, nunits = 0;
};

bool build_sparse_plan(int n, int m, const int32_t *Pp, const int32_t *Pi, const int32_t *Ap, const int32_t *Aj,
                       int ordering, const int32_t *user_perm, const int32_t *stage, SparsePlanHost &out,
                       const char **msg, int lds_hint = 0);

}
```

Measured before the change: 215,800.

## Build extra LDS-wide unit schedules and select per launch by dynamic LDS size

```diff
diff --git a/smooth_feedback_amd/csrc/capi_sparse.hip b/smooth_feedback_amd/csrc/capi_sparse.hip
--- a/smooth_feedback_amd/csrc/capi_sparse.hip
+++ b/smooth_feedback_amd/csrc/capi_sparse.hip
@@ -48,12 +48,17 @@
                        int nnzA_io, int32_t **blob_out, sfb::SparsePlanDev &d)
 {
   static const std::vector<int32_t> none;
+  static const sfb::SparsePlanHost::UnitSchedule nowide;
+  const sfb::SparsePlanHost::UnitSchedule &w0 = h.wide.size() > 0 ? h.wide[0] : nowide, &w1 = h.wide.size() > 1 ? h.wide[1] : nowide;
   const std::vector<int32_t> *arrs[] = {&h.Pp, &h.Pi, &h.Pcol, &h.Ap, &h.Aj, &h.Arow, &h.Acp, &h.Aci, &h.Acpos,
                                         &h.Prp, &h.Prj, &h.Prpos, &h.Sp, &h.Sj, &h.Spos, &h.perm, &h.pinv,
                                         &h.Kp, &h.Ki, &h.Kdesc, &h.Lp, &h.Li, &h.Rp, &h.Rk, &h.Rpos, &h.Rlen,
                                         &h.fmap, &h.fidx, &h.bmap, &h.bidx, &h.Kmap, &h.rptr, &h.rtgt, &h.rab, &h.snptr, &h.snR, &h.poff, &h.pmap, &h.fmask, &h.bmask,
                                         &h.f2s, &h.seg, &h.pmapL, &h.rsplit, &h.KmapL, &h.KdescT, &h.KmapT, &h.ztop, &h.ustream, &h.utype, &h.uomap,
-                                        Aorig ? Aorig : &none, Amasked ? Amasked : &none};
+                                        Aorig ? Aorig : &none, Amasked ? Amasked : &none,
+                                        &w0.seg, &w0.ustream, &w0.uomap, &w0.KmapL, &w0.KdescT, &w0.KmapT, &w0.ztop,
+                                        &w1.seg, &w1.ustream, &w1.uomap, &w1.KmapL, &w1.KdescT, &w1.KmapT, &w1.ztop};
+  static_assert(sfb::SparsePlanHost::kMaxWide == 2 && sfb::SparsePlanDev::kMaxSched == 3, "wide schedules of the upload");
   constexpr int NA = sizeof(arrs) / sizeof(arrs[0]);
   size_t off[NA + 1];
   off[0] = 0;
@@ -75,9 +80,20 @@
                             &d.Kp, &d.Ki, &d.Kdesc, &d.Lp, &d.Li, &d.Rp, &d.Rk, &d.Rpos, &d.Rlen,
                             &d.fmap, &d.fidx, &d.bmap, &d.bidx, &d.Kmap, &d.rptr, &d.rtgt, &d.rab, &d.snptr, &d.snR, &d.poff, &d.pmap, &d.fmask, &d.bmask,
                             &d.f2s, &d.seg, &d.pmapL, &d.rsplit, &d.KmapL, &d.KdescT, &d.KmapT, &d.ztop, &d.ustream, &d.utype, &d.uomap,
-                            &d.Aorig, &d.Amasked};
+                            &d.Aorig, &d.Amasked,
+                            &d.us[1].seg, &d.us[1].ustream, &d.us[1].uomap, &d.us[1].KmapL, &d.us[1].KdescT, &d.us[1].KmapT, &d.us[1].ztop,
+                            &d.us[2].seg, &d.us[2].ustream, &d.us[2].uomap, &d.us[2].KmapL, &d.us[2].KdescT, &d.us[2].KmapT, &d.us[2].ztop};
+  static_assert(sizeof(ptrs) == sizeof(arrs), "one device pointer per uploaded array");
   d.funits = h.funits; d.bunits = h.bunits; d.ffull0 = h.ffull0; d.ffull1 = h.ffull1; d.bfull0 = h.bfull0; d.bfull1 = h.bfull1; d.idx_scale = h.idx_scale; d.rsteps = h.rsteps; d.maxcol = h.maxcol; d.nsn = h.nsn; d.lds_doubles = h.lds_doubles; d.nseg = h.nseg; d.nnzKT = h.nnzKT; d.nztop = h.nztop; d.units = h.units; d.nunits = h.nunits;
   for (int a = 0; a < NA; ++a) *ptrs[a] = dblob + off[a];
+  d.us[0] = {d.seg, d.ustream, d.uomap, d.KmapL, d.KdescT, d.KmapT, d.ztop, h.nseg, h.nnzKT, h.nztop, h.lds_doubles};
+  d.nsched = 1 + (int)h.wide.size();
+  for (int i = 0; i < sfb::SparsePlanHost::kMaxWide; ++i) {
+    sfb::SparsePlanDev::UnitSched &u = d.us[1 + i];
+    const bool on = i < (int)h.wide.size();
+    u.nseg = on ? h.wide[i].nseg : 0; u.nnzKT = on ? h.wide[i].nnzKT : 0; u.nztop = on ? h.wide[i].nztop : 0;
+    u.lds_doubles = on ? h.wide[i].lds_doubles : 0;
+  }
   d.nnzA_io = nnzA_io;
   d.nmasked = Amasked ? (int)Amasked->size() - 512 : 0;
   if (!Aorig) d.Aorig = d.Amasked = nullptr;
diff --git a/smooth_feedback_amd/csrc/knobs.cpp b/smooth_feedback_amd/csrc/knobs.cpp
--- a/smooth_feedback_amd/csrc/knobs.cpp
+++ b/smooth_feedback_amd/csrc/knobs.cpp
@@ -13,7 +13,7 @@
 namespace {
 const char *const kKnobs[] = {"SFB_SP_GRID",  "SFB_SP_SLICE",  "SFB_SP_PAUSE",      "SFB_SP_PREDICT",   "SFB_SP_LAT",
                               "SFB_SP_FORCE_LAT", "SFB_SP_LAT_WAVES", "SFB_SP_POLISHERS", "SFB_SP_LAT_HELP", "SFB_SP_PHASED", "SFB_SP_LEAN_WAVES", "SFB_MID_GRID", "SFB_MID_SLICE",
-                              "SFB_QP4_MAX_WAVES", "SFB_QP_DENSE_BIG", "SFB_EKF_PERSISTENT", "SFB_PLAN_UNITS", "SFB_PLAN_DEBUG", "SFB_MPC_TIMING"};
+                              "SFB_QP4_MAX_WAVES", "SFB_QP_DENSE_BIG", "SFB_EKF_PERSISTENT", "SFB_PLAN_UNITS", "SFB_PLAN_WIDE", "SFB_PLAN_DEBUG", "SFB_MPC_TIMING"};
 std::mutex g_mu;
 std::atomic<int> g_set{0};
 std::map<std::string, const char *> &table()
diff --git a/smooth_feedback_amd/csrc/qp_sparse.hip b/smooth_feedback_amd/csrc/qp_sparse.hip
--- a/smooth_feedback_amd/csrc/qp_sparse.hip
+++ b/smooth_feedback_amd/csrc/qp_sparse.hip
@@ -13,6 +13,7 @@
 #include "knobs.h"
 #include "../../include/sfb.h"
 #include "qp_sparse_kernel.h"
+#include "sparse_lds.h"
 #include "wave_util.h"
 
 #ifndef SFB_SWEEP_ASM
@@ -43,6 +44,7 @@
 {
   return ph0 | (ph1 << 4) | (int)((pause_at & 0xFFFFFu) << 8) | (dq_mode << 28);
 }
+constexpr int phases_sched(int phases, int sched) { return (int)(((uint32_t)phases & 0x3FFFFFFFu) | ((uint32_t)sched << 30)); }
 constexpr int PH_EVERYTHING = phases_pack(PH_SETUP, PH_FINISH);
 constexpr unsigned long long kFactorStamp = 0x5FB0FAC7A11CE5EDull;
 
@@ -264,9 +266,10 @@
 typedef int vint4u __attribute__((ext_vector_type(4)));
 template<int DEPTH>
 __device__ inline int ldl_numeric_units(const SparsePlanDev &pl, const Item &it, const Ws &w, double *t, const int mode,
-                                        const double c, const double sigma, const double delta, const int lane,
+                                        const double c, const double sigma, const double delta, const int lane, const int sched,
                                         unsigned long long *fill_ticks = nullptr)
 {
+  const SparsePlanDev::UnitSched &S = pl.us[uni(min(sched, uni(pl.nsched) - 1))];
   unsigned long long fclk = fill_ticks ? wall_clock64() : 0ull;
   auto fill_lap = [&](const bool is_fill) {
     if (fill_ticks) {
@@ -283,29 +286,29 @@
 #define SFB_ULAP(i)
 #endif
   double *ACC = w.Lx;
-  for (int z = 0, nz = uni(pl.nztop); z < nz; ++z) {
-    const int z0 = uni(pl.ztop[2 * z]), zn = uni(pl.ztop[2 * z + 1]);
+  for (int z = 0, nz = uni(S.nztop); z < nz; ++z) {
+    const int z0 = uni(S.ztop[2 * z]), zn = uni(S.ztop[2 * z + 1]);
     for (int p = lane; p < zn; p += kWave) ACC[z0 + p] = 0.0;
   }
   wave_sync();
-  kkt_fill<4>(pl.KdescT, pl.KmapT, 0, uni(pl.nnzKT), it, w, ACC, mode, c, sigma, delta, lane);
+  kkt_fill<4>(S.KdescT, S.KmapT, 0, uni(S.nnzKT), it, w, ACC, mode, c, sigma, delta, lane);
   wave_sync();
   SFB_ULAP(0)
   fill_lap(true);
-  const vint4u *__restrict__ stream = reinterpret_cast<const vint4u *>(pl.ustream);
+  const vint4u *__restrict__ stream = reinterpret_cast<const vint4u *>(S.ustream);
   auto at = [&](const unsigned off) -> double & { return *reinterpret_cast<double *>(reinterpret_cast<char *>(t) + off); };
   bool zero_pivot = false;
   constexpr int UB = SFB_COPY_UB;
-  for (int sg = 0, nseg = uni(pl.nseg); sg < nseg; ++sg) {
-    const int32_t *sgp = pl.seg + 12 * sg;
+  for (int sg = 0, nseg = uni(S.nseg); sg < nseg; ++sg) {
+    const int32_t *sgp = S.seg + 12 * sg;
     const int u0 = uni(sgp[0]), u1 = uni(sgp[1]), c0 = uni(sgp[2]), c1 = uni(sgp[3]), closed = uni(sgp[4]), nLs = uni(sgp[5]);
     const int accN = uni(sgp[6]), kp0 = uni(sgp[7]), kp1 = uni(sgp[8]), gL = uni(sgp[9]), nout = uni(sgp[10]);
-    const int32_t *__restrict__ omap = pl.uomap + uni(sgp[11]);
+    const int32_t *__restrict__ omap = S.uomap + uni(sgp[11]);
     const int sink = accN + nout;
     if (closed) {
       for (int e = lane; e < accN; e += kWave) t[e] = 0.0;
       wave_lds_fence();
-      kkt_fill<4>(pl.Kdesc, pl.KmapL, kp0, kp1, it, w, t, mode, c, sigma, delta, lane);
+      kkt_fill<4>(pl.Kdesc, S.KmapL, kp0, kp1, it, w, t, mode, c, sigma, delta, lane);
     } else {
       for (int e0 = lane; e0 < accN; e0 += kWave * UB) {
         double v[UB];
@@ -404,10 +407,10 @@
 
 template<int DEPTH>
 __device__ inline int ldl_numeric_dev(const SparsePlanDev &pl, const Item &it, const Ws &w, double *t, const int mode,
-                                      const double c, const double sigma, const double delta, const int lane,
+                                      const double c, const double sigma, const double delta, const int lane, const int sched,
                                       unsigned long long *fill_ticks = nullptr)
 {
-  if (uni(pl.units)) return ldl_numeric_units<DEPTH>(pl, it, w, t, mode, c, sigma, delta, lane, fill_ticks);
+  if (uni(pl.units)) return ldl_numeric_units<DEPTH>(pl, it, w, t, mode, c, sigma, delta, lane, sched, fill_ticks);
   unsigned long long fclk = fill_ticks ? wall_clock64() : 0ull;
   auto fill_lap = [&](const bool is_fill) {
     if (fill_ticks) {
@@ -956,11 +959,6 @@
   sweep(pl.bidx, uni(pl.bunits), w.LxB, pl.bmask, uni(pl.bfull0), uni(pl.bfull1));
 }
 
-constexpr int kLatRegRows = 12;
-__host__ __device__ constexpr size_t lat_lds_doubles(const int n, const int m)
-{
-  return (size_t)(((n + m + 2) + 1) & ~1) + n + 2 * (size_t)m + (n + m) + 8 + (2 * kLatRegRows * 64) / 4 + (kLatRegRows * 64) / 8 + 4;
-}
 constexpr int kLatResident = (256 - kAgprFree) / 4;
 __device__ __forceinline__ bool lat_resident_ok(const SparsePlanDev &pl) { return uni(pl.funits) >= kLatResident + 16; }
 __device__ __forceinline__ void lat_resident_load(const double *LxF, const int lane)
@@ -1412,7 +1410,7 @@
 
 template<int SD, bool WIDE = false>
 __device__ inline void sp_polish(const SparsePlanDev &pl, const Item &it, const Ws &w, const Ws &wf, const DenseKernelParams &kp,
-                                 double *t, const double c, const int lane, const bool lean)
+                                 double *t, const double c, const int lane, const bool lean, const int sched)
 {
   const int n = uni(pl.n), m = uni(pl.m), k = uni(pl.k);
   const double inf = INFINITY, eps = DBL_EPSILON;
@@ -1425,7 +1423,7 @@
   }
   for (int e = lane; e < k; e += kWave) w.tv[e] = 0.0;
   wave_sync();
-  if (!ldl_numeric_dev<8>(pl, it, wf, t, 1, c, kp.sigma, kp.delta, lane)) return;
+  if (!ldl_numeric_dev<8>(pl, it, wf, t, 1, c, kp.sigma, kp.delta, lane, sched)) return;
   for (uint32_t iter = 0; iter != kp.polish_iter; ++iter) {
 #ifndef SFB_POLISH_RB
 #define SFB_POLISH_RB 2
@@ -1560,6 +1558,7 @@
   };
   if constexpr (TRACE) ph_clk = wall_clock64();
   const int ph0 = phases & 15, ph1 = (phases >> 4) & 15;
+  const int sched = (int)((uint32_t)phases >> 30);
   const uint32_t pause_at = ((uint32_t)phases >> 8) & 0xFFFFFu;
   const int n = uni(pl.n), m = uni(pl.m), k = uni(pl.k);
   const int nnzP = uni(pl.nnzP), nnzA = uni(pl.nnzA);
@@ -1775,7 +1774,7 @@
   phase_lap(0);
   if (!keep_factor) {
     if (lane == 0) w.hdr[kHdrStamp] = 0.0;
-    if (!ldl_numeric_dev<8>(pl, it, w, t, 0, c, kp.sigma, kp.delta, lane, TRACE ? &ph_fill : nullptr)) {
+    if (!ldl_numeric_dev<8>(pl, it, w, t, 0, c, kp.sigma, kp.delta, lane, sched, TRACE ? &ph_fill : nullptr)) {
       ret_code = SFB_QP_UNKNOWN;
     } else if (lane == 0 && allow_reuse) {
       w.hdr[kHdrStamp]   = __longlong_as_double((long long)kFactorStamp);
@@ -2326,10 +2325,10 @@
       const Ws wp = polish_ws(w, gws + slot * ws_doubles,
                               qp_sparse_polish_offset(n, m, uni(pl.nnzL), uni(pl.funits), uni(pl.bunits), pl.Aorig ? nnzA : 0), n, m,
                               uni(pl.nnzL), uni(pl.funits), uni(pl.bunits));
-      sp_polish<SFB_SWEEP_DEPTH, WIDE>(pl, it, w, wp, kp, t, c, lane, lean);
+      sp_polish<SFB_SWEEP_DEPTH, WIDE>(pl, it, w, wp, kp, t, c, lane, lean, sched);
     } else {
       if (lane == 0) w.hdr[kHdrStamp] = 0.0;
-      sp_polish<SFB_SWEEP_DEPTH, WIDE>(pl, it, w, w, kp, t, c, lane, lean);
+      sp_polish<SFB_SWEEP_DEPTH, WIDE>(pl, it, w, w, kp, t, c, lane, lean, sched);
     }
   }
 
@@ -2441,7 +2440,7 @@
   for (bool first = true;; first = false) {
     int item = -1, resume = 0;
     if constexpr (dq_mode == 2) {
-      if (first && (int)blockIdx.x >= __builtin_amdgcn_readfirstlane((fbflags + kFbSlots + 2 * batch)[10])) return;
+      if (first && (int)gridDim.x != __builtin_amdgcn_readfirstlane((fbflags + kFbSlots + 2 * batch)[10])) return;
       if (lane == 0) {
         int32_t *const doneq = fbflags + kFbSlots + 2 * batch + 16;
         for (;;) {
@@ -2531,10 +2530,10 @@
     const int st = sp_solve_item<LAT, TRACE, LAT || POLISHER>(*use, kp, gPx, gq, gAx, gl, gu, gwx, gwy, gx, gy, gobj, giter, gcode, wsb, wsd, lean_waves_item,
                                  lean, (size_t)item, slot, t, lane, resume != 0, fbslot >= 0 ? nullptr : queue, nfresh, slice,
                                   fbslot < 0 && slot == (size_t)item,
-                                 fbslot >= 0 ? PH_EVERYTHING : (helper ? (PH_FINISH | (PH_FINISH << 4)) : phases), keys ? keys + item : nullptr, trace,
+                                 fbslot >= 0 ? PH_EVERYTHING : (helper ? phases_sched(PH_FINISH | (PH_FINISH << 4), (int)((uint32_t)phases >> 30)) : phases), keys ? keys + item : nullptr, trace,
                                  trace_cap, phase_us);
     if (keys != nullptr && st != SP_PAUSED && lane == 0) keys[item] = -1.0f;
-    if (fbslot >= 0 && phases != PH_EVERYTHING && lane == 0)
+    if (fbslot >= 0 && phases_sched(phases, 0) != PH_EVERYTHING && lane == 0)
       carve_ws(gws + (size_t)item * ws_doubles, uni(plp->n), uni(plp->m), uni(plp->nnzL), uni(plp->funits), uni(plp->bunits)).hdr[kHdrComplete] = 1.0;
     if ((dq_mode == 2 || helper) && lane == 0)
       carve_ws(gws + (size_t)item * ws_doubles, uni(plp->n), uni(plp->m), uni(plp->nnzL), uni(plp->funits), uni(plp->bunits)).hdr[kHdrComplete] = 1.0;
@@ -2835,6 +2834,12 @@
   }
   const char *ph    = sfb::knob("SFB_SP_PHASED");
   const bool phased = sliced && ph && atoi(ph) == 1;
+  auto sched_for = [&](const size_t bytes) {
+    int s = 0;
+    for (int i = 1; i < pl.nsched; ++i)
+      if ((size_t)pl.us[i].lds_doubles * sizeof(double) <= bytes) s = i;
+    return s;
+  };
   struct DoneQ { int32_t *q = nullptr; int mode = 0; hipStream_t on = nullptr; };
   auto launch = [&](unsigned g, int32_t *qa, int lw, int phases, const int32_t *ord = nullptr, uint32_t slc = 0, float *keys = nullptr,
                     const int32_t *nfresh = nullptr, int mode_sel = -1, bool lat = false, size_t lds_lat = 0, DoneQ dq = DoneQ{}) -> hipError_t {
@@ -2844,10 +2849,11 @@
     }
     auto *kern = (trace || phase_us) ? qp_sparse_kernel<false, true>
                                      : (dq.mode == 2 ? qp_sparse_kernel<false, false, true> : (lat ? qp_sparse_kernel<true> : qp_sparse_kernel<false>));
-    hipLaunchKernelGGL(kern, dim3(g), dim3(kWave), lat ? lds_lat : lds, dq.mode == 2 ? dq.on : stream, pl.self, kp, Px, q, Ax, l, u, wx, wy, x, y,
+    const size_t dyn = (lat || lds_lat > lds) ? lds_lat : lds;
+    hipLaunchKernelGGL(kern, dim3(g), dim3(kWave), dyn, dq.mode == 2 ? dq.on : stream, pl.self, kp, Px, q, Ax, l, u, wx, wy, x, y,
                        obj, iter, code, workspace, wsd, lw, ord, qa, (int)batch, slc ? slc : (uint32_t)std::max(1, slice),
                        pruned ? fallback->self : nullptr, fallback_ws, pruned ? qp_sparse_ws_doubles(*fallback) : 0,
-                       aux ? aux + batch + kQRing : nullptr, phases, (int)std::min<int64_t>(batch, kFbSlots), keys, nfresh, mode_sel,
+                       aux ? aux + batch + kQRing : nullptr, phases_sched(phases, sched_for(dyn)), (int)std::min<int64_t>(batch, kFbSlots), keys, nfresh, mode_sel,
                        trace, trace_cap, phase_us);
     return hipGetLastError();
   };
@@ -2892,7 +2898,6 @@
     if (lat_hi > 0) {
       DoneQ prod{}, cons{};
       const char *po  = sfb::knob("SFB_SP_POLISHERS");
-      const int npolish = pol_hi;
       if (hipStream_t hs = (po && atoi(po) == 0) ? nullptr : slot.polish; hs != nullptr) {
         int32_t *dq = count + 16;
         if (hipMemsetAsync(dq, 0, (size_t)(kDqRing + batch) * sizeof(int32_t), stream) == hipSuccess && hipEventRecord(slot.ev1, stream) == hipSuccess) {
@@ -2911,9 +2916,12 @@
           hipLaunchKernelGGL(sp_gate_kernel, dim3(1), dim3(1), 0, cons.on, cons.q + kDqStarted);
           e = hipGetLastError();
         }
-        if (e == hipSuccess) {
-          e = launch((unsigned)npolish, qarg, 0, phases_pack(PH_FINISH, PH_FINISH, 0, 2), nullptr, slice3, nullptr, nullptr, -1, false, 0, cons);
-          polishers_out = e == hipSuccess;
+        const size_t lds_pol = std::max(lds, polisher_wide_lds_doubles(pl.n, pl.m) * sizeof(double));
+        for (int i = 0; i < (pol_hi == pol_lo ? 1 : 2) && e == hipSuccess; ++i) {
+          const int np = i == 0 ? pol_lo : pol_hi;
+          e = launch((unsigned)np, qarg, 0, phases_pack(PH_FINISH, PH_FINISH, 0, 2), nullptr, slice3, nullptr, nullptr, -1, false,
+                     np <= book->cus ? lds_pol : 0, cons);
+          polishers_out = polishers_out || e == hipSuccess;
         }
         if (e == hipSuccess) e = hipEventRecord(slot.ev2, cons.on);
         if (e == hipSuccess) e = hipStreamWaitEvent(stream, slot.ev2, 0);
diff --git a/smooth_feedback_amd/csrc/qp_sparse_kernel.h b/smooth_feedback_amd/csrc/qp_sparse_kernel.h
--- a/smooth_feedback_amd/csrc/qp_sparse_kernel.h
+++ b/smooth_feedback_amd/csrc/qp_sparse_kernel.h
@@ -28,6 +28,13 @@
   int nseg, nnzKT, nztop;
   const int32_t *ustream, *utype, *uomap;
   int units, nunits;
+  struct UnitSched {
+    const int32_t *seg, *ustream, *uomap, *KmapL, *KdescT, *KmapT, *ztop;
+    int nseg, nnzKT, nztop, lds_doubles;
+  };
+  static constexpr int kMaxSched = 3;
+  UnitSched us[kMaxSched];
+  int nsched;
   int nnzA_io, nmasked;
   const int32_t *Aorig, *Amasked;
   int32_t *dev_active;
diff --git a/smooth_feedback_amd/csrc/sparse_lds.h b/smooth_feedback_amd/csrc/sparse_lds.h
--- /dev/null
+++ b/smooth_feedback_amd/csrc/sparse_lds.h
@@ -0,0 +1,28 @@
+#pragma once
+#include <cstddef>
+
+#ifdef __HIPCC__
+#define SFB_LDS_HD __host__ __device__
+#else
+#define SFB_LDS_HD
+#endif
+
+namespace sfb {
+
+constexpr int kLatRegRows = 12;
+SFB_LDS_HD constexpr size_t lat_lds_doubles(const int n, const int m)
+{
+  return (size_t)(((n + m + 2) + 1) & ~1) + n + 2 * (size_t)m + (n + m) + 8 + (2 * kLatRegRows * 64) / 4 + (kLatRegRows * 64) / 8 + 4;
+}
+SFB_LDS_HD constexpr bool lat_form_fits(const int n, const int m)
+{
+  return n <= kLatRegRows * 64 && m <= kLatRegRows * 64 && lat_lds_doubles(n, m) * sizeof(double) <= 80 * 1024;
+}
+constexpr size_t kLdsPerCu = 160 * 1024, kLdsGranule = 1280;
+SFB_LDS_HD constexpr size_t polisher_wide_lds_doubles(const int n, const int m)
+{
+  const size_t lat = (lat_lds_doubles(n, m) * sizeof(double) + kLdsGranule - 1) / kLdsGranule * kLdsGranule;
+  return lat_form_fits(n, m) && 3 * lat < kLdsPerCu ? (kLdsPerCu - 3 * lat) / sizeof(double) / 64 * 64 : 0;
+}
+
+}
diff --git a/smooth_feedback_amd/csrc/sparse_plan.cpp b/smooth_feedback_amd/csrc/sparse_plan.cpp
--- a/smooth_feedback_amd/csrc/sparse_plan.cpp
+++ b/smooth_feedback_amd/csrc/sparse_plan.cpp
@@ -1,4 +1,5 @@
 #include "knobs.h"
+#include "sparse_lds.h"
 #include "sparse_plan.h"
 
 #include <algorithm>
@@ -507,16 +508,11 @@
       }
     };
 
-    o.units = 0;
-    o.ustream.clear(); o.utype.clear(); o.uomap.clear();
-    {
-      const char *uk = sfb::knob("SFB_PLAN_UNITS");
-      bool ok = false;
-      for (int attempt = 0; attempt < 2 && !ok; ++attempt) {
-      if (attempt == 1 && lds_large == lds_small) break;
-      o.lds_doubles = attempt == 0 ? lds_small : lds_large;
-      ok = !(uk && uk[0] == '0') && (size_t)o.lds_doubles * 8 < (1u << 16);
-      if (ok) {
+    auto unit_engine = [&]() -> int {
+      o.ustream.clear(); o.utype.clear(); o.uomap.clear();
+      if ((size_t)o.lds_doubles * 8 >= (1u << 16)) return 0;
+      bool ok = true;
+      {
         choose_segments(true);
         std::vector<Seg> cut;
         std::vector<int32_t> seen(o.nnzL + k, -1), percol(k + 1, 0);
@@ -533,7 +529,7 @@
                 for (int ap = bp; ap < FLp[j + 1]; ++ap) {
                   const int b = FLi[bp], a = FLi[ap];
                   const int g = (a == b) ? o.nnzL + b : pos_in_col(b, a);
-                  if (g < 0) { *msg = "internal: update outside the pattern of L"; return false; }
+                  if (g < 0) { *msg = "internal: update outside the pattern of L"; return -1; }
                   if (seen[g] != c0) { seen[g] = c0; touched.push_back(g); percol[b]++; ++nout; }
                 }
               if (own + nout + 3 <= o.lds_doubles) best = j + 1;
@@ -547,10 +543,10 @@
             c0 = best;
           }
         }
-        if (ok) segs.swap(cut);
-      }
-      }
-      if (ok) {
+        if (!ok) return 0;
+        segs.swap(cut);
+      }
+      {
         struct Op { int32_t t, a, b, d; };
         std::vector<int32_t> outidx(o.nnzL + k, -1);
         for (Seg &sg : segs) {
@@ -584,7 +580,7 @@
               for (int ap = bp; ap < FLp[j + 1]; ++ap) {
                 const int b = FLi[bp], a = FLi[ap];
                 const int g = (a == b) ? o.nnzL + b : pos_in_col(b, a);
-                if (g < 0) { *msg = "internal: update outside the pattern of L"; return false; }
+                if (g < 0) { *msg = "internal: update outside the pattern of L"; return -1; }
                 const int T = off_of(g);
                 if ((int)writer.size() <= T) writer.resize(T + 1, -1);
                 deps.push_back({dm_of[ap - FLp[c0]], dm_of[bp - FLp[c0]], writer[T]});
@@ -594,7 +590,7 @@
           }
           for (int e = sg.omap0; e < (int)o.uomap.size(); ++e) outidx[o.uomap[e]] = -1;
           sg.nout = nout;
-          if (sg.accN + nout + 3 > o.lds_doubles) { *msg = "internal: segment does not fit the LDS"; return false; }
+          if (sg.accN + nout + 3 > o.lds_doubles) { *msg = "internal: segment does not fit the LDS"; return -1; }
           const int SINK = sg.accN + nout, ZEROL = SINK + 1, ONE = SINK + 2;
           const int nops = (int)ops.size();
           std::vector<int32_t> nsucc(nops + 1, 0), succ, height(nops, 1), npred(nops, 0);
@@ -657,11 +653,24 @@
           }
           sg.sn1 = (int)o.utype.size();
         }
-        o.units  = 1;
         o.nunits = (int)o.utype.size();
         o.ustream.resize(o.ustream.size() + (size_t)256 * 2 * SparsePlanHost::kSweepPad, 0);
         o.utype.resize(o.utype.size() + SparsePlanHost::kSweepPad + 32, 0);
         o.uomap.resize(o.uomap.size() + 64 * 8, o.nnzL + k);
+      }
+      return 1;
+    };
+    o.units = 0;
+    {
+      const char *uk = sfb::knob("SFB_PLAN_UNITS");
+      int got = 0;
+      for (int attempt = 0; attempt < 2 && got == 0 && !(uk && uk[0] == '0'); ++attempt) {
+        if (attempt == 1 && lds_large == lds_small) break;
+        o.lds_doubles = attempt == 0 ? lds_small : lds_large;
+        if ((got = unit_engine()) < 0) return false;
+      }
+      if (got == 1) {
+        o.units = 1;
       } else {
         o.ustream.clear(); o.utype.clear(); o.uomap.clear();
         o.lds_doubles = lds_large;
@@ -756,56 +765,59 @@
       sg.sn1 = (int)o.snptr.size();
     }
     o.nsn = (int)o.snptr.size();
-    o.nseg = (int)segs.size();
-    o.seg.clear();
-    for (const Seg &sg : segs)
-      for (int v : {sg.sn0, sg.sn1, sg.c0, sg.c1, sg.lds, sg.nL, sg.accN, (int)FKp[sg.c0], (int)FKp[sg.c1], (int)FLp[sg.c0], sg.nout, sg.omap0})
-        o.seg.push_back(v);
-    static_assert(SparsePlanHost::kSegStride == 12, "segment table layout");
-    std::vector<char> col_lds(k, 0);
-    for (const Seg &sg : segs)
-      if (sg.lds) std::fill(col_lds.begin() + sg.c0, col_lds.begin() + sg.c1, 1);
-    o.Kdesc.assign((size_t)(o.nnzK + 64 * 8) * 4, 0);
-    o.KmapL.assign((size_t)o.nnzK + 64 * 8, 0);
-    o.KdescT.clear(); o.KmapT.clear();
-    {
-      size_t si = 0;
-      for (int j = 0; j < k; ++j) {
-        while (segs[si].c1 <= j) ++si;
-        const Seg &sg = segs[si];
-        for (int p = FKp[j]; p < FKp[j + 1]; ++p) {
-          const int kind = FKkind[p], idx = FKidx[p];
-          int r = 0, c = 0;
-          if (kind == K_P) { r = o.Pi[idx]; c = o.Pcol[idx]; }
-          else if (kind == K_A) { r = o.Arow[idx]; c = o.Aj[idx]; }
-          const int32_t d4[4] = {kind, idx, r, c};
-          std::copy(d4, d4 + 4, o.Kdesc.begin() + 4 * (size_t)p);
-          if (sg.lds) {
-            const int g = o.Kmap[p];
-            o.KmapL[p]  = (g < o.nnzL) ? g - FLp[sg.c0] : sg.nL + (g - o.nnzL - sg.c0);
-          } else {
-            o.KdescT.insert(o.KdescT.end(), d4, d4 + 4);
-            o.KmapT.push_back(o.Kmap[p]);
+    auto seg_tables = [&] {
+      o.nseg = (int)segs.size();
+      o.seg.clear();
+      for (const Seg &sg : segs)
+        for (int v : {sg.sn0, sg.sn1, sg.c0, sg.c1, sg.lds, sg.nL, sg.accN, (int)FKp[sg.c0], (int)FKp[sg.c1], (int)FLp[sg.c0], sg.nout, sg.omap0})
+          o.seg.push_back(v);
+      static_assert(SparsePlanHost::kSegStride == 12, "segment table layout");
+      std::vector<char> col_lds(k, 0);
+      for (const Seg &sg : segs)
+        if (sg.lds) std::fill(col_lds.begin() + sg.c0, col_lds.begin() + sg.c1, 1);
+      o.Kdesc.assign((size_t)(o.nnzK + 64 * 8) * 4, 0);
+      o.KmapL.assign((size_t)o.nnzK + 64 * 8, 0);
+      o.KdescT.clear(); o.KmapT.clear();
+      {
+        size_t si = 0;
+        for (int j = 0; j < k; ++j) {
+          while (segs[si].c1 <= j) ++si;
+          const Seg &sg = segs[si];
+          for (int p = FKp[j]; p < FKp[j + 1]; ++p) {
+            const int kind = FKkind[p], idx = FKidx[p];
+            int r = 0, c = 0;
+            if (kind == K_P) { r = o.Pi[idx]; c = o.Pcol[idx]; }
+            else if (kind == K_A) { r = o.Arow[idx]; c = o.Aj[idx]; }
+            const int32_t d4[4] = {kind, idx, r, c};
+            std::copy(d4, d4 + 4, o.Kdesc.begin() + 4 * (size_t)p);
+            if (sg.lds) {
+              const int g = o.Kmap[p];
+              o.KmapL[p]  = (g < o.nnzL) ? g - FLp[sg.c0] : sg.nL + (g - o.nnzL - sg.c0);
+            } else {
+              o.KdescT.insert(o.KdescT.end(), d4, d4 + 4);
+              o.KmapT.push_back(o.Kmap[p]);
+            }
           }
         }
       }
-    }
-    o.nnzKT = (int)o.KmapT.size();
-    for (int pad = 0; pad < 64 * 8; ++pad) {
-      const int32_t d4[4] = {K_SIGMA, 0, 0, 0};
-      o.KdescT.insert(o.KdescT.end(), d4, d4 + 4);
-      o.KmapT.push_back(SCRATCH);
-    }
-    for (size_t p = o.nnzK; p < (size_t)o.nnzK + 64 * 8; ++p) o.Kdesc[4 * p] = K_SIGMA;
-    o.Kmap.resize((size_t)o.nnzK + 64 * 8, SCRATCH);
-    o.ztop.clear();
-    for (const Seg &sg : segs)
-      if (!sg.lds) {
-        o.ztop.push_back(FLp[sg.c0]); o.ztop.push_back(FLp[sg.c1] - FLp[sg.c0]);
-        o.ztop.push_back(o.nnzL + sg.c0); o.ztop.push_back(sg.c1 - sg.c0);
-      }
-    o.ztop.push_back(SCRATCH); o.ztop.push_back(2);
-    o.nztop = (int)o.ztop.size() / 2;
+      o.nnzKT = (int)o.KmapT.size();
+      for (int pad = 0; pad < 64 * 8; ++pad) {
+        const int32_t d4[4] = {K_SIGMA, 0, 0, 0};
+        o.KdescT.insert(o.KdescT.end(), d4, d4 + 4);
+        o.KmapT.push_back(SCRATCH);
+      }
+      for (size_t p = o.nnzK; p < (size_t)o.nnzK + 64 * 8; ++p) o.Kdesc[4 * p] = K_SIGMA;
+      o.Kmap.resize((size_t)o.nnzK + 64 * 8, SCRATCH);
+      o.ztop.clear();
+      for (const Seg &sg : segs)
+        if (!sg.lds) {
+          o.ztop.push_back(FLp[sg.c0]); o.ztop.push_back(FLp[sg.c1] - FLp[sg.c0]);
+          o.ztop.push_back(o.nnzL + sg.c0); o.ztop.push_back(sg.c1 - sg.c0);
+        }
+      o.ztop.push_back(SCRATCH); o.ztop.push_back(2);
+      o.nztop = (int)o.ztop.size() / 2;
+    };
+    seg_tables();
     if (const char *dbg = sfb::knob("SFB_PLAN_DEBUG"); dbg && dbg[0] == '1') {
       int maxR = 0, over64 = 0, nlds = 0, cols_lds = 0;
       long long panel = 0, acc_lds = 0, ext = 0, internal = 0;
@@ -842,6 +854,39 @@
       o.pmapL.push_back(0);
       o.rtgt.push_back(SCRATCH);
       o.rab.push_back(0);
+    }
+
+    o.wide.clear();
+    const char *wk = sfb::knob("SFB_PLAN_WIDE");
+    if (o.units && lds_hint == 0 && !(wk && wk[0] == '0')) {
+      const int budgets[SparsePlanHost::kMaxWide] = {(int)polisher_wide_lds_doubles(n, m), lat_form_fits(n, m) ? (int)lat_lds_doubles(n, m) : 0};
+      auto swap_sched = [&](SparsePlanHost::UnitSchedule &s) {
+        std::swap(s.lds_doubles, o.lds_doubles); std::swap(s.nseg, o.nseg); std::swap(s.nunits, o.nunits);
+        std::swap(s.nnzKT, o.nnzKT); std::swap(s.nztop, o.nztop);
+        s.seg.swap(o.seg); s.ustream.swap(o.ustream); s.utype.swap(o.utype); s.uomap.swap(o.uomap);
+        s.KmapL.swap(o.KmapL); s.KdescT.swap(o.KdescT); s.KmapT.swap(o.KmapT); s.ztop.swap(o.ztop);
+      };
+      for (const int b : budgets) {
+        const SparsePlanHost::UnitSchedule *prev = o.wide.empty() ? nullptr : &o.wide.back();
+        if (b <= (prev ? prev->lds_doubles : o.lds_doubles)) continue;
+        SparsePlanHost::UnitSchedule s;
+        swap_sched(s);
+        o.lds_doubles = b;
+        const int got = unit_engine();
+        if (got == 1) seg_tables();
+        swap_sched(s);
+        if (got < 0) return false;
+        if (got == 0) break;
+        if (s.seg == (prev ? prev->seg : o.seg)) continue;
+        for (int sg = 0; sg < s.nseg; ++sg) {
+          const int32_t *sp = s.seg.data() + SparsePlanHost::kSegStride * sg;
+          if (sp[6] + sp[10] + 3 > b) { *msg = "internal: wide segment does not fit its LDS"; return false; }
+        }
+        o.wide.push_back(std::move(s));
+      }
+      if (const char *dbg = sfb::knob("SFB_PLAN_DEBUG"); dbg && dbg[0] == '1')
+        for (const auto &s : o.wide)
+          fprintf(stderr, "[sfb plan] wide schedule for %d doubles: %d units, %d segments\n", s.lds_doubles, s.nunits, s.nseg);
     }
   }
   auto acc_of = [&](int posS) { return posF[posS]; };
diff --git a/smooth_feedback_amd/csrc/sparse_plan.h b/smooth_feedback_amd/csrc/sparse_plan.h
--- a/smooth_feedback_amd/csrc/sparse_plan.h
+++ b/smooth_feedback_amd/csrc/sparse_plan.h
@@ -33,6 +33,12 @@
   int nseg = 0, nnzKT = 0, nztop = 0;
   std::vector<int32_t> ustream, utype, uomap;
   int units = 0, nunits = 0;
+  struct UnitSchedule {
+    int lds_doubles = 0, nseg = 0, nunits = 0, nnzKT = 0, nztop = 0;
+    std::vector<int32_t> seg, ustream, utype, uomap, KmapL, KdescT, KmapT, ztop;
+  };
+  static constexpr int kMaxWide = 2;
+  std::vector<UnitSchedule> wide;
 };
 
 bool build_sparse_plan(int n, int m, const int32_t *Pp, const int32_t *Pi, const int32_t *Ap, const int32_t *Aj,
```

Result: no change. 216,300, median of 6 (+0.2%).
